# joshuacwnewton/swiftwatcher

Measured on AMD Instinct MI355X. Metric: frames/sec (segment+classify) on 1080p ROI batches, higher is better.
Workload: dtype f64 (image_filtering), f32 (CNN)

## Files before the change

### include/swk.h

```cpp
#ifndef SWK_H
#define SWK_H

#include <stdint.h>

#ifdef __cplusplus
extern "C" {
#endif

#define SWK_ABI_VERSION 2

enum {
    SWK_OK = 0,
    SWK_ERR_ARG = -1,
    SWK_ERR_HIP = -2,
    SWK_ERR_NOGPU = -3,
    SWK_ERR_CAPACITY = -4,
    SWK_ERR_NOMEM = -5,
    SWK_ERR_STALE = -6
};

enum { SWK_MEM_HOST = 0, SWK_MEM_DEVICE = 1 };

enum { SWK_ORDER_RASTER = 0, SWK_ORDER_BLOCK2X2 = 1 };

enum { SWK_GRAY_Q14 = 0, SWK_GRAY_Q15 = 1 };

typedef struct swk_ctx swk_ctx;

typedef struct swk_params {
    double  lmbda;
    double  tol;
    int32_t maxiter;
    int32_t bil_d;
    double  bil_sigma_color;
    double  bil_sigma_space;
    int32_t bil_fma;
    int32_t thresh;
    int32_t open_kh, open_kw;
    int32_t connectivity;
    int32_t label_order;
    int32_t gray_mode;
    int32_t reserved_;
} swk_params;

typedef struct swk_segment {
    int32_t label;
    int32_t r0, c0, r1, c1;
    int32_t reserved_;
    int64_t area;
    int64_t sum_r, sum_c;
} swk_segment;

typedef struct swk_input {
    const uint8_t *frames;
    int32_t mem;
    int32_t channels;
    int32_t nwin;
    int32_t n;
    int32_t Hc, Wc;
    int32_t x0, y0;
    int64_t frame_stride;
    int64_t row_stride;
} swk_input;

typedef struct swk_output {
    int32_t mem;
    int32_t seg_cap;
    uint8_t *gray, *rpca, *bilateral, *thresh, *opened, *labels;
    double  *A, *E;
    int32_t *iters;
    int32_t *nseg;
    swk_segment *segs;
    int32_t planes_on_device;
    int32_t reserved_;
} swk_output;

int32_t swk_abi_version(void);
void    swk_params_default(swk_params *p);
int32_t swk_ctx_create(int32_t device, int32_t max_windows, int32_t max_n,
                       int32_t max_Hc, int32_t max_Wc, swk_ctx **out);
void    swk_ctx_destroy(swk_ctx *ctx);
const char *swk_last_error(const swk_ctx *ctx);
int64_t swk_ctx_device_bytes(const swk_ctx *ctx);

int32_t swk_pinned_alloc(int32_t device, int64_t bytes, void **out);
int32_t swk_pinned_free(void *p);
int32_t swk_stage_frames(const uint8_t *const *frames, int32_t count, int64_t row_stride, int32_t y0, int32_t rows, int64_t x_bytes,
                         int64_t row_bytes, uint8_t *dst, int32_t threads);
int32_t swk_cut_boxes(const uint8_t *const *frames, int32_t nframes, int64_t row_stride, int32_t pixel_bytes, int32_t count,
                      const int32_t *frame_of, const int32_t *boxes, const int64_t *offsets, uint8_t *out);
int32_t swk_device_alloc(swk_ctx *ctx, int64_t bytes, void **out);
int32_t swk_device_free(swk_ctx *ctx, void *p);
int32_t swk_device_read(swk_ctx *ctx, const void *src_device, void *dst_host, int64_t bytes);

int32_t swk_batch_run(swk_ctx *ctx, const swk_input *in, const swk_params *p, swk_output *out);
int32_t swk_batch_run_groups(swk_ctx *ctx, const swk_input *groups, int32_t ngroups, const swk_params *p, swk_output *outs);

enum { SWK_YUV_I420 = 0,
       SWK_YUV_NV12 = 1 };

typedef struct swk_yuv420 {
    const uint8_t *y, *u, *v;
    int32_t mem;
    int32_t layout;
    int32_t H, W;
    int64_t y_row_stride, y_frame_stride;
    int64_t c_row_stride, c_frame_stride;
} swk_yuv420;

int32_t swk_yuv420_to_bgr(swk_ctx *ctx, const swk_yuv420 *src, int32_t count, int32_t x0, int32_t y0, int32_t Hr, int32_t Wr,
                          uint8_t *bgr, int32_t bgr_mem);

int32_t swk_bgr2gray(swk_ctx *ctx, const uint8_t *bgr, int32_t count, int32_t H, int32_t W,
                     int32_t gray_mode, uint8_t *gray);
int32_t swk_ialm(swk_ctx *ctx, const uint8_t *planes, int32_t n, int32_t P,
                 double lmbda, double tol, int32_t maxiter,
                 double *A, double *E, int32_t *iters);
int32_t swk_rpca_epilogue(swk_ctx *ctx, const double *E, int64_t count, uint8_t *S);
int32_t swk_bilateral_u8(swk_ctx *ctx, const uint8_t *src, int32_t count, int32_t H, int32_t W,
                         int32_t d, double sigma_color, double sigma_space, int32_t use_fma,
                         uint8_t *dst);
int32_t swk_thresh_tozero_u8(swk_ctx *ctx, const uint8_t *src, int64_t count, int32_t thresh,
                             uint8_t *dst);
int32_t swk_grey_open3x3_u8(swk_ctx *ctx, const uint8_t *src, int32_t count, int32_t H, int32_t W,
                            uint8_t *dst);
int32_t swk_grey_open_u8(swk_ctx *ctx, const uint8_t *src, int32_t count, int32_t H, int32_t W, int32_t kh, int32_t kw, uint8_t *dst);
int32_t swk_resize_linear_u8(swk_ctx *ctx, const uint8_t *src, int32_t count, int32_t H, int32_t W, int32_t channels, int32_t dH, int32_t dW,
                             uint8_t *dst);
int32_t swk_ccl_u8(swk_ctx *ctx, const uint8_t *src, int32_t count, int32_t H, int32_t W,
                   int32_t connectivity, int32_t label_order, int32_t *labels, int32_t *ncomp);
int32_t swk_regionprops_u8(swk_ctx *ctx, const uint8_t *labels, int32_t count, int32_t H, int32_t W,
                           int32_t seg_cap, swk_segment *segs, int32_t *nseg);

int32_t swk_classifier_input(swk_ctx *ctx, const uint8_t *crops, int64_t crops_bytes, const int64_t *offsets,
                             const int32_t *hw, int32_t nseg, const float mean[3], const float std_[3],
                             uint8_t *patches, float *net, int32_t net_mem);
int32_t swk_classifier_input_window(swk_ctx *ctx, const uint8_t *crops, int64_t crops_bytes, const int64_t *offsets,
                                    const int32_t *hw, int32_t nseg, const float mean[3], const float std_[3],
                                    int32_t pad, int32_t channels_last, uint8_t *patches, float *net, int32_t net_mem);

int32_t swk_segment_inputs(swk_ctx *ctx, const swk_input *in, int32_t frame_h, int32_t frame_w,
                           const swk_segment *segs, const int32_t *nseg, int32_t seg_cap, int32_t min_h, int32_t min_w,
                           const float mean[3], const float std_[3], int32_t pad, int32_t channels_last, int32_t first,
                           int32_t net_cap, float *net, int32_t *seg_frame, int32_t *total, int32_t *skipped);
int32_t swk_segment_inputs_last(swk_ctx *ctx, int32_t min_h, int32_t min_w, const float mean[3], const float std_[3],
                                int32_t pad, int32_t channels_last, int32_t first, int32_t net_cap, float *net,
                                int32_t *seg_frame, int32_t *total, int32_t *skipped);

int32_t swk_nhwc_bias_relu_place(void *stream, const float *src, int32_t n, int32_t sh, int32_t sw, int32_t c, int32_t crop_y,
                                 int32_t crop_x, int32_t h, int32_t w, const float *bias, float *dst, int32_t dH, int32_t dW,
                                 int32_t dC, int32_t off_y, int32_t off_x, int32_t c_off);
int32_t swk_nhwc_maxpool3s2(void *stream, const float *src, int32_t n, int32_t h, int32_t w, int32_t c, float *dst);
int32_t swk_nhwc_head2_relu_mean(void *stream, const float *x, int32_t n, int32_t px, int32_t c, const float *w, const float *bias,
                                 const float *ring, float n_pos, float *out);
int32_t swk_nhwc_head2_dropout_relu_mean(void *stream, const float *x, int32_t n, int32_t px, int32_t c, const int32_t *pos, const float *bg,
                                         int32_t n_pos, const float *w, const float *bias, const uint64_t *keys, uint64_t seed,
                                         int32_t samples, float *out);
int32_t swk_nhwc_conv7x7s2_bias_relu(void *stream, const float *src, int32_t n, int32_t side, int32_t lo, int32_t m, const float *weight,
                                     const float *bias, int32_t cout, float *dst);
int32_t swk_nhwc_conv1x1_bias_relu_place(void *stream, const float *src, int32_t n, int32_t sh, int32_t sw, int32_t cin, int32_t crop_y,
                                         int32_t crop_x, int32_t h, int32_t w, const float *weight, const float *bias, int32_t cout,
                                         float *dst, int32_t dH, int32_t dW, int32_t dC, int32_t off_y, int32_t off_x, int32_t c_off);

int32_t swk_nhwc_maxpool3s2_conv1x1_bias_relu_place(void *stream, const float *src, int32_t n, int32_t t, int32_t cin, const float *weight,
                                                    const float *bias, int32_t cout, float *dst, int32_t dH, int32_t dW, int32_t dC,
                                                    int32_t off_y, int32_t off_x, const float *ring, int32_t live_lo, int32_t live_n);


int32_t swk_nhwc_conv3x3_bias_relu_place(void *stream, const float *src, int32_t n, int32_t t, int32_t cin, const float *weight_t,
                                         const float *bias, int32_t cout, float *dst, int32_t dH, int32_t dW, int32_t dC, int32_t off_y,
                                         int32_t off_x, int32_t c_off);

int32_t swk_winograd_f2x2_3x3_weights(const float *weight, int32_t cout, int32_t cin, float *out);
int32_t swk_nhwc_conv3x3_winograd_bias_relu_place(void *stream, const float *src, int32_t n, int32_t t, int32_t cin, const float *weight_w,
                                                  const float *bias, int32_t cout, float *dst, int32_t dH, int32_t dW, int32_t dC,
                                                  int32_t off_y, int32_t off_x, int32_t c_off);

int32_t swk_winograd_f2x2_3x3_weights_bf16s(const float *weight, int32_t cout, int32_t cin, uint16_t *out);
int32_t swk_nhwc_conv3x3_winograd_bf16s_bias_relu_place(void *stream, const float *src, int32_t n, int32_t t, int32_t cin,
                                                        const uint16_t *weight_s, const float *bias, int32_t cout, float *dst, int32_t dH,
                                                        int32_t dW, int32_t dC, int32_t off_y, int32_t off_x, int32_t c_off);

int32_t swk_track_costs(const double *prev_c, const double *prev_hist0, const uint8_t *prev_has_hist,
                        const double *curr_c, int32_t n_prev, int32_t n_curr, double *cost);
int32_t swk_lsap(const double *cost, int32_t n_rows, int32_t n_cols, int32_t *col4row);

int32_t swk_median_blur_u8(const uint8_t *src, int32_t H, int32_t W, int32_t channels, int32_t ksize, uint8_t *dst);
int32_t swk_otsu_threshold_u8(const uint8_t *src, int64_t count, uint8_t *dst, int32_t *thresh);
int32_t swk_canny_u8(const uint8_t *src, int32_t H, int32_t W, int32_t low, int32_t high, uint8_t *dst);
int32_t swk_dilate_up_u8(const uint8_t *src, int32_t H, int32_t W, int32_t N, uint8_t *dst);
int32_t swk_roi_mask(const uint8_t *frame, int32_t H, int32_t W, int64_t row_stride, const int32_t corners[4],
                     int32_t crop_region[4], uint8_t *mask, int64_t mask_capacity);


#ifdef __cplusplus
}
#endif
#endif
```

### swiftwatcher_amd/_lib.py

```python
import ctypes
import os
import threading

import numpy as np

_HERE = os.path.dirname(os.path.abspath(__file__))
LIB_PATH = os.environ.get("SWK_LIB", os.path.join(_HERE, "libswk.so"))

ABI_VERSION = 2
MEM_HOST, MEM_DEVICE = 0, 1
ERR_STALE = -6
STAGE_DENSE, STAGE_WHOLE, STAGE_ROWS, STAGE_2D, STAGE_DEVICE = 0, 1, 2, 3, -1
STAGES = ("gray", "rpca", "bilateral", "thresh", "opened", "labels")
ORDER_RASTER, ORDER_BLOCK2X2 = 0, 1
GRAY_Q14, GRAY_Q15 = 0, 1
YUV_I420, YUV_NV12 = 0, 1
K_GRAY, K_IALM_STATS, K_IALM_PASS, K_IALM_SMALL, K_FILTER, K_CCL, K_PROPS, K_COPY = range(8)
KERNEL_FAMILIES = ["gray", "ialm_stats", "ialm_pass", "ialm_small", "filter", "ccl", "props", "copy"]

c_u8p = ctypes.POINTER(ctypes.c_uint8)
c_f64p = ctypes.POINTER(ctypes.c_double)
c_i32p = ctypes.POINTER(ctypes.c_int32)


class SwkError(RuntimeError):
    pass


class StaleBatch(SwkError):
    """What a batch left on the device has been overwritten by a later call on the same context."""


class Params(ctypes.Structure):
    _fields_ = [("lmbda", ctypes.c_double), ("tol", ctypes.c_double), ("maxiter", ctypes.c_int32),
                ("bil_d", ctypes.c_int32), ("bil_sigma_color", ctypes.c_double),
                ("bil_sigma_space", ctypes.c_double), ("bil_fma", ctypes.c_int32),
                ("thresh", ctypes.c_int32), ("open_kh", ctypes.c_int32), ("open_kw", ctypes.c_int32),
                ("connectivity", ctypes.c_int32), ("label_order", ctypes.c_int32),
                ("gray_mode", ctypes.c_int32), ("reserved_", ctypes.c_int32)]


class Segment(ctypes.Structure):
    _fields_ = [("label", ctypes.c_int32), ("r0", ctypes.c_int32), ("c0", ctypes.c_int32),
                ("r1", ctypes.c_int32), ("c1", ctypes.c_int32), ("reserved_", ctypes.c_int32),
                ("area", ctypes.c_int64), ("sum_r", ctypes.c_int64), ("sum_c", ctypes.c_int64)]


SEGMENT_DTYPE = np.dtype([("label", "<i4"), ("r0", "<i4"), ("c0", "<i4"), ("r1", "<i4"), ("c1", "<i4"),
                          ("reserved_", "<i4"), ("area", "<i8"), ("sum_r", "<i8"), ("sum_c", "<i8")])
assert SEGMENT_DTYPE.itemsize == ctypes.sizeof(Segment) == 48


class Input(ctypes.Structure):
    _fields_ = [("frames", ctypes.c_void_p), ("mem", ctypes.c_int32), ("channels", ctypes.c_int32),
                ("nwin", ctypes.c_int32), ("n", ctypes.c_int32), ("Hc", ctypes.c_int32), ("Wc", ctypes.c_int32),
                ("x0", ctypes.c_int32), ("y0", ctypes.c_int32),
                ("frame_stride", ctypes.c_int64), ("row_stride", ctypes.c_int64)]


class Output(ctypes.Structure):
    _fields_ = [("mem", ctypes.c_int32), ("seg_cap", ctypes.c_int32),
                ("gray", ctypes.c_void_p), ("rpca", ctypes.c_void_p), ("bilateral", ctypes.c_void_p),
                ("thresh", ctypes.c_void_p), ("opened", ctypes.c_void_p), ("labels", ctypes.c_void_p),
                ("A", ctypes.c_void_p), ("E", ctypes.c_void_p),
                ("iters", ctypes.c_void_p), ("nseg", ctypes.c_void_p), ("segs", ctypes.c_void_p),
                ("planes_on_device", ctypes.c_int32), ("reserved_", ctypes.c_int32)]


class Yuv420(ctypes.Structure):
    _fields_ = [("y", ctypes.c_void_p), ("u", ctypes.c_void_p), ("v", ctypes.c_void_p), ("mem", ctypes.c_int32),
                ("layout", ctypes.c_int32), ("H", ctypes.c_int32), ("W", ctypes.c_int32),
                ("y_row_stride", ctypes.c_int64), ("y_frame_stride", ctypes.c_int64),
                ("c_row_stride", ctypes.c_int64), ("c_frame_stride", ctypes.c_int64)]


_lib = None
_lib_lock = threading.Lock()

_SIGS = {
    "swk_abi_version": (ctypes.c_int32, []),
    "swk_params_default": (None, [ctypes.POINTER(Params)]),
    "swk_ctx_create": (ctypes.c_int32, [ctypes.c_int32] * 5 + [ctypes.POINTER(ctypes.c_void_p)]),
    "swk_ctx_destroy": (None, [ctypes.c_void_p]),
    "swk_last_error": (ctypes.c_char_p, [ctypes.c_void_p]),
    "swk_ctx_device_bytes": (ctypes.c_int64, [ctypes.c_void_p]),
    "swk_batch_run": (ctypes.c_int32, [ctypes.c_void_p, ctypes.POINTER(Input), ctypes.POINTER(Params), ctypes.POINTER(Output)]),
    "swk_batch_run_groups": (ctypes.c_int32, [ctypes.c_void_p, ctypes.POINTER(Input), ctypes.c_int32, ctypes.POINTER(Params), ctypes.POINTER(Output)]),
    "swk_yuv420_to_bgr": (ctypes.c_int32, [ctypes.c_void_p, ctypes.POINTER(Yuv420)] + [ctypes.c_int32] * 5 + [ctypes.c_void_p, ctypes.c_int32]),
    "swk_bgr2gray": (ctypes.c_int32, [ctypes.c_void_p, ctypes.c_void_p, ctypes.c_int32, ctypes.c_int32, ctypes.c_int32, ctypes.c_int32, ctypes.c_void_p]),
    "swk_ialm": (ctypes.c_int32, [ctypes.c_void_p, ctypes.c_void_p, ctypes.c_int32, ctypes.c_int32, ctypes.c_double, ctypes.c_double, ctypes.c_int32, ctypes.c_void_p, ctypes.c_void_p, ctypes.c_void_p]),
    "swk_rpca_epilogue": (ctypes.c_int32, [ctypes.c_void_p, ctypes.c_void_p, ctypes.c_int64, ctypes.c_void_p]),
    "swk_bilateral_u8": (ctypes.c_int32, [ctypes.c_void_p, ctypes.c_void_p, ctypes.c_int32, ctypes.c_int32, ctypes.c_int32, ctypes.c_int32, ctypes.c_double, ctypes.c_double, ctypes.c_int32, ctypes.c_void_p]),
    "swk_thresh_tozero_u8": (ctypes.c_int32, [ctypes.c_void_p, ctypes.c_void_p, ctypes.c_int64, ctypes.c_int32, ctypes.c_void_p]),
    "swk_grey_open3x3_u8": (ctypes.c_int32, [ctypes.c_void_p, ctypes.c_void_p, ctypes.c_int32, ctypes.c_int32, ctypes.c_int32, ctypes.c_void_p]),
    "swk_grey_open_u8": (ctypes.c_int32, [ctypes.c_void_p, ctypes.c_void_p] + [ctypes.c_int32] * 5 + [ctypes.c_void_p]),
    "swk_resize_linear_u8": (ctypes.c_int32, [ctypes.c_void_p, ctypes.c_void_p] + [ctypes.c_int32] * 6 + [ctypes.c_void_p]),
    "swk_ccl_u8": (ctypes.c_int32, [ctypes.c_void_p, ctypes.c_void_p, ctypes.c_int32, ctypes.c_int32, ctypes.c_int32, ctypes.c_int32, ctypes.c_int32, ctypes.c_void_p, ctypes.c_void_p]),
    "swk_regionprops_u8": (ctypes.c_int32, [ctypes.c_void_p, ctypes.c_void_p, ctypes.c_int32, ctypes.c_int32, ctypes.c_int32, ctypes.c_int32, ctypes.c_void_p, ctypes.c_void_p]),
    "swk_classifier_input": (ctypes.c_int32, [ctypes.c_void_p, ctypes.c_void_p, ctypes.c_int64, ctypes.c_void_p, ctypes.c_void_p, ctypes.c_int32, ctypes.c_void_p, ctypes.c_void_p, ctypes.c_void_p, ctypes.c_void_p, ctypes.c_int32]),
    "swk_set_sparse_speculation": (ctypes.c_int32, [ctypes.c_void_p, ctypes.c_double]),
    "swk_set_integer_start": (ctypes.c_int32, [ctypes.c_void_p, ctypes.c_int32]),
    "swk_last_integer_start_windows": (ctypes.c_int32, [ctypes.c_void_p, ctypes.c_void_p]),
    "swk_debug_ialm_start": (ctypes.c_int32, [ctypes.c_void_p, ctypes.c_void_p, ctypes.c_int32, ctypes.c_int32, ctypes.c_int32, ctypes.c_double] + [ctypes.c_void_p] * 7),
    "swk_debug_ialm_first_step": (ctypes.c_int32, [ctypes.c_void_p, ctypes.c_void_p, ctypes.c_int32, ctypes.c_int32, ctypes.c_int32, ctypes.c_double] + [ctypes.c_void_p] * 7),
    "swk_last_host_stage": (ctypes.c_int32, [ctypes.c_void_p, ctypes.c_void_p, ctypes.c_int32]),
    "swk_debug_resize_table": (ctypes.c_int32, [ctypes.c_void_p, ctypes.c_int32, ctypes.c_int32, ctypes.c_int32, ctypes.c_void_p, ctypes.c_void_p]),
    "swk_last_eig_sweeps": (ctypes.c_int32, [ctypes.c_void_p, ctypes.c_void_p]),
    "swk_set_norm_speculation": (ctypes.c_int32, [ctypes.c_void_p, ctypes.c_double]),
    "swk_set_norm_guard": (ctypes.c_int32, [ctypes.c_void_p, ctypes.c_double]),
    "swk_prof_guard_windows": (ctypes.c_int32, [ctypes.c_void_p, ctypes.c_void_p]),
    "swk_last_stopping_norms": (ctypes.c_int32, [ctypes.c_void_p, ctypes.c_void_p, ctypes.c_void_p, ctypes.c_int32]),
    "swk_set_start_refine": (ctypes.c_int32, [ctypes.c_void_p, ctypes.c_double]),
    "swk_prof_refined_windows": (ctypes.c_int32, [ctypes.c_void_p, ctypes.c_void_p, ctypes.c_void_p]),
    "swk_prof_pass_bytes_per_element": (ctypes.c_int32, [ctypes.c_void_p, ctypes.c_void_p]),
    "swk_prof_redo_batches": (ctypes.c_int32, [ctypes.c_void_p, ctypes.c_void_p]),
    "swk_prof_redo_windows": (ctypes.c_int32, [ctypes.c_void_p, ctypes.c_void_p]),
    "swk_nhwc_bias_relu_place": (ctypes.c_int32, [ctypes.c_void_p, ctypes.c_void_p] + [ctypes.c_int32] * 8 + [ctypes.c_void_p, ctypes.c_void_p] + [ctypes.c_int32] * 6),
    "swk_set_cnn_tuning": (ctypes.c_int32, [ctypes.c_int32, ctypes.c_int32]),
    "swk_nhwc_conv7x7s2_bias_relu": (ctypes.c_int32, [ctypes.c_void_p, ctypes.c_void_p, ctypes.c_int32, ctypes.c_int32, ctypes.c_int32, ctypes.c_int32, ctypes.c_void_p, ctypes.c_void_p, ctypes.c_int32, ctypes.c_void_p]),
    "swk_nhwc_conv1x1_bias_relu_place": (ctypes.c_int32, [ctypes.c_void_p, ctypes.c_void_p] + [ctypes.c_int32] * 8 + [ctypes.c_void_p, ctypes.c_void_p, ctypes.c_int32, ctypes.c_void_p] + [ctypes.c_int32] * 6),
    "swk_nhwc_conv3x3_bias_relu_place": (ctypes.c_int32, [ctypes.c_void_p, ctypes.c_void_p, ctypes.c_int32, ctypes.c_int32, ctypes.c_int32, ctypes.c_void_p, ctypes.c_void_p, ctypes.c_int32, ctypes.c_void_p] + [ctypes.c_int32] * 6),
    "swk_nhwc_conv3x3_winograd_bias_relu_place": (ctypes.c_int32, [ctypes.c_void_p, ctypes.c_void_p, ctypes.c_int32, ctypes.c_int32, ctypes.c_int32, ctypes.c_void_p, ctypes.c_void_p, ctypes.c_int32, ctypes.c_void_p] + [ctypes.c_int32] * 6),
    "swk_winograd_f2x2_3x3_weights": (ctypes.c_int32, [ctypes.c_void_p, ctypes.c_int32, ctypes.c_int32, ctypes.c_void_p]),
    "swk_nhwc_conv3x3_winograd_bf16s_bias_relu_place": (ctypes.c_int32, [ctypes.c_void_p, ctypes.c_void_p, ctypes.c_int32, ctypes.c_int32, ctypes.c_int32, ctypes.c_void_p, ctypes.c_void_p, ctypes.c_int32, ctypes.c_void_p] + [ctypes.c_int32] * 6),
    "swk_winograd_f2x2_3x3_weights_bf16s": (ctypes.c_int32, [ctypes.c_void_p, ctypes.c_int32, ctypes.c_int32, ctypes.c_void_p]),
    "swk_nhwc_maxpool3s2_conv1x1_bias_relu_place": (ctypes.c_int32, [ctypes.c_void_p, ctypes.c_void_p, ctypes.c_int32, ctypes.c_int32, ctypes.c_int32, ctypes.c_void_p, ctypes.c_void_p, ctypes.c_int32, ctypes.c_void_p] + [ctypes.c_int32] * 5 + [ctypes.c_void_p, ctypes.c_int32, ctypes.c_int32]),
    "swk_nhwc_maxpool3s2": (ctypes.c_int32, [ctypes.c_void_p, ctypes.c_void_p, ctypes.c_int32, ctypes.c_int32, ctypes.c_int32, ctypes.c_int32, ctypes.c_void_p]),
    "swk_nhwc_head2_relu_mean": (ctypes.c_int32, [ctypes.c_void_p, ctypes.c_void_p, ctypes.c_int32, ctypes.c_int32, ctypes.c_int32, ctypes.c_void_p,
                                                  ctypes.c_void_p, ctypes.c_void_p, ctypes.c_float, ctypes.c_void_p]),
    "swk_nhwc_head2_dropout_relu_mean": (ctypes.c_int32, [ctypes.c_void_p, ctypes.c_void_p, ctypes.c_int32, ctypes.c_int32, ctypes.c_int32, ctypes.c_void_p,
                                                          ctypes.c_void_p, ctypes.c_int32, ctypes.c_void_p, ctypes.c_void_p, ctypes.c_void_p, ctypes.c_uint64,
                                                          ctypes.c_int32, ctypes.c_void_p]),
    "swk_segment_inputs": (ctypes.c_int32, [ctypes.c_void_p, ctypes.c_void_p, ctypes.c_int32, ctypes.c_int32, ctypes.c_void_p, ctypes.c_void_p, ctypes.c_int32, ctypes.c_int32, ctypes.c_int32, ctypes.c_void_p, ctypes.c_void_p, ctypes.c_int32, ctypes.c_int32, ctypes.c_int32, ctypes.c_int32, ctypes.c_void_p, ctypes.c_void_p, ctypes.c_void_p, ctypes.c_void_p]),
    "swk_segment_inputs_last": (ctypes.c_int32, [ctypes.c_void_p, ctypes.c_int32, ctypes.c_int32, ctypes.c_void_p, ctypes.c_void_p, ctypes.c_int32, ctypes.c_int32, ctypes.c_int32, ctypes.c_int32, ctypes.c_void_p, ctypes.c_void_p, ctypes.c_void_p, ctypes.c_void_p]),
    "swk_device_alloc": (ctypes.c_int32, [ctypes.c_void_p, ctypes.c_int64, ctypes.POINTER(ctypes.c_void_p)]),
    "swk_device_free": (ctypes.c_int32, [ctypes.c_void_p, ctypes.c_void_p]),
    "swk_device_read": (ctypes.c_int32, [ctypes.c_void_p, ctypes.c_void_p, ctypes.c_void_p, ctypes.c_int64]),
    "swk_classifier_input_window": (ctypes.c_int32, [ctypes.c_void_p, ctypes.c_void_p, ctypes.c_int64, ctypes.c_void_p, ctypes.c_void_p, ctypes.c_int32, ctypes.c_void_p, ctypes.c_void_p, ctypes.c_int32, ctypes.c_int32, ctypes.c_void_p, ctypes.c_void_p, ctypes.c_int32]),
    "swk_track_costs": (ctypes.c_int32, [ctypes.c_void_p, ctypes.c_void_p, ctypes.c_void_p, ctypes.c_void_p, ctypes.c_int32, ctypes.c_int32, ctypes.c_void_p]),
    "swk_lsap": (ctypes.c_int32, [ctypes.c_void_p, ctypes.c_int32, ctypes.c_int32, ctypes.c_void_p]),
    "swk_median_blur_u8": (ctypes.c_int32, [ctypes.c_void_p, ctypes.c_int32, ctypes.c_int32, ctypes.c_int32, ctypes.c_int32, ctypes.c_void_p]),
    "swk_otsu_threshold_u8": (ctypes.c_int32, [ctypes.c_void_p, ctypes.c_int64, ctypes.c_void_p, ctypes.c_void_p]),
    "swk_canny_u8": (ctypes.c_int32, [ctypes.c_void_p, ctypes.c_int32, ctypes.c_int32, ctypes.c_int32, ctypes.c_int32, ctypes.c_void_p]),
    "swk_dilate_up_u8": (ctypes.c_int32, [ctypes.c_void_p, ctypes.c_int32, ctypes.c_int32, ctypes.c_int32, ctypes.c_void_p]),
    "swk_roi_mask": (ctypes.c_int32, [ctypes.c_void_p, ctypes.c_int32, ctypes.c_int32, ctypes.c_int64, ctypes.c_void_p, ctypes.c_void_p, ctypes.c_void_p, ctypes.c_int64]),
    "swk_pinned_alloc": (ctypes.c_int32, [ctypes.c_int32, ctypes.c_int64, ctypes.POINTER(ctypes.c_void_p)]),
    "swk_pinned_free": (ctypes.c_int32, [ctypes.c_void_p]),
    "swk_cut_boxes": (ctypes.c_int32, [ctypes.c_void_p, ctypes.c_int32, ctypes.c_int64, ctypes.c_int32, ctypes.c_int32, ctypes.c_void_p, ctypes.c_void_p, ctypes.c_void_p, ctypes.c_void_p]),
    "swk_stage_frames": (ctypes.c_int32, [ctypes.c_void_p, ctypes.c_int32, ctypes.c_int64, ctypes.c_int32, ctypes.c_int32, ctypes.c_int64, ctypes.c_int64, ctypes.c_void_p, ctypes.c_int32]),
    "swk_prof_enable": (ctypes.c_int32, [ctypes.c_void_p, ctypes.c_int32]),
    "swk_prof_reset": (ctypes.c_int32, [ctypes.c_void_p]),
    "swk_prof_get": (ctypes.c_int32, [ctypes.c_void_p, ctypes.c_int32, ctypes.POINTER(ctypes.c_double), ctypes.POINTER(ctypes.c_int64)]),
    "swk_prof_window_iters": (ctypes.c_int32, [ctypes.c_void_p, ctypes.POINTER(ctypes.c_int64)]),
    "swk_set_ialm_variant": (ctypes.c_int32, [ctypes.c_void_p, ctypes.c_int32]),
    "swk_set_pass_tuning": (ctypes.c_int32, [ctypes.c_void_p, ctypes.c_int32]),
    "swk_set_eig_method": (ctypes.c_int32, [ctypes.c_void_p, ctypes.c_int32]),
}
EXPORTS = sorted(_SIGS)


def _preload_torch_hip_runtime():
    import importlib.util
    try:
        spec = importlib.util.find_spec("torch")
    except (ImportError, ValueError):
        spec = None
    if spec is None or not spec.origin:
        return
    cand = os.path.join(os.path.dirname(spec.origin), "lib", "libamdhip64.so")
    if os.path.exists(cand):
        try:
            ctypes.CDLL(cand, mode=ctypes.RTLD_GLOBAL)
        except OSError:
            pass


def load():
    global _lib
    with _lib_lock:
        if _lib is None:
            if not os.path.exists(LIB_PATH):
                raise SwkError("libswk.so not built: run `python swiftwatcher_amd/csrc/build.py` "
                               "(there is no CPU fallback)")
            _preload_torch_hip_runtime()
            lib = ctypes.CDLL(LIB_PATH)
            for name, (res, args) in _SIGS.items():
                fn = getattr(lib, name)
                fn.restype = res
                fn.argtypes = args
            if lib.swk_abi_version() != ABI_VERSION:
                raise SwkError("libswk.so ABI version mismatch")
            _lib = lib
    return _lib


def default_params(**overrides):
    p = Params()
    load().swk_params_default(ctypes.byref(p))
    for k, v in overrides.items():
        if not hasattr(p, k):
            raise TypeError("unknown swk parameter %r" % k)
        setattr(p, k, v)
    return p


def _ptr(a):
    return ctypes.c_void_p(a.ctypes.data) if a is not None else None


class _SerialisedLib:

    def __init__(self, lib, lock):
        self._lib, self._lock = lib, lock

    def __getattr__(self, name):
        fn = getattr(self._lib, name)
        lock = self._lock

        def call(*args):
            with lock:
                return fn(*args)
        call.__name__ = name
        setattr(self, name, call)
        return call


class Context:

    def __init__(self, device=0, max_windows=0, max_n=0, max_Hc=0, max_Wc=0):
        self._lock = threading.RLock()
        self._lib = _SerialisedLib(load(), self._lock)
        self._h = ctypes.c_void_p()
        rc = self._lib.swk_ctx_create(device, max_windows, max_n, max_Hc, max_Wc, ctypes.byref(self._h))
        if rc != 0:
            msg = self._lib.swk_last_error(None)
            self._h = None
            raise SwkError("swk_ctx_create failed (%d): %s" % (rc, msg.decode() if msg else "?"))
        self.device = device
        self.generation = 0
        self._plane_pool = {}

    def close(self):
        if getattr(self, "_h", None):
            for ptrs in self._plane_pool.values():
                for p in ptrs:
                    self._lib.swk_device_free(self._h, ctypes.c_void_p(p))
            self._plane_pool = {}
            self._lib.swk_ctx_destroy(self._h)
            self._h = None

    def device_alloc(self, nbytes):
        ptr = ctypes.c_void_p()
        self._check(self._lib.swk_device_alloc(self._h, int(nbytes), ctypes.byref(ptr)))
        return ptr.value

    def device_free(self, ptr):
        if getattr(self, "_h", None) and ptr:
            self._check(self._lib.swk_device_free(self._h, ctypes.c_void_p(ptr)))

    def device_read(self, ptr, shape, dtype=np.uint8):
        out = np.empty(shape, dtype)
        self._check(self._lib.swk_device_read(self._h, ctypes.c_void_p(ptr), _ptr(out), out.nbytes))
        return out

    def staging(self, shape):
        key = (threading.get_ident(), tuple(shape))
        with self._lock:
            cache = self.__dict__.setdefault("_staging", {})
            arr = cache.get(key)
            if arr is None:
                if len(cache) >= 3:
                    cache.pop(next(iter(cache)))
                arr = cache[key] = pinned_empty(shape, np.uint8, device=self.device)
        return arr

    def take_planes(self, nbytes):
        with self._lock:
            free = self._plane_pool.get(nbytes)
            if free:
                return free.pop()
        return self.device_alloc(nbytes)

    def give_planes(self, ptr, nbytes, keep=4):
        if not getattr(self, "_h", None):
            return
        with self._lock:
            free = self._plane_pool.setdefault(nbytes, [])
            if len(free) < keep:
                free.append(ptr)
                return
        self.device_free(ptr)

    def __del__(self):
        try:
            self.close()
        except Exception:
            pass

    def _check(self, rc):
        if rc != 0:
            msg = self._lib.swk_last_error(self._h)
            raise SwkError("libswk error %d: %s" % (rc, msg.decode() if msg else "?"))

    @property
    def device_bytes(self):
        return int(self._lib.swk_ctx_device_bytes(self._h))

    def prof_enable(self, on=True):
        self._check(self._lib.swk_prof_enable(self._h, int(bool(on))))

    def prof_reset(self):
        self._check(self._lib.swk_prof_reset(self._h))

    def prof(self):
        out = {}
        for i, name in enumerate(KERNEL_FAMILIES):
            ms, n = ctypes.c_double(), ctypes.c_int64()
            self._check(self._lib.swk_prof_get(self._h, i, ctypes.byref(ms), ctypes.byref(n)))
            out[name] = (ms.value, n.value)
        wi = ctypes.c_int64()
        self._check(self._lib.swk_prof_window_iters(self._h, ctypes.byref(wi)))
        out["window_iters"] = wi.value
        return out

    def set_ialm_variant(self, variant):
        self._check(self._lib.swk_set_ialm_variant(self._h, int(variant)))

    def set_pass_tuning(self, flags):
        self._check(self._lib.swk_set_pass_tuning(self._h, int(flags)))

    def set_sparse_speculation(self, factor):
        self._check(self._lib.swk_set_sparse_speculation(self._h, float(factor)))

    def set_integer_start(self, on):
        self._check(self._lib.swk_set_integer_start(self._h, int(bool(on))))

    def set_norm_guard(self, rel):
        self._check(self._lib.swk_set_norm_guard(self._h, float(rel)))

    @property
    def guard_windows(self):
        v = ctypes.c_int64(0)
        self._check(self._lib.swk_prof_guard_windows(self._h, ctypes.byref(v)))
        return v.value

    def set_start_refine(self, tau):
        self._check(self._lib.swk_set_start_refine(self._h, float(tau)))

    @property
    def refined_windows(self):
        a, b = ctypes.c_int64(0), ctypes.c_int64(0)
        self._check(self._lib.swk_prof_refined_windows(self._h, ctypes.byref(a), ctypes.byref(b)))
        return a.value, b.value

    def last_stopping_norms(self, cap=4096):
        r, e = np.zeros(cap), np.zeros(cap)
        n = self._lib.swk_last_stopping_norms(self._h, _ptr(r), _ptr(e), cap)
        if n < 0:
            self._check(n)
        return r[:min(n, cap)], e[:min(n, cap)]

    def set_norm_speculation(self, factor):
        self._check(self._lib.swk_set_norm_speculation(self._h, float(factor)))

    @property
    def pass_bytes_per_element(self):
        v = ctypes.c_double(0)
        self._check(self._lib.swk_prof_pass_bytes_per_element(self._h, ctypes.byref(v)))
        return v.value

    @property
    def last_eig_sweeps(self):
        v = ctypes.c_int32(0)
        self._check(self._lib.swk_last_eig_sweeps(self._h, ctypes.byref(v)))
        return v.value

    @property
    def last_integer_start_windows(self):
        v = ctypes.c_int32(0)
        self._check(self._lib.swk_last_integer_start_windows(self._h, ctypes.byref(v)))
        return v.value

    def debug_ialm_start(self, windows, lmbda=0.01):
        x = np.ascontiguousarray(windows, np.uint8)
        nwin, n, P = x.shape
        G = np.zeros((nwin, n, n), np.float64)
        sumsq, maxv = np.zeros(nwin, np.uint64), np.zeros(nwin, np.uint32)
        int_gram, scal = np.zeros(nwin, np.int32), np.zeros((nwin, 4), np.float64)
        nblk, ran = np.zeros(1, np.int32), np.zeros(1, np.int32)
        self._check(self._lib.swk_debug_ialm_start(self._h, _ptr(x), nwin, n, P, float(lmbda), _ptr(G), _ptr(sumsq), _ptr(maxv),
                                                   _ptr(int_gram), _ptr(scal), _ptr(nblk), _ptr(ran)))
        return dict(G=G, sumsq=sumsq, maxv=maxv, int_gram=int_gram, dual_norm=scal[:, 0], mu_0=scal[:, 1], thr_0=scal[:, 2],
                    dnorm=scal[:, 3], nblk=int(nblk[0]), gram8_ran=int(ran[0]))

    def debug_ialm_first_step(self, windows, lmbda=0.01):
        x = np.ascontiguousarray(windows, np.uint8)
        nwin, n, P = x.shape
        B_fin, B_std = np.zeros((nwin, n, n), np.float64), np.zeros((nwin, n, n), np.float64)
        refine, sweeps, int_gram = np.zeros(nwin, np.int32), np.zeros(nwin, np.int32), np.zeros(nwin, np.int32)
        cond_sum, scal = np.zeros(nwin, np.float64), np.zeros((nwin, 4), np.float64)
        self._check(self._lib.swk_debug_ialm_first_step(self._h, _ptr(x), nwin, n, P, float(lmbda), _ptr(B_fin), _ptr(B_std),
                                                        _ptr(refine), _ptr(cond_sum), _ptr(sweeps), _ptr(int_gram), _ptr(scal)))
        return dict(B_fin=B_fin, B_std=B_std, refine=refine, cond_sum=cond_sum, sweeps=sweeps, int_gram=int_gram,
                    dual_norm=scal[:, 0], mu_0=scal[:, 1], thr_0=scal[:, 2], dnorm=scal[:, 3])

    def last_host_stage(self, cap=256):
        kinds = np.zeros(cap, np.int32)
        n = self._lib.swk_last_host_stage(self._h, _ptr(kinds), cap)
        if n < 0:
            self._check(n)
        return [int(k) for k in kinds[:min(n, cap)]]

    @property
    def redo_batches(self):
        v = ctypes.c_int64(0)
        self._check(self._lib.swk_prof_redo_batches(self._h, ctypes.byref(v)))
        return v.value

    @property
    def redo_windows(self):
        v = ctypes.c_int64(0)
        self._check(self._lib.swk_prof_redo_windows(self._h, ctypes.byref(v)))
        return v.value

    def set_eig_method(self, method):
        self._check(self._lib.swk_set_eig_method(self._h, int(method)))

    def batch_run_raw(self, inp, params, out):
        with self._lock:
            self.generation += 1
            generation = self.generation
            self._check(self._lib.swk_batch_run(self._h, ctypes.byref(inp), ctypes.byref(params), ctypes.byref(out)))
        return generation

    def _group_io(self, frames, nwin, n, crop, reverse_frames, seg_cap, stages, want_A, want_E, device_stages=False):
        F = nwin * n
        on_device = hasattr(frames, "data_ptr") and getattr(frames, "is_cuda", False)
        shape = tuple(frames.shape)
        if str(frames.dtype) != ("torch.uint8" if on_device else "uint8") or shape[0] != F or len(shape) not in (3, 4):
            raise ValueError("frames must be uint8 (nwin*n, H, W[, 3])")
        if on_device:
            strides, base = tuple(int(x) for x in frames.stride()), frames.data_ptr()
        else:
            strides, base = frames.strides, frames.ctypes.data
        ch = 1 if len(shape) == 3 else shape[3]
        if (len(shape) == 4 and (strides[3] != 1 or strides[2] != ch)) or (len(shape) == 3 and strides[2] != 1):
            raise ValueError("frames must be contiguous along columns/channels")
        H, W = shape[1], shape[2]
        x0, y0, Wc, Hc = crop if crop is not None else (0, 0, W, H)
        if x0 < 0 or y0 < 0 or x0 + Wc > W or y0 + Hc > H:
            raise ValueError("crop rectangle outside the frame")
        inp = Input(frames=base + ((F - 1) * strides[0] if reverse_frames else 0), mem=MEM_DEVICE if on_device else MEM_HOST,
                    channels=ch, nwin=nwin, n=n, Hc=Hc, Wc=Wc, x0=x0, y0=y0,
                    frame_stride=-strides[0] if reverse_frames else strides[0], row_stride=strides[1])
        res = {}
        out = Output(mem=MEM_HOST, seg_cap=seg_cap)
        if device_stages and stages:
            planes = res["planes"] = DevicePlanes(self, tuple(stages), F, Hc, Wc)
            out.planes_on_device = 1
            for name in stages:
                setattr(out, name, planes.pointer(name))
        else:
            for name in stages:
                res[name] = np.empty((F, Hc, Wc), np.uint8)
                setattr(out, name, res[name].ctypes.data)
        P = Hc * Wc
        if want_A:
            res["A"] = np.empty((nwin, P, n), np.float64)
            out.A = res["A"].ctypes.data
        if want_E:
            res["E"] = np.empty((nwin, P, n), np.float64)
            out.E = res["E"].ctypes.data
        res["iters"] = np.zeros(nwin, np.int32)
        res["nseg"] = np.zeros(F, np.int32)
        res["segs"] = np.zeros((F, seg_cap), SEGMENT_DTYPE)
        out.iters = res["iters"].ctypes.data
        out.nseg = res["nseg"].ctypes.data
        out.segs = res["segs"].ctypes.data
        return inp, out, res

    def batch_run(self, frames, nwin, n, crop=None, params=None, stages=STAGES, want_A=False, want_E=False, seg_cap=255,
                  device_stages=False, reverse_frames=False):
        inp, out, res = self._group_io(frames, nwin, n, crop, reverse_frames, seg_cap, stages, want_A, want_E, device_stages)
        res["generation"] = self.batch_run_raw(inp, params or default_params(), out)
        return res

    def batch_run_groups(self, groups, params=None, stages=STAGES, want_A=False, want_E=False, seg_cap=255):
        params = params or default_params()
        G = len(groups)
        if G < 1:
            raise ValueError("no groups")
        ins = (Input * G)()
        outs = (Output * G)()
        results = []
        for g, grp in enumerate(groups):
            ins[g], outs[g], res = self._group_io(grp["frames"], int(grp["nwin"]), int(grp["n"]), grp.get("crop"),
                                                  bool(grp.get("reverse_frames", False)), int(grp.get("seg_cap", seg_cap)), stages,
                                                  want_A, want_E)
            results.append(res)
        with self._lock:
            self.generation += 1
            generation = self.generation
            self._check(self._lib.swk_batch_run_groups(self._h, ins, G, ctypes.byref(params), outs))
        for res in results:
            res["generation"] = generation
        return results

    def yuv420_to_bgr(self, y, u, v=None, rect=None, device_out=False):
        on_device = hasattr(y, "data_ptr") and getattr(y, "is_cuda", False)
        planes = [y, u] + ([v] if v is not None else [])
        want = "torch.uint8" if on_device else "uint8"
        if not on_device:
            planes = [p if isinstance(p, np.ndarray) and p.dtype == np.uint8 and p.ndim and p.strides[-1] == 1 else np.ascontiguousarray(p, np.uint8)
                      for p in planes]
        if any((hasattr(p, "data_ptr") and getattr(p, "is_cuda", False)) != on_device or str(p.dtype) != want for p in planes):
            raise ValueError("the planes must be uint8, all numpy arrays or all tensors on the context's GPU")
        single = len(planes[0].shape) == 2
        if single:
            planes = [p[None] for p in planes]

        def geometry(p):
            if on_device:
                return tuple(p.shape), tuple(int(x) for x in p.stride()), p.data_ptr()
            return p.shape, p.strides, p.ctypes.data
        (yshape, ystr, yptr), (cshape, cstr, uptr) = geometry(planes[0]), geometry(planes[1])
        if len(yshape) != 3 or ystr[2] != 1:
            raise ValueError("y must be (count, H, W), contiguous along a row")
        count, H, W = yshape
        ch, cw = (H + 1) // 2, (W + 1) // 2
        if v is not None:
            vshape, vstr, vptr = geometry(planes[2])
            if tuple(cshape) != (count, ch, cw) or tuple(vshape) != (count, ch, cw) or cstr[2] != 1 or tuple(vstr) != tuple(cstr):
                raise ValueError("u and v must be (count, ceil(H/2), ceil(W/2)) with equal strides, contiguous along a row")
            layout = YUV_I420
        else:
            vptr = None
            ok = (len(cshape) == 4 and tuple(cshape) == (count, ch, cw, 2) and cstr[3] == 1 and cstr[2] == 2) or \
                 (len(cshape) == 3 and tuple(cshape) == (count, ch, 2 * cw) and cstr[2] == 1)
            if not ok:
                raise ValueError("the NV12 chroma plane must be (count, ceil(H/2), ceil(W/2), 2) or (count, ceil(H/2), 2 ceil(W/2))")
            layout = YUV_NV12
        x0, y0, Wr, Hr = rect if rect is not None else (0, 0, W, H)
        src = Yuv420(y=yptr, u=uptr, v=vptr, mem=MEM_DEVICE if on_device else MEM_HOST, layout=layout, H=H, W=W,
                     y_row_stride=ystr[1], y_frame_stride=ystr[0], c_row_stride=cstr[1], c_frame_stride=cstr[0])
        shape = (count, int(Hr), int(Wr), 3) if Hr > 0 and Wr > 0 and count > 0 else (1, 1, 1, 3)
        if device_out:
            import torch
            out = torch.empty(shape, dtype=torch.uint8, device="cuda:%d" % self.device)
            optr, omem = ctypes.c_void_p(out.data_ptr()), MEM_DEVICE
        else:
            out = np.empty(shape, np.uint8)
            optr, omem = _ptr(out), MEM_HOST
        self._check(self._lib.swk_yuv420_to_bgr(self._h, ctypes.byref(src), count, int(x0), int(y0), int(Hr), int(Wr), optr, omem))
        return out[0] if single else out

    def bgr2gray(self, bgr, gray_mode=GRAY_Q14):
        bgr = np.ascontiguousarray(bgr, np.uint8)
        single = bgr.ndim == 3
        b4 = bgr[None] if single else bgr
        cnt, H, W, _ = b4.shape
        out = np.empty((cnt, H, W), np.uint8)
        self._check(self._lib.swk_bgr2gray(self._h, _ptr(b4), cnt, H, W, gray_mode, _ptr(out)))
        return out[0] if single else out

    def ialm(self, planes, lmbda=0.01, tol=0.001, maxiter=100, want_E=True):
        planes = np.ascontiguousarray(planes, np.uint8)
        n, P = planes.shape
        A = np.empty((P, n), np.float64)
        E = np.empty((P, n), np.float64) if want_E else None
        it = np.zeros(1, np.int32)
        self._check(self._lib.swk_ialm(self._h, _ptr(planes), n, P, lmbda, tol, maxiter, _ptr(A), _ptr(E), _ptr(it)))
        return A, E, int(it[0])

    def rpca_epilogue(self, E):
        E = np.ascontiguousarray(E, np.float64)
        out = np.empty(E.shape, np.uint8)
        self._check(self._lib.swk_rpca_epilogue(self._h, _ptr(E), E.size, _ptr(out)))
        return out

    def _planes(self, a):
        a = np.ascontiguousarray(a, np.uint8)
        return (a[None], True) if a.ndim == 2 else (a, False)

    def bilateral_u8(self, src, d=7, sigma_color=15.0, sigma_space=1.0, use_fma=False):
        s, single = self._planes(src)
        out = np.empty_like(s)
        self._check(self._lib.swk_bilateral_u8(self._h, _ptr(s), s.shape[0], s.shape[1], s.shape[2], d,
                                               sigma_color, sigma_space, int(bool(use_fma)), _ptr(out)))
        return out[0] if single else out

    def thresh_tozero_u8(self, src, thresh=15):
        s = np.ascontiguousarray(src, np.uint8)
        out = np.empty_like(s)
        self._check(self._lib.swk_thresh_tozero_u8(self._h, _ptr(s), s.size, thresh, _ptr(out)))
        return out

    def grey_open3x3_u8(self, src):
        s, single = self._planes(src)
        out = np.empty_like(s)
        self._check(self._lib.swk_grey_open3x3_u8(self._h, _ptr(s), s.shape[0], s.shape[1], s.shape[2], _ptr(out)))
        return out[0] if single else out

    def grey_open_u8(self, src, size):
        s, single = self._planes(src)
        out = np.empty_like(s)
        self._check(self._lib.swk_grey_open_u8(self._h, _ptr(s), s.shape[0], s.shape[1], s.shape[2], int(size[0]), int(size[1]), _ptr(out)))
        return out[0] if single else out

    def resize_linear_u8(self, frame, dsize):
        f = np.ascontiguousarray(frame, np.uint8)
        H, W = f.shape[:2]
        ch = 1 if f.ndim == 2 else f.shape[2]
        dW, dH = int(dsize[0]), int(dsize[1])
        out = np.empty((dH, dW) + ((ch,) if f.ndim == 3 else ()), np.uint8)
        self._check(self._lib.swk_resize_linear_u8(self._h, _ptr(f), 1, H, W, ch, dH, dW, _ptr(out)))
        return out

    def ccl_u8(self, src, connectivity=8, label_order=ORDER_BLOCK2X2):
        s, single = self._planes(src)
        lab = np.empty(s.shape, np.int32)
        nc = np.zeros(s.shape[0], np.int32)
        self._check(self._lib.swk_ccl_u8(self._h, _ptr(s), s.shape[0], s.shape[1], s.shape[2], connectivity,
                                         label_order, _ptr(lab), _ptr(nc)))
        return (int(nc[0]), lab[0]) if single else (nc, lab)

    def classifier_input(self, crops, mean, std, want_patches=False, net_ptr=None, pad=100, channels_last=False):
        n = len(crops)
        flat = [np.ascontiguousarray(c, np.uint8).reshape(-1) for c in crops]
        sizes = np.array([f.size for f in flat], np.int64)
        offsets = np.concatenate([[0], np.cumsum(sizes)[:-1]]).astype(np.int64)
        packed = np.concatenate(flat) if n else np.zeros(0, np.uint8)
        hw = np.array([[c.shape[0], c.shape[1]] for c in crops], np.int32)
        m = np.asarray(mean, np.float32)
        s = np.asarray(std, np.float32)
        patches = np.empty((n, 24, 24, 3), np.uint8) if want_patches else None
        net = None
        if net_ptr is None:
            net = np.empty((n, 3, 24 + 2 * pad, 24 + 2 * pad), np.float32)
            nptr, nmem = _ptr(net), MEM_HOST
        else:
            nptr, nmem = ctypes.c_void_p(net_ptr), MEM_DEVICE
        self._check(self._lib.swk_classifier_input_window(self._h, _ptr(packed), packed.size, _ptr(offsets), _ptr(hw), n,
                                                          _ptr(m), _ptr(s), int(pad), 1 if channels_last else 0, _ptr(patches), nptr,
                                                          nmem))
        return patches, net

    def segment_inputs(self, inp, frame_hw, segs_ptr, nseg_ptr, seg_cap, mean, std, net_ptr, net_cap, first=0, pad=8,
                       min_seg_size=(24, 24), seg_frame_ptr=None, channels_last=False):
        m = np.asarray(mean, np.float32)
        s = np.asarray(std, np.float32)
        total = ctypes.c_int32(0)
        skipped = ctypes.c_int32(0)
        self._check(self._lib.swk_segment_inputs(self._h, ctypes.byref(inp), int(frame_hw[0]), int(frame_hw[1]),
                                                 ctypes.c_void_p(segs_ptr), ctypes.c_void_p(nseg_ptr), int(seg_cap),
                                                 int(min_seg_size[0]), int(min_seg_size[1]), _ptr(m), _ptr(s), int(pad),
                                                 1 if channels_last else 0, int(first), int(net_cap), ctypes.c_void_p(net_ptr),
                                                 ctypes.c_void_p(seg_frame_ptr) if seg_frame_ptr else None,
                                                 ctypes.byref(total), ctypes.byref(skipped)))
        return total.value, skipped.value

    def segment_inputs_last(self, generation, mean, std, net_ptr, net_cap, first=0, pad=8, min_seg_size=(24, 24),
                            seg_frame_ptr=None, channels_last=False, known_total=-1):
        m = np.asarray(mean, np.float32)
        s = np.asarray(std, np.float32)
        total = ctypes.c_int32(int(known_total))
        skipped = ctypes.c_int32(0)
        with self._lock:
            if generation != self.generation:
                raise StaleBatch("the context has run another batch since")
            rc = self._lib.swk_segment_inputs_last(self._h, int(min_seg_size[0]), int(min_seg_size[1]), _ptr(m), _ptr(s), int(pad),
                                                   1 if channels_last else 0, int(first), int(net_cap), ctypes.c_void_p(net_ptr),
                                                   ctypes.c_void_p(seg_frame_ptr) if seg_frame_ptr else None,
                                                   ctypes.byref(total), ctypes.byref(skipped))
            if rc == ERR_STALE:
                raise StaleBatch("the context no longer holds that batch")
            self._check(rc)
        return total.value, skipped.value

    def debug_resize_table(self, first, count, route=1):
        bounds = np.empty((count, 24, 2), np.int32)
        coeffs = np.empty((count, 24, 343), np.int32)
        self._check(self._lib.swk_debug_resize_table(self._h, int(first), int(count), int(route), _ptr(bounds), _ptr(coeffs)))
        return bounds, coeffs

    def regionprops_u8(self, labels, seg_cap=255):
        s, single = self._planes(labels)
        segs = np.zeros((s.shape[0], seg_cap), SEGMENT_DTYPE)
        nseg = np.zeros(s.shape[0], np.int32)
        self._check(self._lib.swk_regionprops_u8(self._h, _ptr(s), s.shape[0], s.shape[1], s.shape[2], seg_cap,
                                                 _ptr(segs), _ptr(nseg)))
        return (segs[0, :nseg[0]], int(nseg[0])) if single else (segs, nseg)


def stage_frames(frames, y0, y1, x0, x1, dst, threads=4):
    f0 = frames[0]
    px = f0.strides[1] if f0.ndim >= 2 else 1
    ok = all(f.dtype == np.uint8 and f.shape == f0.shape and f.strides == f0.strides for f in frames) and \
        f0.ndim in (2, 3) and (f0.ndim == 2 or (f0.strides[2] == 1 and f0.strides[1] == f0.shape[2])) and \
        (f0.ndim == 3 or f0.strides[1] == 1) and f0.strides[0] >= f0.shape[1] * px and dst.flags.c_contiguous
    if not ok:
        for i, f in enumerate(frames):
            dst[i] = f[y0:y1, x0:x1]
        return
    ptrs = (ctypes.c_void_p * len(frames))(*[f.ctypes.data for f in frames])
    rc = load().swk_stage_frames(ptrs, len(frames), f0.strides[0], y0, y1 - y0, x0 * px, (x1 - x0) * px, dst.ctypes.data, threads)
    if rc:
        raise SwkError("swk_stage_frames failed (%d)" % rc)


def cut_boxes(arrays, frame_of, boxes):
    a0 = arrays[0]
    px = a0.strides[1]
    h = np.maximum(boxes[:, 1] - boxes[:, 0], 0).astype(np.int64)
    w = np.maximum(boxes[:, 3] - boxes[:, 2], 0).astype(np.int64)
    sizes = h * w * px
    offsets = np.zeros(len(boxes), np.int64)
    if len(boxes) > 1:
        np.cumsum(sizes[:-1], out=offsets[1:])
    out = np.empty(int(sizes.sum()) if len(boxes) else 0, np.uint8)
    if len(boxes):
        ptrs = (ctypes.c_void_p * len(arrays))(*[a.ctypes.data for a in arrays])
        fo = np.ascontiguousarray(frame_of, np.int32)
        bx = np.ascontiguousarray(boxes, np.int32)
        rc = load().swk_cut_boxes(ptrs, len(arrays), a0.strides[0], px, len(boxes), fo.ctypes.data, bx.ctypes.data, offsets.ctypes.data,
                                  out.ctypes.data)
        if rc:
            raise SwkError("swk_cut_boxes failed (%d)" % rc)
    return out, offsets


class DevicePlanes:

    def __init__(self, ctx, stages, F, Hc, Wc):
        self.ctx, self.stages, self.F, self.Hc, self.Wc = ctx, stages, F, Hc, Wc
        self.plane = F * Hc * Wc
        self.nbytes = (self.plane + 3) // 4 * 4 * len(stages)
        self.ptr = ctx.take_planes(self.nbytes)

    def pointer(self, stage):
        return self.ptr + self.stages.index(stage) * ((self.plane + 3) // 4 * 4)

    def read(self, stage, frame):
        return self.ctx.device_read(self.pointer(stage) + frame * self.Hc * self.Wc, (self.Hc, self.Wc))

    def read_stack(self, stage):
        return self.ctx.device_read(self.pointer(stage), (self.F, self.Hc, self.Wc))

    def __del__(self):
        try:
            if self.ptr:
                self.ctx.give_planes(self.ptr, self.nbytes)
                self.ptr = 0
        except Exception:
            pass


def track_costs(prev_c, prev_hist0, prev_has_hist, curr_c):
    n_prev, n_curr = len(prev_c), len(curr_c)
    pc = np.ascontiguousarray(prev_c, np.float64).reshape(n_prev, 2)
    ph = np.ascontiguousarray(prev_hist0, np.float64).reshape(n_prev, 2)
    hh = np.ascontiguousarray(prev_has_hist, np.uint8).reshape(n_prev)
    cc = np.ascontiguousarray(curr_c, np.float64).reshape(n_curr, 2)
    packed = np.concatenate([pc.ravel(), ph.ravel(), cc.ravel()])
    return track_costs_packed(packed, hh.tobytes(), n_prev, n_curr)


def track_costs_packed(packed, has_hist, n_prev, n_curr):
    n = n_prev + n_curr
    cost = np.empty((n, n), np.float64)
    base = packed.ctypes.data
    rc = _track_costs_fn()(base, base + 16 * n_prev, has_hist, base + 32 * n_prev, n_prev, n_curr, cost.ctypes.data)
    if rc:
        raise SwkError("swk_track_costs failed (%d)" % rc)
    return cost


_fast = {}


def _track_costs_fn():
    fn = _fast.get("costs")
    if fn is None:
        fn = _fast["costs"] = load().swk_track_costs
    return fn


def lsap(cost):
    if cost.dtype != np.float64 or not cost.flags.c_contiguous:
        cost = np.ascontiguousarray(cost, np.float64)
    nr, nc = cost.shape
    out = np.empty(nr, np.int32)
    fn = _fast.get("lsap")
    if fn is None:
        fn = _fast["lsap"] = load().swk_lsap
    rc = fn(cost.ctypes.data, nr, nc, out.ctypes.data)
    if rc:
        raise SwkError("swk_lsap failed (%d)" % rc)
    return out


def pinned_empty(shape, dtype=np.uint8, device=0):
    import weakref
    count = int(np.prod(shape))
    nbytes = max(count * np.dtype(dtype).itemsize, 1)
    lib = load()
    ptr = ctypes.c_void_p()
    if lib.swk_pinned_alloc(int(device), nbytes, ctypes.byref(ptr)) != 0 or not ptr.value:
        return np.empty(shape, dtype)
    buf = (ctypes.c_uint8 * nbytes).from_address(ptr.value)
    weakref.finalize(buf, lib.swk_pinned_free, ctypes.c_void_p(ptr.value))
    return np.frombuffer(buf, dtype=dtype, count=count).reshape(shape)


def _host_call(name, *args):
    rc = getattr(load(), name)(*args)
    if rc:
        raise SwkError("%s failed (%d)" % (name, rc))


def median_blur_u8(image, ksize):
    a = np.ascontiguousarray(image, np.uint8)
    ch = 1 if a.ndim == 2 else a.shape[2]
    out = np.empty_like(a)
    _host_call("swk_median_blur_u8", _ptr(a), a.shape[0], a.shape[1], ch, int(ksize), _ptr(out))
    return out


def otsu_threshold_u8(image):
    a = np.ascontiguousarray(image, np.uint8)
    out = np.empty_like(a)
    t = ctypes.c_int32(0)
    _host_call("swk_otsu_threshold_u8", _ptr(a), a.size, _ptr(out), ctypes.byref(t))
    return t.value, out


def canny_u8(image, low, high):
    a = np.ascontiguousarray(image, np.uint8)
    out = np.empty_like(a)
    _host_call("swk_canny_u8", _ptr(a), a.shape[0], a.shape[1], int(low), int(high), _ptr(out))
    return out


def dilate_up_u8(image, N):
    a = np.ascontiguousarray(image, np.uint8)
    out = np.empty_like(a)
    _host_call("swk_dilate_up_u8", _ptr(a), a.shape[0], a.shape[1], int(N), _ptr(out))
    return out


def roi_mask(frame, corners):
    if hasattr(frame, "as_full_frame"):
        frame = frame.as_full_frame()
    if not isinstance(frame, np.ndarray):
        frame = np.asarray(frame)
    if frame.dtype != np.uint8 or frame.ndim != 3 or frame.shape[2] != 3 or frame.strides[2] != 1 or frame.strides[1] != 3:
        frame = np.ascontiguousarray(frame, np.uint8)
    c = np.array([corners[0][0], corners[0][1], corners[1][0], corners[1][1]], np.int32)
    crop = np.zeros(4, np.int32)
    left, right = min(c[0], c[2]), max(c[0], c[2])
    width = int(right - left)
    hc, wc = int(0.5 * width) + int(0.125 * width), width + 2 * int(0.125 * width)
    mask = np.empty((max(hc, 1), max(wc, 1)), np.uint8)
    _host_call("swk_roi_mask", _ptr(frame), frame.shape[0], frame.shape[1], frame.strides[0], _ptr(c), _ptr(crop), _ptr(mask), mask.size)
    return [(int(crop[0]), int(crop[1])), (int(crop[2]), int(crop[3]))], mask


_default_ctx = {}
_ctx_lock = threading.Lock()


def default_context(device=0):
    with _ctx_lock:
        ctx = _default_ctx.get(device)
        if ctx is None:
            ctx = _default_ctx[device] = Context(device)
    return ctx
```

### swiftwatcher_amd/csrc/cnn_common.h

```cpp
#pragma once
#include "swk_internal.h"

#include <cstring>

namespace swk {

typedef float f16v __attribute__((ext_vector_type(16)));
typedef __bf16 bf16x8 __attribute__((ext_vector_type(8)));

struct Place {
    float *dst;
    int dH, dW, dC, off_y, off_x, c_off;
};
struct Crop {
    int sh, sw, crop_y, crop_x;
};

inline bool place_ok(const Place &p, int h, int w, int c, bool quads, const Crop *crop = nullptr)
{
    if (!p.dst || c < 1 || p.off_y < 0 || p.off_x < 0 || p.off_y + h > p.dH || p.off_x + w > p.dW || p.c_off < 0 || p.c_off + c > p.dC) return false;
    if (quads && ((c & 3) || (p.dC & 3) || (p.c_off & 3) || ((uintptr_t)p.dst & 15))) return false;
    return !crop || (crop->crop_y >= 0 && crop->crop_x >= 0 && crop->crop_y + h <= crop->sh && crop->crop_x + w <= crop->sw);
}

int launch_expand1x1_split_bf16(hipStream_t s, const float *src, int64_t rows, const Crop &cr, int cin, int h, int w, const float *wgt,
                                const float *bias, int cout, const Place &pl);
extern int g_expand_split_bf16;
extern int g_wino_bf16s_layout;

__device__ __forceinline__ void store_bias_relu(float *q, const f16v &acc, int g, const float4 b)
{
    float4 v;
    v.x = fmaxf(acc[4 * g] + b.x, 0.0f);
    v.y = fmaxf(acc[4 * g + 1] + b.y, 0.0f);
    v.z = fmaxf(acc[4 * g + 2] + b.z, 0.0f);
    v.w = fmaxf(acc[4 * g + 3] + b.w, 0.0f);
    *(float4 *)q = v;
}

__device__ __forceinline__ void split3(float x, __bf16 &a, __bf16 &b, __bf16 &c)
{
    a = (__bf16)x;
    const float r = x - (float)a;
    b = (__bf16)r;
    c = (__bf16)(r - (float)b);
}
inline void split3_host(float x, uint16_t part[3])
{
    for (int i = 0; i < 3; ++i) {
        uint32_t u;
        float back;
        memcpy(&u, &x, 4);
        u = (u + 0x7fffu + ((u >> 16) & 1u)) & 0xffff0000u;
        memcpy(&back, &u, 4);
        part[i] = (uint16_t)(u >> 16);
        x -= back;
    }
}

inline void winograd_U(const float g[9], double U[4][4])
{
    static const double G[4][3] = {{1.0, 0.0, 0.0}, {0.5, 0.5, 0.5}, {0.5, -0.5, 0.5}, {0.0, 0.0, 1.0}};
    double tmp[4][3];
    for (int a = 0; a < 4; ++a)
        for (int c = 0; c < 3; ++c) tmp[a][c] = G[a][0] * g[c] + G[a][1] * g[3 + c] + G[a][2] * g[6 + c];
    for (int a = 0; a < 4; ++a)
        for (int c = 0; c < 4; ++c) U[a][c] = tmp[a][0] * G[c][0] + tmp[a][1] * G[c][1] + tmp[a][2] * G[c][2];
}

template <int N>
__device__ __forceinline__ void lds_dma_copy(unsigned lds, const void *g, unsigned voff)
{
    static_assert(N >= 1 && N <= 3, "1 KB pieces per statement");
    unsigned keep;
#define SWK_LDS_DMA(pieces)                                                                                                 \
    asm volatile("s_mov_b32 %0, m0\n\ts_mov_b32 m0, %2\n\ts_nop 0\n\t" pieces "s_mov_b32 m0, %0" : "=&s"(keep) : "v"(voff), "s"(lds), "s"(g) : "memory")
#define SWK_LDS_DMA_PIECE(offset) "global_load_lds_dwordx4 %1, %3" offset "\n\t"
    if constexpr (N == 1) SWK_LDS_DMA(SWK_LDS_DMA_PIECE(""));
    else if constexpr (N == 2) SWK_LDS_DMA(SWK_LDS_DMA_PIECE("") SWK_LDS_DMA_PIECE(" offset:1024"));
    else SWK_LDS_DMA(SWK_LDS_DMA_PIECE("") SWK_LDS_DMA_PIECE(" offset:1024") SWK_LDS_DMA_PIECE(" offset:2048"));
#undef SWK_LDS_DMA_PIECE
#undef SWK_LDS_DMA
}
template <int KEEP>
__device__ __forceinline__ void lds_dma_wait()
{
    asm volatile("s_waitcnt vmcnt(%0)" ::"n"(KEEP) : "memory");
}

}
```

### swiftwatcher_amd/csrc/cnn_conv1x1.hip

```cpp
#include "cnn_common.h"

namespace swk {

template <int NBLK, int KC, int D, int CS, int NWV>
__global__ __launch_bounds__(64 * NWV) void k_conv1x1_relu_place(const float *__restrict__ src, int64_t rows, int sh, int sw, int cin, int crop_y,
                                                            int crop_x, int h, int w, const float *__restrict__ wgt, const float *__restrict__ bias,
                                                            int cout, float *__restrict__ dst, int dH, int dW, int dC, int off_y, int off_x, int c_off,
                                                            FastDiv fhw, FastDiv fw)
{
    constexpr int NP = 32 * NBLK, PITCH = NP + 1, KH = KC / 2, NV = KH / 4, NB = NBLK / CS, NT = 64 * NWV, SLOTS = NWV / CS;
    static_assert(NBLK % CS == 0 && NWV % CS == 0, "column splits");
    extern __shared__ float lds[];
    const int tid = threadIdx.x, lane = tid & 63, wave = tid >> 6, r = lane & 31, hh = lane >> 5;
    float *lbias = lds + ((cin * PITCH + 3) & ~3);
    const int hw = h * w;
    const int cs = wave % CS;
    const int64_t ntiles = (rows + 31) >> 5, stride = (int64_t)gridDim.x * SLOTS;
    int64_t tile = (int64_t)blockIdx.x * SLOTS + wave / CS;

    auto locate = [&](int64_t t, int64_t &ro) -> const float * {
        const unsigned m = (unsigned)t * 32u + (unsigned)r;
        const bool valid = m < (unsigned)rows;
        const unsigned mm = valid ? m : (unsigned)rows - 1u;
        const unsigned b = fhw.div(mm), rem = mm - b * (unsigned)hw;
        const unsigned y = fw.div(rem), x = rem - y * (unsigned)w;
        ro = valid ? (((int64_t)b * dH + off_y + y) * dW + off_x + x) * (int64_t)dC + c_off + 32 * NB * cs : -1;
        return src + (((int64_t)b * sh + crop_y + y) * sw + crop_x + x) * (int64_t)cin + KH * hh;
    };
    float4 a[D][NV];
    int64_t ro = -1, ro_next = -1;
    const float *p = src, *pn = src;
    if (tile < ntiles) {
        p = locate(tile, ro);
#pragma unroll
        for (int d = 0; d < D; ++d)
#pragma unroll
            for (int v = 0; v < NV; ++v) a[d][v] = *(const float4 *)(p + KC * d + 4 * v);
    }
    for (int co = tid >> 4; co < NP; co += NT / 16)
        for (int c4 = (tid & 15) * 4; c4 < cin; c4 += 64) {
            const float4 wv = co < cout ? *(const float4 *)(wgt + (int64_t)co * cin + c4) : make_float4(0.0f, 0.0f, 0.0f, 0.0f);
            float *q = lds + c4 * PITCH + co;
            q[0] = wv.x; q[PITCH] = wv.y; q[2 * PITCH] = wv.z; q[3 * PITCH] = wv.w;
        }
    for (int i = tid; i < NP; i += NT) lbias[i] = i < cout ? bias[i] : 0.0f;
    __syncthreads();

    for (; tile < ntiles; tile += stride) {
        const bool more = tile + stride < ntiles;
        if (more) pn = locate(tile + stride, ro_next);
        f16v acc[NB];
#pragma unroll
        for (int nb = 0; nb < NB; ++nb)
#pragma unroll
            for (int e = 0; e < 16; ++e) acc[nb][e] = 0.0f;
        for (int kb = 0; kb < cin; kb += KC * D) {
#pragma unroll
            for (int d = 0; d < D; ++d) {
                const int k0 = kb + KC * d;
                float av[KH];
#pragma unroll
                for (int v = 0; v < NV; ++v) { av[4 * v] = a[d][v].x; av[4 * v + 1] = a[d][v].y; av[4 * v + 2] = a[d][v].z; av[4 * v + 3] = a[d][v].w; }
                const int kn = k0 + KC * D;
                if (kn < cin) {
#pragma unroll
                    for (int v = 0; v < NV; ++v) a[d][v] = *(const float4 *)(p + kn + 4 * v);
                } else if (more) {
#pragma unroll
                    for (int v = 0; v < NV; ++v) a[d][v] = *(const float4 *)(pn + kn - cin + 4 * v);
                }
                const float *wrow = lds + (k0 + KH * hh) * PITCH + 32 * NB * cs + r;
                float bw[2][NB];
#pragma unroll
                for (int nb = 0; nb < NB; ++nb) bw[0][nb] = wrow[32 * nb];
#pragma unroll
                for (int i = 0; i < KH; ++i) {
                    if (i < KH - 1) {
#pragma unroll
                        for (int nb = 0; nb < NB; ++nb) bw[(i + 1) & 1][nb] = wrow[(i + 1) * PITCH + 32 * nb];
                    }
#pragma unroll
                    for (int nb = 0; nb < NB; ++nb) acc[nb] = __builtin_amdgcn_mfma_f32_32x32x2f32(bw[i & 1][nb], av[i], acc[nb], 0, 0, 0);
                    if (i < KH - 1) __builtin_amdgcn_sched_group_barrier(0x100 , NB, 0);
                    __builtin_amdgcn_sched_group_barrier(0x008 , NB, 0);
                }
            }
        }
        if (ro >= 0) {
            float *o = dst + ro + 4 * hh;
#pragma unroll
            for (int nb = 0; nb < NB; ++nb)
#pragma unroll
                for (int g = 0; g < 4; ++g) {
                    const int c = nb * 32 + 8 * g;
                    if (32 * NB * cs + c + 4 * hh < cout) store_bias_relu(o + c, acc[nb], g, *(const float4 *)(lbias + 32 * NB * cs + c + 4 * hh));
                }
        }
        p = pn;
        ro = ro_next;
    }
}

template <int NBLK, int KC, int D, int CS, int NWV>
static int launch_conv1x1_d(hipStream_t s, const float *src, int64_t rows, const Crop &cr, int cin, int h, int w, const float *wgt,
                            const float *bias, int cout, const Place &pl)
{
    const size_t lds = (size_t)(((cin * (32 * NBLK + 1) + 3) & ~3) + 32 * NBLK) * sizeof(float);
    static unsigned long long attr_mask = 0;
    if (!ensure_dyn_lds((const void *)k_conv1x1_relu_place<NBLK, KC, D, CS, NWV>, 160 * 1024 - 256, attr_mask)) return SWK_ERR_HIP;
    if (lds > 160 * 1024 - 256 || rows > (int64_t)0x7fffff00) return SWK_ERR_CAPACITY;
    constexpr int SLOTS = NWV / CS;
    const int64_t ntiles = (rows + 31) / 32;
    int64_t blocks = (ntiles + SLOTS - 1) / SLOTS;
    const int64_t by_lds = (int64_t)((160 * 1024 - 256) / lds), by_waves = 16 / NWV;
    const int64_t per_cu = by_lds < 1 ? 1 : (by_lds < by_waves ? by_lds : by_waves);
    const int64_t cap = 256 * per_cu;
    if (blocks > cap) blocks = cap;
    hipLaunchKernelGGL((k_conv1x1_relu_place<NBLK, KC, D, CS, NWV>), dim3((unsigned)blocks), dim3(64 * NWV), lds, s, src, rows, cr.sh, cr.sw, cin,
                       cr.crop_y, cr.crop_x, h, w, wgt, bias, cout, pl.dst, pl.dH, pl.dW, pl.dC, pl.off_y, pl.off_x, pl.c_off, FastDiv((unsigned)(h * w)), FastDiv((unsigned)w));
    return hipGetLastError() == hipSuccess ? SWK_OK : SWK_ERR_HIP;
}

int g_expand_split_bf16 = getenv("SWK_EXPAND_SPLIT_BF16") ? atoi(getenv("SWK_EXPAND_SPLIT_BF16")) : 0;
int g_conv1x1_ring = 0;

#define SWK_C1_ARGS s, src, rows, cr, cin, h, w, wgt, bias, cout, pl
template <int NBLK>
static int launch_conv1x1(hipStream_t s, const float *src, int64_t rows, const Crop &cr, int cin, int h, int w, const float *wgt, const float *bias,
                          int cout, const Place &pl)
{
    constexpr int CS = NBLK >= 6 ? 2 : 1;
    if (g_conv1x1_ring == 0) {
        const int64_t ntiles = (rows + 31) / 32;
        const int nwv = ntiles >= 16 * 160 / CS ? 16 : ntiles >= 8 * 160 / CS ? 8 : 4;
#define SWK_C1_BY_WAVES(KC)                                                              \
        do {                                                                             \
            if (nwv == 16) return launch_conv1x1_d<NBLK, KC, 1, CS, 16>(SWK_C1_ARGS);    \
            if (nwv == 8) return launch_conv1x1_d<NBLK, KC, 1, CS, 8>(SWK_C1_ARGS);      \
            return launch_conv1x1_d<NBLK, KC, 1, CS, 4>(SWK_C1_ARGS);                    \
        } while (0)
        if (cin % 32 == 0) SWK_C1_BY_WAVES(32);
        if (cin == 48) SWK_C1_BY_WAVES(48);
        SWK_C1_BY_WAVES(16);
#undef SWK_C1_BY_WAVES
    }
    if (cin % 32 == 0) {
        const int n = cin / 32, dmax = NBLK >= 6 ? 2 : 4;
        const int d = dmax >= 4 && n % 4 == 0 ? 4 : dmax >= 3 && n % 3 == 0 ? 3 : dmax >= 2 && n % 2 == 0 ? 2 : 1;
        switch (d) {
        case 4: if constexpr (NBLK < 6) return launch_conv1x1_d<NBLK, 32, 4, 1, 8>(SWK_C1_ARGS);
        case 3: if constexpr (NBLK < 6) return launch_conv1x1_d<NBLK, 32, 3, 1, 8>(SWK_C1_ARGS);
        case 2: return launch_conv1x1_d<NBLK, 32, 2, 1, 8>(SWK_C1_ARGS);
        default: return launch_conv1x1_d<NBLK, 32, 1, 1, 8>(SWK_C1_ARGS);
        }
    }
    if (cin == 48) return launch_conv1x1_d<NBLK, 48, 1, 1, 8>(SWK_C1_ARGS);
    return launch_conv1x1_d<NBLK, 16, 1, 1, 8>(SWK_C1_ARGS);
}
#undef SWK_C1_ARGS

}

#pragma GCC visibility push(default)
extern "C" {

int32_t swk_nhwc_conv1x1_bias_relu_place(void *stream, const float *src, int32_t n, int32_t sh, int32_t sw, int32_t cin, int32_t crop_y,
                                         int32_t crop_x, int32_t h, int32_t w, const float *weight, const float *bias, int32_t cout,
                                         float *dst, int32_t dH, int32_t dW, int32_t dC, int32_t off_y, int32_t off_x, int32_t c_off)
{
    const swk::Place pl{dst, dH, dW, dC, off_y, off_x, c_off};
    const swk::Crop cr{sh, sw, crop_y, crop_x};
    if (!src || !weight || !bias || n < 1 || h < 1 || w < 1 || cin < 16 || (cin & 15) || cin > 1024 || cout > 256 ||
        !swk::place_ok(pl, h, w, cout, true, &cr) || ((((uintptr_t)src) | ((uintptr_t)weight)) & 15))
        return SWK_ERR_ARG;
    using namespace swk;
    const int64_t rows = (int64_t)n * h * w;
    hipStream_t s = (hipStream_t)stream;
    if (g_expand_split_bf16 && cout == 4 * cin) {
        const int rc = launch_expand1x1_split_bf16(s, src, rows, cr, cin, h, w, weight, bias, cout, pl);
        if (rc != SWK_ERR_ARG) return rc;
    }
    switch ((cout + 31) / 32) {
    case 1: return launch_conv1x1<1>(s, src, rows, cr, cin, h, w, weight, bias, cout, pl);
    case 2: return launch_conv1x1<2>(s, src, rows, cr, cin, h, w, weight, bias, cout, pl);
    case 3: return launch_conv1x1<3>(s, src, rows, cr, cin, h, w, weight, bias, cout, pl);
    case 4: return launch_conv1x1<4>(s, src, rows, cr, cin, h, w, weight, bias, cout, pl);
    case 6: return launch_conv1x1<6>(s, src, rows, cr, cin, h, w, weight, bias, cout, pl);
    case 8: return launch_conv1x1<8>(s, src, rows, cr, cin, h, w, weight, bias, cout, pl);
    default: return SWK_ERR_ARG;
    }
}

int32_t swk_set_cnn_tuning(int32_t knob, int32_t value)
{
    if (knob == 0 && (value == 0 || value == 1)) { swk::g_conv1x1_ring = value; return SWK_OK; }
    if (knob == 1 && (value == 0 || value == 1)) { swk::g_expand_split_bf16 = value; return SWK_OK; }
    if (knob == 2 && value >= 0 && value <= 2) { swk::g_wino_bf16s_layout = value; return SWK_OK; }
    return SWK_ERR_ARG;
}

}
#pragma GCC visibility pop
```

### swiftwatcher_amd/csrc/cnn_wino3x3_bf16s.hip

```cpp
#include "cnn_common.h"

#include <type_traits>

namespace swk {

static int wino_bf16s_spp(int cin, int cout) { return cin == 64 && cout == 256 ? 2 : cin / 16; }

template <int KG> struct WinoVPad { static constexpr int value = KG == 6 ? 3 : 16 / KG; };

template <int NBLK, int SPP>
__global__ __launch_bounds__(64 * NBLK, 2) void k_wino3x3_bf16s_relu_place(const float *__restrict__ src, int nseg, int t, int T,
                                                                          const uint16_t *__restrict__ wu, const float *__restrict__ bias,
                                                                          int cout, float *__restrict__ dst, int dH, int dW, int dC, int off_y,
                                                                          int off_x, int c_off, FastDiv fTT, FastDiv fT)
{
    constexpr int NW = NBLK, NT = 64 * NW, KG = NBLK, CIN = 8 * KG, S = CIN / 16, PHS = S / SPP, SLOTS = 64, NP = 32 * NBLK;
    constexpr int VT = SLOTS + WinoVPad<KG>::value;
    constexpr int WPB = SPP * 3 * 1024;
    static_assert(S % SPP == 0 && NT == SLOTS * KG, "one staging item per thread");
    extern __shared__ uint4 lds_w[];
    char *const Wl = (char *)lds_w;
    uint4 *const V0 = (uint4 *)(Wl + 2 * NW * WPB), *const V1 = V0 + 3 * KG * VT;
    float *const lbias = (float *)(V1 + 3 * KG * VT);
    const int tid = threadIdx.x, lane = tid & 63, wave = tid >> 6, r = lane & 31, hh = lane >> 5;
    const int o = t - 2, TT = T * T;
    const int64_t ntiles = (int64_t)nseg * TT, src_floats = (int64_t)nseg * t * t * CIN;
    const int64_t ntasks = (ntiles + SLOTS - 1) / SLOTS;
    for (int i = tid; i < NP; i += NT) lbias[i] = i < cout ? bias[i] : 0.0f;

    const int sg = tid % KG, sslot = tid / KG;
    unsigned sbase;
    int slim;
    const char *const srcb = (const char *)src;
    auto stage_setup = [&](int64_t task) {
        int64_t m = task * SLOTS + sslot;
        if (m >= ntiles) m = ntiles - 1;
        const unsigned bu = fTT.div((unsigned)m), rem = (unsigned)m - bu * (unsigned)TT, ty = fT.div(rem), tx = rem - ty * (unsigned)T;
        const int64_t b = bu;
        const int64_t base = (((b * t + 2 * ty) * t + 2 * tx) * (int64_t)CIN + 8 * sg) * 4;
        const int64_t lim = src_floats * 4 - 32 - base;
        sbase = (unsigned)base;
        slim = (int)(lim < (1 << 30) ? lim : (1 << 30));
    };
    float4 st[4][2];
    auto stage_issue = [&](int p) {
        const int xi = p >> 2, nu = p & 3;
        const int ra0 = (0x1210 >> (4 * xi)) & 15, ra1 = (0x3122 >> (4 * xi)) & 15;
        const int rb0 = (0x1210 >> (4 * nu)) & 15, rb1 = (0x3122 >> (4 * nu)) & 15;
        const int os[4] = {(ra0 * t + rb0) * (CIN * 4), (ra0 * t + rb1) * (CIN * 4), (ra1 * t + rb0) * (CIN * 4), (ra1 * t + rb1) * (CIN * 4)};
#pragma unroll
        for (int i = 0; i < 4; ++i) {
            const char *q = srcb + (sbase + (unsigned)(os[i] < slim ? os[i] : slim));
            st[i][0] = *(const float4 *)q;
            st[i][1] = *(const float4 *)(q + 16);
        }
    };
    auto stage_store = [&](int p, uint4 *Vn) {
        const float sx = (p >> 2) == 1 ? 1.0f : -1.0f, sn = (p & 3) == 1 ? 1.0f : -1.0f;
        bf16x8 v1, v2, v3;
#pragma unroll
        for (int h = 0; h < 2; ++h) {
            const float a[4] = {st[0][h].x, st[0][h].y, st[0][h].z, st[0][h].w}, b[4] = {st[1][h].x, st[1][h].y, st[1][h].z, st[1][h].w},
                        c[4] = {st[2][h].x, st[2][h].y, st[2][h].z, st[2][h].w}, d[4] = {st[3][h].x, st[3][h].y, st[3][h].z, st[3][h].w};
#pragma unroll
            for (int e = 0; e < 4; ++e) {
                const float v = __builtin_fmaf(__builtin_fmaf(d[e], sn, c[e]), sx, __builtin_fmaf(b[e], sn, a[e]));
                __bf16 x1, x2, x3;
                split3(v, x1, x2, x3);
                v1[4 * h + e] = x1; v2[4 * h + e] = x2; v3[4 * h + e] = x3;
            }
        }
        uint4 *q = Vn + sg * VT + sslot;
        q[0] = __builtin_bit_cast(uint4, v1);
        q[KG * VT] = __builtin_bit_cast(uint4, v2);
        q[2 * KG * VT] = __builtin_bit_cast(uint4, v3);
    };

    const unsigned wvoff = (unsigned)(lane * 16);
    auto w_issue = [&](int g, int buf) {
        const char *gp = (const char *)wu + ((int64_t)g * NW + __builtin_amdgcn_readfirstlane(wave)) * WPB;
        const unsigned l = __builtin_amdgcn_readfirstlane((unsigned)(uintptr_t)(Wl + (buf * NW + wave) * WPB));
#pragma unroll
        for (int sub = 0; sub < SPP; ++sub) lds_dma_copy<3>(l + sub * 3072u, gp + sub * 3072, wvoff);
    };

    int64_t task = blockIdx.x;
    if (task < ntasks) {
        stage_setup(task);
        stage_issue(0);
        stage_store(0, V0);
        w_issue(0, 0);
    }
    lds_dma_wait<0>();
    __syncthreads();
    for (; task < ntasks; task += gridDim.x) {
        int64_t ro[2];
        bool valid[2], vy1[2], vx1[2];
#pragma unroll
        for (int tg = 0; tg < 2; ++tg) {
            const int64_t m = task * SLOTS + tg * 32 + r;
            valid[tg] = m < ntiles;
            const int64_t mm = valid[tg] ? m : ntiles - 1;
            const unsigned bu = fTT.div((unsigned)mm), rem = (unsigned)mm - bu * (unsigned)TT;
            const int ty = (int)fT.div(rem), tx = (int)(rem - (unsigned)ty * (unsigned)T);
            const int64_t b = bu;
            ro[tg] = ((b * dH + off_y + 2 * ty) * dW + off_x + 2 * tx) * (int64_t)dC + c_off + 32 * wave + 4 * hh;
            vy1[tg] = 2 * ty + 1 < o;
            vx1[tg] = 2 * tx + 1 < o;
        }
        const bool more = task + gridDim.x < ntasks;
        f16v Y[2][2][2];
#pragma unroll
        for (int i = 0; i < 2; ++i)
#pragma unroll
            for (int j = 0; j < 2; ++j)
#pragma unroll
                for (int tg = 0; tg < 2; ++tg)
#pragma unroll
                    for (int e = 0; e < 16; ++e) Y[i][j][tg][e] = 0.0f;
        auto phase = [&](const char *Wb, const uint4 *Vc, int s0, f16v *M) {
            const uint4 *wq = (const uint4 *)Wb + lane;
#pragma unroll
            for (int sub = 0; sub < SPP; ++sub) {
                const int s = s0 + sub;
                const bf16x8 u1 = __builtin_bit_cast(bf16x8, wq[(3 * sub) * 64]), u2 = __builtin_bit_cast(bf16x8, wq[(3 * sub + 1) * 64]),
                             u3 = __builtin_bit_cast(bf16x8, wq[(3 * sub + 2) * 64]);
#pragma unroll
                for (int tg = 0; tg < 2; ++tg) {
                    const uint4 *vq = Vc + (2 * s + hh) * VT + 32 * tg + r;
                    const bf16x8 x1 = __builtin_bit_cast(bf16x8, vq[0]), x2 = __builtin_bit_cast(bf16x8, vq[KG * VT]),
                                 x3 = __builtin_bit_cast(bf16x8, vq[2 * KG * VT]);
                    M[tg] = __builtin_amdgcn_mfma_f32_32x32x16_bf16(u1, x3, M[tg], 0, 0, 0);
                    M[tg] = __builtin_amdgcn_mfma_f32_32x32x16_bf16(u2, x2, M[tg], 0, 0, 0);
                    M[tg] = __builtin_amdgcn_mfma_f32_32x32x16_bf16(u3, x1, M[tg], 0, 0, 0);
                    M[tg] = __builtin_amdgcn_mfma_f32_32x32x16_bf16(u1, x2, M[tg], 0, 0, 0);
                    M[tg] = __builtin_amdgcn_mfma_f32_32x32x16_bf16(u2, x1, M[tg], 0, 0, 0);
                    M[tg] = __builtin_amdgcn_mfma_f32_32x32x16_bf16(u1, x1, M[tg], 0, 0, 0);
                }
            }
        };
        for (int p = 0; p < 16; ++p) {
            const uint4 *Vc = (p & 1) ? V1 : V0;
            uint4 *Vn = (p & 1) ? V0 : V1;
            const int pn = (p + 1) & 15;
            if (p == 15 && more) stage_setup(task + gridDim.x);
            const int xi = p >> 2, nu = p & 3;
            const float ax[2] = {xi < 3 ? 1.0f : 0.0f, xi == 0 ? 0.0f : xi == 1 ? 1.0f : -1.0f};
            const float an[2] = {nu < 3 ? 1.0f : 0.0f, nu == 0 ? 0.0f : nu == 1 ? 1.0f : -1.0f};
            f16v M[2];
#pragma unroll
            for (int tg = 0; tg < 2; ++tg)
#pragma unroll
                for (int e = 0; e < 16; ++e) M[tg][e] = 0.0f;
#pragma unroll
            for (int h = 0; h < PHS; ++h) {
                const int g = p * PHS + h, gn = g + 1 == 16 * PHS ? 0 : g + 1;
                w_issue(gn, (g + 1) & 1);
                if (h == 0) stage_issue(pn);
                phase(Wl + ((g & 1) * NW + wave) * WPB, Vc, h * SPP, M);
                if (h == PHS - 1) {
                    stage_store(pn, Vn);
#pragma unroll
                    for (int i = 0; i < 2; ++i)
#pragma unroll
                        for (int j = 0; j < 2; ++j) {
                            const float c = ax[i] * an[j];
                            if (c != 0.0f) {
#pragma unroll
                                for (int tg = 0; tg < 2; ++tg)
#pragma unroll
                                    for (int e = 0; e < 16; ++e) Y[i][j][tg][e] = __builtin_fmaf(M[tg][e], c, Y[i][j][tg][e]);
                            }
                        }
                }
                if (h == 0 && PHS > 1) lds_dma_wait<8>();
                else lds_dma_wait<0>();
                if (h == PHS - 1) __syncthreads();
            }
        }
#pragma unroll
        for (int tg = 0; tg < 2; ++tg) {
            if (!valid[tg]) continue;
#pragma unroll
            for (int i = 0; i < 2; ++i)
#pragma unroll
                for (int j = 0; j < 2; ++j) {
                    if ((i == 1 && !vy1[tg]) || (j == 1 && !vx1[tg])) continue;
                    float *q = dst + ro[tg] + ((int64_t)i * dW + j) * dC;
#pragma unroll
                    for (int gq = 0; gq < 4; ++gq) {
                        const int c = 32 * wave + 8 * gq + 4 * hh;
                        if (c < cout) store_bias_relu(q + 8 * gq, Y[i][j][tg], gq, *(const float4 *)(lbias + c));
                    }
                }
        }
    }
}

template <int NBLK, int SPP>
static int launch_wino3x3_bf16s(hipStream_t s, const float *src, int n, int t, const uint16_t *wu, const float *bias, int cout, const Place &pl)
{
    constexpr int NW = NBLK, KG = NBLK, CIN = 8 * NBLK, VT = 64 + WinoVPad<KG>::value;
    const size_t lds = (size_t)2 * NW * SPP * 3 * 1024 + (size_t)2 * 3 * KG * VT * 16 + 32 * NBLK * sizeof(float);
    static_assert((size_t)2 * NW * SPP * 3 * 1024 + (size_t)2 * 3 * KG * VT * 16 + 32 * NBLK * 4 <= 160 * 1024 - 256, "LDS of one workgroup");
    static unsigned long long attr_mask = 0;
    if (!ensure_dyn_lds((const void *)k_wino3x3_bf16s_relu_place<NBLK, SPP>, 160 * 1024 - 256, attr_mask)) return SWK_ERR_HIP;
    if ((int64_t)n * t * t * CIN * 4 >= ((int64_t)1 << 32)) return SWK_ERR_CAPACITY;
    const int T = (t - 2 + 1) / 2;
    const int64_t ntiles = (int64_t)n * T * T;
    int64_t blocks = (ntiles + 63) / 64;
    const int64_t by_lds = (int64_t)((160 * 1024 - 256) / lds), by_waves = 8 / NW;
    const int64_t per_cu = by_waves < 1 ? 1 : (by_lds < by_waves ? by_lds : by_waves);
    if (blocks > 256 * per_cu) blocks = 256 * per_cu;
    hipLaunchKernelGGL((k_wino3x3_bf16s_relu_place<NBLK, SPP>), dim3((unsigned)blocks), dim3(64 * NW), lds, s, src, n, t, T, wu, bias, cout, pl.dst,
                       pl.dH, pl.dW, pl.dC, pl.off_y, pl.off_x, pl.c_off, FastDiv((unsigned)(T * T)), FastDiv((unsigned)T));
    return hipGetLastError() == hipSuccess ? SWK_OK : SWK_ERR_HIP;
}

template <int KG> struct WinoVPadW { static constexpr int value = KG == 4 ? 2 : KG == 6 ? 3 : 1; };

typedef __bf16 bf16x4 __attribute__((ext_vector_type(4)));

template <int NBLK, int SPP, int TGW, int WCB, int WPS>
__global__ __launch_bounds__(64 * NBLK * WCB, WPS) void k_wino3x3_bf16s_shared_relu_place(const float *__restrict__ src, int nseg, int t, int T,
                                                                                         const uint16_t *__restrict__ wu,
                                                                                         const float *__restrict__ bias, int cout,
                                                                                         float *__restrict__ dst, int dH, int dW, int dC, int off_y,
                                                                                         int off_x, int c_off, FastDiv fTT, FastDiv fT)
{
    constexpr int NW = NBLK * WCB, NT = 64 * NW, KG = NBLK, CIN = 8 * KG, S = CIN / 16, PHS = S / SPP, SLOTS = 32 * TGW * WCB, NP = 32 * NBLK;
    constexpr bool LATE = WPS == 4;
    constexpr int NH = TGW;
    constexpr int VT = SLOTS + WinoVPadW<KG>::value;
    constexpr int WPB = SPP * 3 * 1024;
    constexpr int PC = 3 * SPP, PC0 = (PC + WCB - 1) / WCB;
    static_assert(S % SPP == 0 && NT * NH == 2 * SLOTS * KG && (TGW == 1 || TGW == 2) && (WCB == 1 || WCB == 2), "staging items and waves");
    extern __shared__ uint4 lds_w[];
    char *const Wl = (char *)lds_w;
    uint4 *const V0 = (uint4 *)(Wl + 2 * NBLK * WPB), *const V1 = V0 + 3 * KG * VT;
    float *const lbias = (float *)(V1 + 3 * KG * VT);
    const int tid = threadIdx.x, lane = tid & 63, r = lane & 31, hh = lane >> 5;
    const int wv = __builtin_amdgcn_readfirstlane(tid >> 6), cb = wv % NBLK, wj = wv / NBLK, tg0 = wj * TGW;
    const int o = t - 2, TT = T * T;
    const int64_t ntiles = (int64_t)nseg * TT, src_floats = (int64_t)nseg * t * t * CIN;
    const int64_t ntasks = (ntiles + SLOTS - 1) / SLOTS;
    for (int i = tid; i < NP; i += NT) lbias[i] = i < cout ? bias[i] : 0.0f;

    const int item = NH == 2 ? tid : tid >> 1, shalf = NH == 2 ? 0 : tid & 1;
    const int sg = item % KG, sslot = item / KG;
    unsigned sbase;
    int slim;
    const char *const srcb = (const char *)src;
    auto stage_setup = [&](int64_t task) {
        int64_t m = task * SLOTS + sslot;
        if (m >= ntiles) m = ntiles - 1;
        const unsigned bu = fTT.div((unsigned)m), rem = (unsigned)m - bu * (unsigned)TT, ty = fT.div(rem), tx = rem - ty * (unsigned)T;
        const int64_t b = bu;
        const int64_t base = (((b * t + 2 * ty) * t + 2 * tx) * (int64_t)CIN + 8 * sg + 4 * shalf) * 4;
        const int64_t lim = src_floats * 4 - 16 * NH - base;
        sbase = (unsigned)base;
        slim = (int)(lim < (1 << 30) ? lim : (1 << 30));
    };
    float4 st[4][NH];
    auto stage_issue = [&](int p) {
        const int xi = p >> 2, nu = p & 3;
        const int ra0 = (0x1210 >> (4 * xi)) & 15, ra1 = (0x3122 >> (4 * xi)) & 15;
        const int rb0 = (0x1210 >> (4 * nu)) & 15, rb1 = (0x3122 >> (4 * nu)) & 15;
        const int os[4] = {(ra0 * t + rb0) * (CIN * 4), (ra0 * t + rb1) * (CIN * 4), (ra1 * t + rb0) * (CIN * 4), (ra1 * t + rb1) * (CIN * 4)};
#pragma unroll
        for (int i = 0; i < 4; ++i) {
            const char *q = srcb + (sbase + (unsigned)(os[i] < slim ? os[i] : slim));
#pragma unroll
            for (int h = 0; h < NH; ++h) st[i][h] = *(const float4 *)(q + 16 * h);
        }
    };
    auto stage_store = [&](int p, uint4 *Vn) {
        const float sx = (p >> 2) == 1 ? 1.0f : -1.0f, sn = (p & 3) == 1 ? 1.0f : -1.0f;
        bf16x4 v1[NH], v2[NH], v3[NH];
#pragma unroll
        for (int h = 0; h < NH; ++h) {
            const float a[4] = {st[0][h].x, st[0][h].y, st[0][h].z, st[0][h].w}, b[4] = {st[1][h].x, st[1][h].y, st[1][h].z, st[1][h].w},
                        c[4] = {st[2][h].x, st[2][h].y, st[2][h].z, st[2][h].w}, d[4] = {st[3][h].x, st[3][h].y, st[3][h].z, st[3][h].w};
#pragma unroll
            for (int e = 0; e < 4; ++e) {
                const float v = __builtin_fmaf(__builtin_fmaf(d[e], sn, c[e]), sx, __builtin_fmaf(b[e], sn, a[e]));
                __bf16 x1, x2, x3;
                split3(v, x1, x2, x3);
                v1[h][e] = x1; v2[h][e] = x2; v3[h][e] = x3;
            }
        }
        uint4 *q = Vn + sg * VT + sslot;
        if constexpr (NH == 2) {
            const uint2 a1 = __builtin_bit_cast(uint2, v1[0]), b1 = __builtin_bit_cast(uint2, v1[NH - 1]), a2 = __builtin_bit_cast(uint2, v2[0]),
                        b2 = __builtin_bit_cast(uint2, v2[NH - 1]), a3 = __builtin_bit_cast(uint2, v3[0]), b3 = __builtin_bit_cast(uint2, v3[NH - 1]);
            q[0] = make_uint4(a1.x, a1.y, b1.x, b1.y);
            q[KG * VT] = make_uint4(a2.x, a2.y, b2.x, b2.y);
            q[2 * KG * VT] = make_uint4(a3.x, a3.y, b3.x, b3.y);
        } else {
            ((uint2 *)q)[shalf] = __builtin_bit_cast(uint2, v1[0]);
            ((uint2 *)(q + KG * VT))[shalf] = __builtin_bit_cast(uint2, v2[0]);
            ((uint2 *)(q + 2 * KG * VT))[shalf] = __builtin_bit_cast(uint2, v3[0]);
        }
    };

    const unsigned wvoff = (unsigned)(lane * 16);
    auto w_pieces = [&](auto first, auto count, unsigned l, const char *gp) {
        constexpr int F = decltype(first)::value, N = decltype(count)::value;
#pragma unroll
        for (int i = 0; i + 3 <= N; i += 3) lds_dma_copy<3>(l + (F + i) * 1024u, gp + (F + i) * 1024, wvoff);
        if constexpr (N % 3 != 0) lds_dma_copy<N % 3>(l + (F + N - N % 3) * 1024u, gp + (F + N - N % 3) * 1024, wvoff);
    };
    auto w_issue = [&](int g, int buf) {
        const char *gp = (const char *)wu + ((int64_t)g * NBLK + cb) * WPB;
        const unsigned l = __builtin_amdgcn_readfirstlane((unsigned)(uintptr_t)(Wl + (buf * NBLK + cb) * WPB));
        if (WCB == 1 || wj == 0) w_pieces(std::integral_constant<int, 0>(), std::integral_constant<int, PC0>(), l, gp);
        else w_pieces(std::integral_constant<int, PC0>(), std::integral_constant<int, PC - PC0>(), l, gp);
    };

    int64_t task = blockIdx.x;
    if (task < ntasks) {
        stage_setup(task);
        stage_issue(0);
        stage_store(0, V0);
        w_issue(0, 0);
    }
    lds_dma_wait<0>();
    __syncthreads();
    for (; task < ntasks; task += gridDim.x) {
        const bool more = task + gridDim.x < ntasks;
        f16v Y[2][2][TGW];
#pragma unroll
        for (int i = 0; i < 2; ++i)
#pragma unroll
            for (int j = 0; j < 2; ++j)
#pragma unroll
                for (int tg = 0; tg < TGW; ++tg)
#pragma unroll
                    for (int e = 0; e < 16; ++e) Y[i][j][tg][e] = 0.0f;
        auto phase = [&](const char *Wb, const uint4 *Vc, int s0, f16v *M) {
            const uint4 *wq = (const uint4 *)Wb + lane;
#pragma unroll
            for (int sub = 0; sub < SPP; ++sub) {
                const int s = s0 + sub;
                const bf16x8 u1 = __builtin_bit_cast(bf16x8, wq[(3 * sub) * 64]), u2 = __builtin_bit_cast(bf16x8, wq[(3 * sub + 1) * 64]),
                             u3 = __builtin_bit_cast(bf16x8, wq[(3 * sub + 2) * 64]);
#pragma unroll
                for (int tg = 0; tg < TGW; ++tg) {
                    const uint4 *vq = Vc + (2 * s + hh) * VT + 32 * (tg0 + tg) + r;
                    const bf16x8 x1 = __builtin_bit_cast(bf16x8, vq[0]), x2 = __builtin_bit_cast(bf16x8, vq[KG * VT]),
                                 x3 = __builtin_bit_cast(bf16x8, vq[2 * KG * VT]);
                    M[tg] = __builtin_amdgcn_mfma_f32_32x32x16_bf16(u1, x3, M[tg], 0, 0, 0);
                    M[tg] = __builtin_amdgcn_mfma_f32_32x32x16_bf16(u2, x2, M[tg], 0, 0, 0);
                    M[tg] = __builtin_amdgcn_mfma_f32_32x32x16_bf16(u3, x1, M[tg], 0, 0, 0);
                    M[tg] = __builtin_amdgcn_mfma_f32_32x32x16_bf16(u1, x2, M[tg], 0, 0, 0);
                    M[tg] = __builtin_amdgcn_mfma_f32_32x32x16_bf16(u2, x1, M[tg], 0, 0, 0);
                    M[tg] = __builtin_amdgcn_mfma_f32_32x32x16_bf16(u1, x1, M[tg], 0, 0, 0);
                }
                if constexpr (WPS == 4) __builtin_amdgcn_sched_barrier(0);
            }
        };
        for (int p = 0; p < 16; ++p) {
            const uint4 *Vc = (p & 1) ? V1 : V0;
            uint4 *Vn = (p & 1) ? V0 : V1;
            const int pn = (p + 1) & 15;
            if (p == 15 && more) stage_setup(task + gridDim.x);
            const int xi = p >> 2, nu = p & 3;
            const float ax[2] = {xi < 3 ? 1.0f : 0.0f, xi == 0 ? 0.0f : xi == 1 ? 1.0f : -1.0f};
            const float an[2] = {nu < 3 ? 1.0f : 0.0f, nu == 0 ? 0.0f : nu == 1 ? 1.0f : -1.0f};
            f16v M[TGW];
#pragma unroll
            for (int tg = 0; tg < TGW; ++tg)
#pragma unroll
                for (int e = 0; e < 16; ++e) M[tg][e] = 0.0f;
#pragma unroll
            for (int h = 0; h < PHS; ++h) {
                const int g = p * PHS + h, gn = g + 1 == 16 * PHS ? 0 : g + 1;
                w_issue(gn, (g + 1) & 1);
                if (h == 0 && !LATE) stage_issue(pn);
                phase(Wl + ((g & 1) * NBLK + cb) * WPB, Vc, h * SPP, M);
                if (h == PHS - 1) {
                    if (LATE) stage_issue(pn);
                    stage_store(pn, Vn);
#pragma unroll
                    for (int i = 0; i < 2; ++i)
#pragma unroll
                        for (int j = 0; j < 2; ++j) {
                            const float c = ax[i] * an[j];
                            if (c != 0.0f) {
#pragma unroll
                                for (int tg = 0; tg < TGW; ++tg)
#pragma unroll
                                    for (int e = 0; e < 16; ++e) Y[i][j][tg][e] = __builtin_fmaf(M[tg][e], c, Y[i][j][tg][e]);
                            }
                        }
                }
                if (h == 0 && PHS > 1) lds_dma_wait<LATE ? 0 : 4 * NH>();
                else lds_dma_wait<0>();
                if (h == PHS - 1 || WCB > 1) __syncthreads();
            }
        }
        int le = lane;
        asm volatile("" : "+v"(le));
        const int re = le & 31, he = le >> 5;
        int64_t ro[TGW];
        bool valid[TGW], vy1[TGW], vx1[TGW];
#pragma unroll
        for (int tg = 0; tg < TGW; ++tg) {
            const int64_t m = task * SLOTS + (tg0 + tg) * 32 + re;
            valid[tg] = m < ntiles;
            const int64_t mm = valid[tg] ? m : ntiles - 1;
            const unsigned bu = fTT.div((unsigned)mm), rem = (unsigned)mm - bu * (unsigned)TT;
            const int ty = (int)fT.div(rem), tx = (int)(rem - (unsigned)ty * (unsigned)T);
            const int64_t b = bu;
            ro[tg] = ((b * dH + off_y + 2 * ty) * dW + off_x + 2 * tx) * (int64_t)dC + c_off + 32 * cb + 4 * he;
            vy1[tg] = 2 * ty + 1 < o;
            vx1[tg] = 2 * tx + 1 < o;
        }
#pragma unroll
        for (int tg = 0; tg < TGW; ++tg) {
            if (!valid[tg]) continue;
#pragma unroll
            for (int i = 0; i < 2; ++i)
#pragma unroll
                for (int j = 0; j < 2; ++j) {
                    if ((i == 1 && !vy1[tg]) || (j == 1 && !vx1[tg])) continue;
                    float *q = dst + ro[tg] + ((int64_t)i * dW + j) * dC;
#pragma unroll
                    for (int gq = 0; gq < 4; ++gq) {
                        const int c = 32 * cb + 8 * gq + 4 * he;
                        if (c < cout) store_bias_relu(q + 8 * gq, Y[i][j][tg], gq, *(const float4 *)(lbias + c));
                    }
                }
        }
    }
}

template <int NBLK, int SPP, int TGW, int WCB, int WPS>
static int launch_wino3x3_bf16s_shared(hipStream_t s, const float *src, int n, int t, const uint16_t *wu, const float *bias, int cout,
                                       const Place &pl)
{
    constexpr int KG = NBLK, CIN = 8 * NBLK, SLOTS = 32 * TGW * WCB, VT = SLOTS + WinoVPadW<KG>::value;
    constexpr size_t lds = (size_t)2 * NBLK * SPP * 3 * 1024 + (size_t)2 * 3 * KG * VT * 16 + 32 * NBLK * sizeof(float);
    constexpr int per_cu = 4 * WPS / (NBLK * WCB);
    static_assert(per_cu >= 1 && per_cu * lds <= 160 * 1024 - 256, "LDS of a CU's workgroups");
    static unsigned long long attr_mask = 0;
    if (!ensure_dyn_lds((const void *)k_wino3x3_bf16s_shared_relu_place<NBLK, SPP, TGW, WCB, WPS>, 160 * 1024 - 256, attr_mask)) return SWK_ERR_HIP;
    if ((int64_t)n * t * t * CIN * 4 >= ((int64_t)1 << 32)) return SWK_ERR_CAPACITY;
    const int T = (t - 2 + 1) / 2;
    const int64_t ntiles = (int64_t)n * T * T;
    int64_t blocks = (ntiles + SLOTS - 1) / SLOTS;
    if (blocks > 256 * per_cu) blocks = 256 * per_cu;
    hipLaunchKernelGGL((k_wino3x3_bf16s_shared_relu_place<NBLK, SPP, TGW, WCB, WPS>), dim3((unsigned)blocks), dim3(64 * NBLK * WCB), lds, s, src, n, t,
                       T, wu, bias, cout, pl.dst, pl.dH, pl.dW, pl.dC, pl.off_y, pl.off_x, pl.c_off, FastDiv((unsigned)(T * T)),
                       FastDiv((unsigned)T));
    return hipGetLastError() == hipSuccess ? SWK_OK : SWK_ERR_HIP;
}

int g_wino_bf16s_layout = 0;

}

#pragma GCC visibility push(default)
extern "C" {

int32_t swk_winograd_f2x2_3x3_weights_bf16s(const float *weight, int32_t cout, int32_t cin, uint16_t *out)
{
    if (!weight || !out || cout < 1 || cin < 16 || (cin & 15)) return SWK_ERR_ARG;
    const int spp = swk::wino_bf16s_spp(cin, cout), S = cin / 16, PHS = S / spp, CG = (cout + 31) / 32;
    if (S % spp) return SWK_ERR_ARG;
    for (int64_t i = 0, e = (int64_t)16 * cin * CG * 32 * 3; i < e; ++i) out[i] = 0;
    for (int co = 0; co < cout; ++co)
        for (int ci = 0; ci < cin; ++ci) {
            double U[4][4];
            swk::winograd_U(weight + ((int64_t)co * cin + ci) * 9, U);
            const int s = ci >> 4, ph = s / spp, sub = s % spp, lane = ((ci >> 3) & 1) * 32 + (co & 31), j = ci & 7, cb = co >> 5;
            for (int p = 0; p < 16; ++p) {
                uint16_t part[3];
                swk::split3_host((float)U[p >> 2][p & 3], part);
                const int64_t blk = (((int64_t)p * PHS + ph) * CG + cb) * spp + sub;
                for (int k = 0; k < 3; ++k) out[((blk * 3 + k) * 64 + lane) * 8 + j] = part[k];
            }
        }
    return SWK_OK;
}

int32_t swk_nhwc_conv3x3_winograd_bf16s_bias_relu_place(void *stream, const float *src, int32_t n, int32_t t, int32_t cin,
                                                        const uint16_t *weight_s, const float *bias, int32_t cout, float *dst, int32_t dH,
                                                        int32_t dW, int32_t dC, int32_t off_y, int32_t off_x, int32_t c_off)
{
    const swk::Place pl{dst, dH, dW, dC, off_y, off_x, c_off};
    if (!src || !weight_s || !bias || n < 1 || t < 3 || !swk::place_ok(pl, t - 2, t - 2, cout, true) || (((uintptr_t)src | (uintptr_t)weight_s) & 15))
        return SWK_ERR_ARG;
    using namespace swk;
    hipStream_t s = (hipStream_t)stream;
    const int knob = g_wino_bf16s_layout;
    if (cin == 16 && cout == 64) return launch_wino3x3_bf16s<2, 1>(s, src, n, t, weight_s, bias, cout, pl);
    if (cin == 32 && cout == 128) {
        const int lay = knob ? knob : 1;
        if (lay == 2) return launch_wino3x3_bf16s_shared<4, 2, 2, 2, 2>(s, src, n, t, weight_s, bias, cout, pl);
        return launch_wino3x3_bf16s<4, 2>(s, src, n, t, weight_s, bias, cout, pl);
    }
    if (cin == 48 && cout == 192) {
        const int lay = knob ? knob : 2;
        if (lay == 2) return launch_wino3x3_bf16s_shared<6, 3, 1, 2, 3>(s, src, n, t, weight_s, bias, cout, pl);
        return launch_wino3x3_bf16s<6, 3>(s, src, n, t, weight_s, bias, cout, pl);
    }
    if (cin == 64 && cout == 256) {
        const int lay = knob ? knob : 2;
        if (lay == 2) return launch_wino3x3_bf16s_shared<8, 2, 1, 2, 4>(s, src, n, t, weight_s, bias, cout, pl);
        return launch_wino3x3_bf16s<8, 2>(s, src, n, t, weight_s, bias, cout, pl);
    }
    return SWK_ERR_ARG;
}

}
#pragma GCC visibility pop
```

### swiftwatcher_amd/segment_classification.py

```python
import ctypes
import os
import threading

import numpy as np
import torch
from torch import nn

IMAGENET_MEAN = (0.485, 0.456, 0.406)
IMAGENET_STD = (0.229, 0.224, 0.225)
RESIZE = 24
PAD = (224 - 24) // 2


class Fire(nn.Module):

    def __init__(self, inplanes, squeeze_planes, expand1x1_planes, expand3x3_planes):
        super().__init__()
        self.squeeze = nn.Conv2d(inplanes, squeeze_planes, kernel_size=1)
        self.squeeze_activation = nn.ReLU(inplace=True)
        self.expand1x1 = nn.Conv2d(squeeze_planes, expand1x1_planes, kernel_size=1)
        self.expand1x1_activation = nn.ReLU(inplace=True)
        self.expand3x3 = nn.Conv2d(squeeze_planes, expand3x3_planes, kernel_size=3, padding=1)
        self.expand3x3_activation = nn.ReLU(inplace=True)

    def forward(self, x):
        x = self.squeeze_activation(self.squeeze(x))
        return torch.cat([self.expand1x1_activation(self.expand1x1(x)),
                          self.expand3x3_activation(self.expand3x3(x))], 1)


class SqueezeNet10(nn.Module):

    def __init__(self, num_classes=2):
        super().__init__()
        self.num_classes = num_classes
        self.features = nn.Sequential(
            nn.Conv2d(3, 96, kernel_size=7, stride=2), nn.ReLU(inplace=True),
            nn.MaxPool2d(kernel_size=3, stride=2, ceil_mode=True),
            Fire(96, 16, 64, 64), Fire(128, 16, 64, 64), Fire(128, 32, 128, 128),
            nn.MaxPool2d(kernel_size=3, stride=2, ceil_mode=True),
            Fire(256, 32, 128, 128), Fire(256, 48, 192, 192), Fire(384, 48, 192, 192), Fire(384, 64, 256, 256),
            nn.MaxPool2d(kernel_size=3, stride=2, ceil_mode=True),
            Fire(512, 64, 256, 256))
        self.classifier = nn.Sequential(nn.Dropout(p=0.5), nn.Conv2d(512, num_classes, kernel_size=1),
                                        nn.ReLU(inplace=True), nn.AdaptiveAvgPool2d((1, 1)))

    def forward(self, x):
        return torch.flatten(self.classifier(self.features(x)), 1)


def _dropout_head(x, pos, bg, n_pos, hw, hb, keys, seed, samples):
    from . import _lib
    lib = _lib.load()
    k = x.shape[0]
    if not (x.is_contiguous(memory_format=torch.channels_last) and hw.shape[0] == 2 and keys.shape[0] == k and keys.is_contiguous()):
        raise RuntimeError("the dropout head needs a channels-last tensor, a two-class head and one key per segment")
    out = torch.empty((k, samples, 2), dtype=torch.float32, device=x.device)
    stream = ctypes.c_void_p(torch.cuda.current_stream(x.device).cuda_stream)
    rc = lib.swk_nhwc_head2_dropout_relu_mean(stream, x.data_ptr(), k, x.shape[2] * x.shape[3], x.shape[1], pos.data_ptr(),
                                              None if bg is None else bg.data_ptr(), n_pos, hw.data_ptr(), hb.data_ptr(), keys.data_ptr(),
                                              ctypes.c_uint64(seed & 0xFFFFFFFFFFFFFFFF), samples, out.data_ptr())
    if rc:
        raise RuntimeError("swk_nhwc_head2_dropout_relu_mean failed (%d)" % rc)
    return out


def _affected(lo, hi, k, st, pad, out_size):
    a = -((-(lo + pad - k + 1)) // st)
    b = (hi + pad) // st
    return max(a, 0), min(b, out_size - 1)


class CroppedSqueezeNet10:

    IN_LO, IN_HI = 92, 131

    def __init__(self, model, border):
        self.model = model
        dev = next(model.parameters()).device
        feats = list(model.features)
        with torch.no_grad():
            x = border.to(dev, torch.float32).view(1, 3, 1, 1).expand(1, 3, 224, 224).contiguous()
            maps = []
            for layer in feats:
                maps.append(x)
                x = layer(x)
            head = torch.relu(model.classifier[1](x))
        lo, hi = PAD, PAD + RESIZE - 1
        size = 224
        self.plan = []
        assert isinstance(feats[0], nn.Conv2d) and feats[0].padding == (0, 0)
        out_size = maps[1].shape[-1]
        lo, hi = _affected(lo, hi, 7, 2, 0, out_size)
        need = (2 * lo, 2 * hi + 6)
        assert need[0] >= self.IN_LO and need[1] <= self.IN_HI
        assert (2 * lo - self.IN_LO) % 2 == 0
        self.conv_skip = (2 * lo - self.IN_LO) // 2
        conv_lo = lo - self.conv_skip
        conv_hi = conv_lo + (self.IN_HI - self.IN_LO + 1 - 7) // 2
        size = out_size
        out_size = maps[3].shape[-1]
        plo, phi = _affected(lo, hi, 3, 2, 0, out_size)
        assert 2 * plo >= conv_lo and 2 * phi + 2 <= conv_hi
        self.pool1_slice = (2 * plo - conv_lo, 2 * phi + 2 - conv_lo + 1)
        lo, hi, size = plo, phi, out_size
        for i in range(3, len(feats)):
            layer = feats[i]
            in_map = maps[i]
            if isinstance(layer, Fire):
                a, b = max(lo - 1, 0), min(hi + 1, size - 1)
                n0, n1 = a - 1, b + 1
                c0, c1 = max(n0, 0), min(n1, size - 1)
                tile = in_map[:, :, c0:c1 + 1, c0:c1 + 1].contiguous()
                self.plan.append(("fire", layer, tile, lo - c0, hi - lo + 1, (c0 - n0, n1 - c1), (a - c0, b - a + 1)))
                lo, hi = a, b
            else:
                out_size = maps[i + 1].shape[-1] if i + 1 < len(feats) else x.shape[-1]
                a, b = _affected(lo, hi, 3, 2, 0, out_size)
                n0, n1 = 2 * a, 2 * b + 2
                assert n0 >= 0 and n1 <= size - 1
                tile = in_map[:, :, n0:n1 + 1, n0:n1 + 1].contiguous()
                self.plan.append(("pool", layer, tile, lo - n0, hi - lo + 1, None, None))
                lo, hi, size = a, b, out_size
        self.final = (lo, hi, size)
        self.final_bg = x[:, :, lo:hi + 1, lo:hi + 1].contiguous()
        ring = head.clone()
        ring[:, :, lo:hi + 1, lo:hi + 1] = 0
        self.ring_sum = ring.sum(dim=(2, 3))
        self.n_pos = float(size * size)
        self.head_bg = x.permute(0, 2, 3, 1).reshape(size * size, x.shape[1]).contiguous()
        self.head_pos = torch.tensor([r * size + c for r in range(lo, hi + 1) for c in range(lo, hi + 1)], dtype=torch.int32, device=dev)
        self.sq_bg = []
        with torch.no_grad():
            for kind, layer, tile, off, n, pad, crop in self.plan:
                if kind != "fire":
                    self.sq_bg.append(None)
                    continue
                sq = layer.squeeze_activation(layer.squeeze(tile))
                if pad[0] or pad[1]:
                    sq = torch.nn.functional.pad(sq, (pad[0], pad[1], pad[0], pad[1]))
                self.sq_bg.append(sq.contiguous())
        self._cap = 0
        self._buf = None
        self.memory_format = torch.channels_last if dev.type == "cuda" else torch.contiguous_format
        if self.memory_format == torch.channels_last:
            model.to(memory_format=torch.channels_last)
        self.own_kernels = os.environ.get("SWK_OWN_CNN_KERNELS", "1") == "1"
        self._head = None
        self.winograd = True
        self.wino_split_bf16 = os.environ.get("SWK_WINO_SPLIT_BF16", "1") == "1"
        self.fuse_pool = os.environ.get("SWK_FUSE_POOL", "1") == "1"
        self._w1 = None
        self._wt3 = {}
        self._ww3 = {}
        self._ws3 = {}

    def macs_per_segment(self):
        m = self.model
        c1 = m.features[0]
        side = (self.IN_HI - self.IN_LO + 1 - 7) // 2 + 1
        executed = useful = side * side * c1.out_channels * c1.in_channels * 49
        last_n = None
        on_gpu = self.ring_sum.is_cuda and self.memory_format == torch.channels_last and self.own_kernels
        for kind, layer, tile, off, n, pad, crop in self.plan:
            if kind != "fire":
                continue
            t = tile.shape[2] + pad[0] + pad[1]
            sq, e1, e3 = layer.squeeze, layer.expand1x1, layer.expand3x3
            executed += n * n * sq.out_channels * sq.in_channels
            e1_side = n if on_gpu else t
            executed += e1_side * e1_side * e1.out_channels * e1.in_channels
            wino = on_gpu and self.winograd and e3.out_channels == 4 * e3.in_channels and e3.in_channels in (16, 32, 48, 64)
            if wino:
                tiles = ((t - 2 + 1) // 2) ** 2
                executed += tiles * 16 * e3.out_channels * e3.in_channels
            else:
                executed += (t - 2) ** 2 * e3.out_channels * e3.in_channels * 9
            useful += n * n * sq.out_channels * sq.in_channels
            useful += crop[1] ** 2 * (e1.out_channels * e1.in_channels + e3.out_channels * e3.in_channels * 9)
            last_n = crop[1]
        head = m.classifier[1]
        executed += last_n * last_n * head.out_channels * head.in_channels
        useful += last_n * last_n * head.out_channels * head.in_channels
        return int(executed), int(useful)

    def _buffers(self, batch):
        if batch <= self._cap:
            return self._buf
        bufs = []
        for (kind, layer, tile, off, n, pad, crop), sq in zip(self.plan, self.sq_bg):
            if kind == "fire":
                bufs.append(sq.expand(batch, -1, -1, -1).contiguous(memory_format=self.memory_format))
            else:
                bufs.append(tile.expand(batch, -1, -1, -1).contiguous(memory_format=self.memory_format))
        live = []
        for j, (kind, layer, tile, off, n, pad, crop) in enumerate(self.plan):
            nxt = self.plan[j + 1][0] if j + 1 < len(self.plan) else "head"
            if kind == "fire" and nxt != "pool":
                if nxt == "fire":
                    _, _, ntile, noff, nn, _, _ = self.plan[j + 1]
                    bg = ntile[:, :, noff:noff + nn, noff:noff + nn]
                else:
                    bg = self.final_bg
                assert bg.shape[2] == crop[1] and bg.shape[1] == layer.expand1x1.out_channels + layer.expand3x3.out_channels
                live.append(bg.expand(batch, -1, -1, -1).contiguous(memory_format=self.memory_format))
            else:
                live.append(None)
        self._buf, self._cap = (bufs, live), batch
        self.version = getattr(self, "version", 0) + 1
        return self._buf

    def _gpu_path(self, tiles):
        return tiles.is_cuda and self.memory_format == torch.channels_last and all(
            kind != "fire" or not (pad[0] or pad[1]) for kind, _, _, _, _, pad, _ in self.plan)

    def reserve(self, batch):
        self._buffers(batch)
        if self.ring_sum.is_cuda:
            self._aux_buffers(batch)
            self._prepare_operands()

    def _prepare_operands(self):
        if not (self.own_kernels and self.ring_sum.is_cuda and self.memory_format == torch.channels_last):
            return
        self._conv1_operand()
        for j, (kind, layer, tile, off, n, pad, crop) in enumerate(self.plan):
            if kind == "fire":
                self._w3_operand(j, layer.expand3x3)
        self._head_operand()

    def _conv1_operand(self):
        if self._w1 is None:
            self._w1 = self.model.features[0].weight.detach().contiguous(memory_format=torch.contiguous_format).clone()
        return self._w1

    def _head_operand(self):
        if self._head is None:
            head = self.model.classifier[1]
            self._head = (head.weight.detach().reshape(head.out_channels, -1).contiguous(), head.bias.detach().contiguous(),
                          self.ring_sum.reshape(-1).contiguous())
        return self._head

    def _w3_kind(self, conv):
        cin, cout = conv.in_channels, conv.out_channels
        if self.winograd and cout == 4 * cin and cin in (16, 32, 48, 64):
            return "bf16s" if self.wino_split_bf16 and cin != 16 else "f32"
        return "direct"

    def _w3_operand(self, j, conv, kind=None):
        from . import _lib
        kind = kind or self._w3_kind(conv)
        cache = {"bf16s": self._ws3, "f32": self._ww3, "direct": self._wt3}[kind]
        w = cache.get(j)
        if w is not None:
            return w
        cin, cout = conv.in_channels, conv.out_channels
        dev = conv.weight.device
        if kind == "direct":
            w = conv.weight.detach().permute(2, 3, 1, 0).contiguous(memory_format=torch.contiguous_format)
        else:
            lib = _lib.load()
            wc = conv.weight.detach().to("cpu", torch.float32).contiguous()
            ncol = 32 * (-(-cout // 32))
            if kind == "bf16s":
                out = torch.empty(3 * 16 * cin * ncol, dtype=torch.int16)
                if lib.swk_winograd_f2x2_3x3_weights_bf16s(wc.data_ptr(), cout, cin, out.data_ptr()):
                    raise RuntimeError("swk_winograd_f2x2_3x3_weights_bf16s failed")
            else:
                out = torch.empty(16 * cin * ncol, dtype=torch.float32)
                if lib.swk_winograd_f2x2_3x3_weights(wc.data_ptr(), cout, cin, out.data_ptr()):
                    raise RuntimeError("swk_winograd_f2x2_3x3_weights failed")
            w = out.to(dev)
        cache[j] = w
        return w

    @torch.no_grad()
    def __call__(self, tiles, row0=0, dropout=None):
        if self._gpu_path(tiles):
            with torch.cuda.device(tiles.device):
                return self._forward_hip_glue(tiles, row0, dropout)
        if dropout is not None:
            raise RuntimeError("dropout sampling runs on the library's HIP head kernel: it needs the GPU path")
        if row0:
            raise ValueError("row0 is a feature of the GPU path")
        m = self.model
        conv2d = torch.nn.functional.conv2d
        k = tiles.shape[0]
        bufs, live = self._buffers(k)
        x = torch.relu(m.features[0](tiles.contiguous(memory_format=self.memory_format)))
        a, b = self.pool1_slice
        x = m.features[2](x[:, :, a:b, a:b])
        for j, (kind, layer, tile, off, n, pad, crop) in enumerate(self.plan):
            if kind == "pool":
                x = layer(bufs[j][:k])
                continue
            sq = bufs[j][:k]
            o = off + pad[0]
            torch.clamp_min(layer.squeeze(x), 0, out=sq[:, :, o:o + n, o:o + n])
            e3 = conv2d(sq, layer.expand3x3.weight, layer.expand3x3.bias)
            e1 = conv2d(sq, layer.expand1x1.weight, layer.expand1x1.bias)
            c, cn = crop
            c1 = layer.expand1x1.out_channels
            if live[j] is not None:
                dest = live[j][:k]
            else:
                _, _, _, poff, pn, _, _ = self.plan[j + 1]
                assert pn == cn
                dest = bufs[j + 1][:k, :, poff:poff + pn, poff:poff + pn]
            cp = c + pad[0]
            torch.clamp_min(e1[:, :, cp:cp + cn, cp:cp + cn], 0, out=dest[:, :c1])
            torch.clamp_min(e3, 0, out=dest[:, c1:])
            x = dest
        s = torch.relu(m.classifier[1](x)).sum(dim=(2, 3))
        return (s + self.ring_sum) / self.n_pos

    def _forward_hip_glue(self, tiles, row0=0, dropout=None):
        from . import _lib
        lib = _lib.load()
        stream = ctypes.c_void_p(torch.cuda.current_stream(tiles.device).cuda_stream)
        m = self.model
        conv2d = torch.nn.functional.conv2d
        k = tiles.shape[0]
        bufs, live = self._buffers(row0 + k)
        rows = slice(row0, row0 + k)
        cl = torch.channels_last

        def nhwc(t):
            return t if t.is_contiguous(memory_format=cl) else t.contiguous(memory_format=cl)

        def place(e, bias, dest, crop, size, off, c_off):
            e = nhwc(e)
            rc = lib.swk_nhwc_bias_relu_place(stream, e.data_ptr(), k, e.shape[2], e.shape[3], e.shape[1], crop, crop, size, size,
                                              bias.data_ptr(), dest.data_ptr(), dest.shape[2], dest.shape[3], dest.shape[1],
                                              off, off, c_off)
            if rc:
                raise RuntimeError("swk_nhwc_bias_relu_place failed (%d)" % rc)

        def conv1x1(src, crop, size, conv, dest, off, c_off):
            src = nhwc(src)
            wgt = conv.weight.reshape(conv.out_channels, conv.in_channels)
            rc = lib.swk_nhwc_conv1x1_bias_relu_place(stream, src.data_ptr(), k, src.shape[2], src.shape[3], src.shape[1], crop, crop,
                                                      size, size, wgt.data_ptr(), conv.bias.data_ptr(), conv.out_channels,
                                                      dest.data_ptr(), dest.shape[2], dest.shape[3], dest.shape[1], off, off, c_off)
            if rc:
                raise RuntimeError("swk_nhwc_conv1x1_bias_relu_place failed (%d)" % rc)

        def conv3x3(src, j, conv, dest, off, c_off):
            src = nhwc(src)
            cin, cout = conv.in_channels, conv.out_channels
            kind = self._w3_kind(conv)
            if kind != "direct" and k * src.shape[2] * src.shape[2] * cin * 4 < (1 << 32):
                ww = self._w3_operand(j, conv, kind)
                fn = "swk_nhwc_conv3x3_winograd_bf16s_bias_relu_place" if kind == "bf16s" else "swk_nhwc_conv3x3_winograd_bias_relu_place"
                rc = getattr(lib, fn)(stream, src.data_ptr(), k, src.shape[2], cin, ww.data_ptr(), conv.bias.data_ptr(), cout,
                                      dest.data_ptr(), dest.shape[2], dest.shape[3], dest.shape[1], off, off, c_off)
                if rc:
                    raise RuntimeError("%s failed (%d)" % (fn, rc))
                return
            wt = self._w3_operand(j, conv, "direct")
            assert src.shape[2] == src.shape[3]
            rc = lib.swk_nhwc_conv3x3_bias_relu_place(stream, src.data_ptr(), k, src.shape[2], src.shape[1], wt.data_ptr(),
                                                      conv.bias.data_ptr(), conv.out_channels, dest.data_ptr(), dest.shape[2],
                                                      dest.shape[3], dest.shape[1], off, off, c_off)
            if rc:
                raise RuntimeError("swk_nhwc_conv3x3_bias_relu_place failed (%d)" % rc)

        def pool(src, dst):
            rc = lib.swk_nhwc_maxpool3s2(stream, src.data_ptr(), k, src.shape[2], src.shape[3], src.shape[1], dst.data_ptr())
            if rc:
                raise RuntimeError("swk_nhwc_maxpool3s2 failed (%d)" % rc)

        def pool_squeeze(src, conv, dest, off, ring=None, live=(0, 0)):
            wgt = conv.weight.reshape(conv.out_channels, conv.in_channels)
            rc = lib.swk_nhwc_maxpool3s2_conv1x1_bias_relu_place(stream, src.data_ptr(), k, src.shape[2], src.shape[1], wgt.data_ptr(),
                                                                 conv.bias.data_ptr(), conv.out_channels, dest.data_ptr(), dest.shape[2],
                                                                 dest.shape[3], dest.shape[1], off, off,
                                                                 None if ring is None else ring.data_ptr(), live[0], live[1])
            if rc:
                raise RuntimeError("swk_nhwc_maxpool3s2_conv1x1_bias_relu_place failed (%d)" % rc)

        aux = self._aux_buffers(row0 + k)
        conv1 = m.features[0]
        a, b = self.pool1_slice
        c1buf = aux["conv1"][rows]
        side = tiles.shape[2]
        if self.own_kernels and conv1.out_channels == 96 and side % 2 == 0 and 2 * (b - 1) + 8 <= side:
            w1 = self._conv1_operand()
            xin = nhwc(tiles)
            rc = lib.swk_nhwc_conv7x7s2_bias_relu(stream, xin.data_ptr(), k, side, a, b - a, w1.data_ptr(), conv1.bias.data_ptr(),
                                                  conv1.out_channels, c1buf.data_ptr())
            if rc:
                raise RuntimeError("swk_nhwc_conv7x7s2_bias_relu failed (%d)" % rc)
        else:
            e = conv2d(nhwc(tiles), conv1.weight, None, stride=conv1.stride)
            place(e, conv1.bias, c1buf, a, b - a, 0, 0)
        fuse = self.fuse_pool and self.own_kernels
        to_pool = c1buf
        pool_ring, pool_live = None, (0, 0)
        x = aux["pool_in"][rows]
        if not fuse:
            pool(c1buf, x)
        pi = 0
        for j, (kind, layer, tile, off, n, pad, crop) in enumerate(self.plan):
            if kind == "pool":
                x = aux["pool_out"][pi][rows]
                if fuse:
                    to_pool, pool_ring, pool_live = bufs[j][rows], bufs[j][0:1], (off, n)
                else:
                    pool(bufs[j][rows], x)
                pi += 1
                continue
            sq = bufs[j][rows]
            c, cn = crop
            c1 = layer.expand1x1.out_channels
            if live[j] is not None:
                dest, doff = live[j][rows], 0
            else:
                dest, doff = bufs[j + 1][rows], self.plan[j + 1][3]
            if self.own_kernels:
                if fuse and to_pool is not None:
                    assert (to_pool.shape[2] - 3) // 2 + 1 == n
                    pool_squeeze(to_pool, layer.squeeze, sq, off, pool_ring, pool_live)
                    to_pool = None
                else:
                    conv1x1(x, 0, n, layer.squeeze, sq, off, 0)
                conv1x1(sq, off, n, layer.expand1x1, dest, doff + off - c, 0)
            else:
                place(conv2d(x, layer.squeeze.weight, None), layer.squeeze.bias, sq, 0, n, off, 0)
                e1 = conv2d(sq, layer.expand1x1.weight, None)
                place(e1, layer.expand1x1.bias, dest, c, cn, doff, 0)
            if self.own_kernels:
                conv3x3(sq, j, layer.expand3x3, dest, doff, c1)
            else:
                place(conv2d(sq, layer.expand3x3.weight, None), layer.expand3x3.bias, dest, 0, cn, doff, c1)
            x = dest
        head = m.classifier[1]
        if dropout is not None:
            if not (self.own_kernels and head.out_channels == 2 and x.shape[1] in (256, 512, 768, 1024)):
                raise RuntimeError("dropout sampling runs on the library's HIP head kernel (own kernels, a two-class head)")
            hw, hb, _ = self._head_operand()
            keys, seed, samples = dropout
            return _dropout_head(x, self.head_pos, self.head_bg, int(self.n_pos), hw, hb, keys, seed, samples)
        if self.own_kernels and head.out_channels == 2 and x.shape[1] in (256, 512, 768, 1024) and x.is_contiguous(memory_format=cl):
            hw, hb, ring = self._head_operand()
            out = torch.empty((k, 2), dtype=torch.float32, device=x.device)
            rc = lib.swk_nhwc_head2_relu_mean(stream, x.data_ptr(), k, x.shape[2] * x.shape[3], x.shape[1], hw.data_ptr(), hb.data_ptr(),
                                              ring.data_ptr(), self.n_pos, out.data_ptr())
            if rc:
                raise RuntimeError("swk_nhwc_head2_relu_mean failed (%d)" % rc)
            return out
        px = x.permute(0, 2, 3, 1).reshape(-1, x.shape[1])
        s = torch.relu(torch.nn.functional.linear(px, head.weight.view(head.out_channels, -1), head.bias))
        s = s.view(k, -1, head.out_channels).sum(dim=1)
        return (s + self.ring_sum) / self.n_pos

    def _aux_buffers(self, batch):
        if getattr(self, "_aux_cap", 0) >= batch:
            return self._aux
        dev = self.ring_sum.device
        cl = torch.channels_last

        def buf(c, h):
            return torch.empty((batch, c, h, h), dtype=torch.float32, device=dev).contiguous(memory_format=cl)

        a, b = self.pool1_slice
        conv1_c = self.model.features[0].out_channels
        aux = {"conv1": buf(conv1_c, b - a), "pool_in": buf(conv1_c, (b - a - 3) // 2 + 1), "pool_out": []}
        for kind, layer, tile, off, n, pad, crop in self.plan:
            if kind == "pool":
                aux["pool_out"].append(buf(tile.shape[1], (tile.shape[2] - 3) // 2 + 1))
        self._aux, self._aux_cap = aux, batch
        self.version = getattr(self, "version", 0) + 1
        return aux


def setup_model(num_classes):
    model = SqueezeNet10(num_classes)
    for p in model.parameters():
        p.requires_grad = False
    return model


def resize_segment(segment_image):
    if segment_image.shape[0] == RESIZE and segment_image.shape[1] == RESIZE:
        return np.ascontiguousarray(segment_image)
    from PIL import Image
    bil = getattr(Image, "Resampling", Image).BILINEAR
    return np.asarray(Image.fromarray(np.ascontiguousarray(segment_image)).resize((RESIZE, RESIZE), bil))


class SegmentClassifier:

    @classmethod
    def from_state_dict(cls, state, **kw):
        import io
        buf = io.BytesIO()
        torch.save(state, buf)
        buf.seek(0)
        return cls(buf, **kw)

    def __init__(self, model_path, device=None, batch_size=1024, cropped=True, dropout_seed=None):
        if device is None:
            if not torch.cuda.is_available():
                raise RuntimeError("SegmentClassifier runs on the MI355X (PyTorch-ROCm); pass device='cpu' "
                                   "explicitly to run the torch CPU kernels instead")
            device = "cuda:0"
        self.device = torch.device(device)
        self._cudnn_benchmark = self.device.type == "cuda" and os.environ.get("SWK_CUDNN_BENCHMARK", "1") == "1"
        self.batch_size = batch_size
        self.model = setup_model(2)
        state = torch.load(model_path, map_location="cpu", weights_only=True)
        self.model.load_state_dict(state, strict=True)
        self.model = self.model.to(self.device).eval()
        mean = torch.tensor(IMAGENET_MEAN, dtype=torch.float32, device=self.device).view(1, 3, 1, 1)
        std = torch.tensor(IMAGENET_STD, dtype=torch.float32, device=self.device).view(1, 3, 1, 1)
        self._mean, self._std = mean, std
        self._border = ((0.0 - mean) / std).expand(1, 3, 224, 224).contiguous()
        self.cropped = CroppedSqueezeNet10(self.model, ((0.0 - mean) / std).view(3)) if cropped else None
        self.timing = False
        self._events = []
        self._slots = None
        self._lock = threading.RLock()
        self._split_rows = int(os.environ.get("SWK_CNN_SPLIT_ROWS", "1024")) if self.device.type == "cuda" else 0
        self._side_stream = None
        self._graphs = {}
        self._use_graphs = self.device.type == "cuda" and os.environ.get("SWK_HIP_GRAPHS", "1") == "1"
        self._graph_error = None
        self.dropout_seed = None if dropout_seed is None else int(dropout_seed)
        self._full_head = None

    def preprocess(self, segment_images, window=False):
        lo, hi = (CroppedSqueezeNet10.IN_LO, CroppedSqueezeNet10.IN_HI + 1) if window else (0, 224)
        if self.device.type == "cuda" and all(max(im.shape[0], im.shape[1]) <= 512 for im in segment_images):
            from . import _lib
            x = torch.empty((len(segment_images), 3, hi - lo, hi - lo), dtype=torch.float32, device=self.device)
            torch.cuda.current_stream(self.device).synchronize()
            _lib.default_context(self.device.index or 0).classifier_input(segment_images, IMAGENET_MEAN, IMAGENET_STD,
                                                                          net_ptr=x.data_ptr(), pad=PAD - lo)
            return x
        patches = np.stack([resize_segment(im) for im in segment_images])
        t = torch.from_numpy(patches).to(self.device).permute(0, 3, 1, 2).to(torch.float32).div_(255.0)
        t = (t - self._mean) / self._std
        x = self._border[:, :, lo:hi, lo:hi].repeat(t.shape[0], 1, 1, 1)
        x[:, :, PAD - lo:PAD - lo + RESIZE, PAD - lo:PAD - lo + RESIZE] = t
        return x

    @torch.no_grad()
    def _bucket(self, k):
        if self.device.type != "cuda":
            return k
        if k >= self.batch_size:
            return max(self.batch_size, k)
        if k <= 512:
            return min(self.batch_size, -(-k // 64) * 64)
        return min(self.batch_size, -(-k // 512) * 512)

    def _forward(self, x):
        if self._cudnn_benchmark and (self.cropped is None or not self.cropped.own_kernels):
            with torch.backends.cudnn.flags(enabled=True, benchmark=True):
                return self.cropped(x) if self.cropped is not None else self.model(x)
        if (self._split_rows and x.shape[0] >= self._split_rows and self.cropped is not None and self.cropped.own_kernels
                and self.cropped._gpu_path(x)):
            return self._forward_two_streams(x)
        return self.cropped(x) if self.cropped is not None else self.model(x)

    def _full_head_operand(self, n_pos):
        if self._full_head is None or self._full_head[2].shape[0] != n_pos:
            head = self.model.classifier[1]
            self._full_head = (head.weight.detach().reshape(head.out_channels, -1).contiguous(), head.bias.detach().contiguous(),
                               torch.arange(n_pos, dtype=torch.int32, device=self.device))
        return self._full_head

    @torch.no_grad()
    def _forward_dropout(self, x, keys, samples, seed):
        if self.device.type != "cuda":
            raise RuntimeError("dropout sampling runs on the library's HIP head kernel: it needs the GPU")
        samples = int(samples)
        if not 1 <= samples <= 256:
            raise ValueError("samples must be 1..256")
        if self.cropped is not None:
            if not (self.cropped.own_kernels and self.cropped._gpu_path(x)):
                raise RuntimeError("dropout sampling runs on the library's own kernels (SWK_OWN_CNN_KERNELS=1, channels-last)")
            self.cropped.reserve(x.shape[0])
            return self.cropped(x, dropout=(keys, int(seed), samples))
        with torch.cuda.device(self.device):
            with torch.backends.cudnn.flags(enabled=True, benchmark=self._cudnn_benchmark):
                f = self.model.features(x)
            f = f.contiguous(memory_format=torch.channels_last)
            n_pos = f.shape[2] * f.shape[3]
            hw, hb, pos = self._full_head_operand(n_pos)
            return _dropout_head(f, pos, None, n_pos, hw, hb, keys, int(seed), samples)

    def _keys_tensor(self, keys, k):
        if not (isinstance(keys, np.ndarray) and keys.dtype in (np.uint64, np.int64)):
            keys = np.array([int(v) & 0xFFFFFFFFFFFFFFFF for v in np.asarray(keys, dtype=object).reshape(-1)], dtype=np.uint64)
        keys = np.ascontiguousarray(keys.reshape(-1)).view(np.int64)
        if keys.shape[0] != k:
            raise ValueError("%d keys for %d segments" % (keys.shape[0], k))
        return torch.from_numpy(keys.copy()).to(self.device)

    def dropout_scores(self, segment_images, keys, samples=32, seed=0):
        with self._lock:
            kt = self._keys_tensor(keys, len(segment_images))
            out = []
            for i in range(0, len(segment_images), self.batch_size):
                chunk = segment_images[i:i + self.batch_size]
                x = self.preprocess(chunk, window=self.cropped is not None)
                out.append(self._forward_dropout(x, kt[i:i + len(chunk)], samples, seed))
            return torch.cat(out) if out else torch.zeros((0, int(samples), 2), device=self.device)

    def keep_probability(self, segments, samples=32, seed=0):
        from .data_structures import segment_keys
        if not segments:
            return np.zeros(0, np.float64)
        keys = segment_keys([s.parent_frame_number for s in segments], [s.label for s in segments])
        sc = self.dropout_scores([s.segment_image for s in segments], keys, samples, seed)
        return (sc[:, :, 1] > sc[:, :, 0]).sum(dim=1).cpu().numpy().astype(np.float64) / float(int(samples))

    def _predict_images(self, segments):
        images = [s.segment_image for s in segments]
        if self.dropout_seed is None:
            return torch.max(self.scores(images), 1)[1].cpu().numpy()
        from .data_structures import segment_keys
        keys = segment_keys([s.parent_frame_number for s in segments], [s.label for s in segments])
        return torch.max(self.dropout_scores(images, keys, 1, self.dropout_seed)[:, 0], 1)[1].cpu().numpy()

    def _forward_two_streams(self, x):
        k = x.shape[0]
        half = -(-k // 2 // 512) * 512
        cur = torch.cuda.current_stream(self.device)
        if self._side_stream is None:
            self._side_stream = torch.cuda.Stream(device=self.device)
        side = self._side_stream
        self.cropped.reserve(k)
        side.wait_stream(cur)
        with torch.cuda.stream(side):
            hi = self.cropped(x[half:], row0=half)
        lo = self.cropped(x[:half])
        cur.wait_stream(side)
        hi.record_stream(cur)
        return torch.cat([lo, hi])

    def _forward_graphed(self, x):
        key = (x.data_ptr(), int(x.shape[0]), getattr(self.cropped, "version", 0))
        entry = self._graphs.get(key)
        if entry is None:
            try:
                self._forward(x)
                torch.cuda.current_stream(self.device).synchronize()
                graph = torch.cuda.CUDAGraph()
                with torch.cuda.graph(graph, capture_error_mode="thread_local"):
                    out = self._forward(x)
                if len(self._graphs) >= 24:
                    self._graphs.clear()
                entry = self._graphs[key] = (graph, out)
            except Exception as exc:
                self._use_graphs = False
                self._graph_error = repr(exc)
                torch.cuda.synchronize(self.device)
                return self._forward(x)
        entry[0].replay()
        return entry[1]

    def _run(self, x, k, persistent=False):
        if persistent and self._use_graphs and x.shape[0] <= 512 and self.cropped is not None and not self.timing:
            return self._forward_graphed(x)[:k]
        if self.timing and self.device.type == "cuda":
            a, b = torch.cuda.Event(enable_timing=True), torch.cuda.Event(enable_timing=True)
            a.record()
            out = self._forward(x)[:k]
            b.record()
            self._events.append((a, b, int(x.shape[0])))
            return out
        return self._forward(x)[:k]

    def net_time(self, reset=True):
        if self._events:
            torch.cuda.synchronize(self.device)
        ms = sum(a.elapsed_time(b) for a, b, _ in self._events)
        rows, calls = sum(r for _, _, r in self._events), len(self._events)
        if reset:
            self._events = []
        return ms, rows, calls

    def _scores_unlocked(self, segment_images):
        out = []
        for i in range(0, len(segment_images), self.batch_size):
            chunk = segment_images[i:i + self.batch_size]
            k, b = len(chunk), self._bucket(len(chunk))
            x = self.preprocess(chunk, window=self.cropped is not None)
            if b != k:
                x = torch.cat([x, x[:1].expand(b - k, -1, -1, -1)])
            out.append(self._run(x, k))
        return torch.cat(out) if out else torch.zeros((0, 2), device=self.device)

    def _device_slots(self, side, nhwc):
        key = (side, nhwc, self.batch_size)
        if self._slots is None or self._slots[0] != key:
            fmt = torch.channels_last if nhwc else torch.contiguous_format
            xb = [torch.empty((self.batch_size, 3, side, side), dtype=torch.float32, device=self.device, memory_format=fmt) for _ in range(2)]
            fb = [torch.empty((self.batch_size,), dtype=torch.int32, device=self.device) for _ in range(2)]
            torch.cuda.current_stream(self.device).synchronize()
            self._slots = (key, xb, fb, [None, None])
        return self._slots[1:]

    def scores(self, segment_images):
        with self._lock:
            return self._scores_unlocked(segment_images)

    def _scores_device(self, cut, keys=None):
        with self._lock:
            return self._scores_device_unlocked(cut, keys)

    @torch.no_grad()
    def _scores_device_unlocked(self, cut, keys=None):
        if self.device.type != "cuda":
            raise RuntimeError("device-resident scoring needs the GPU")
        pad = PAD - CroppedSqueezeNet10.IN_LO if self.cropped is not None else PAD
        side = RESIZE + 2 * pad
        bs = self.batch_size
        nhwc = self.cropped is not None and self.cropped.memory_format == torch.channels_last
        xb, fb, done = self._device_slots(side, nhwc)

        def produce(slot, first):
            if done[slot] is not None:
                done[slot].synchronize()
            total, skipped = cut(xb[slot].data_ptr(), fb[slot].data_ptr(), bs, first, pad, nhwc)
            if skipped:
                raise RuntimeError("%d segment boxes were empty or had a side above 4096 pixels" % skipped)
            return total

        scores, frames_of = [], []
        total = produce(0, 0)
        kt = self._keys_tensor(keys, total) if keys is not None else None
        first, i = 0, 0
        while first < total:
            slot = i & 1
            k = min(bs, total - first)
            if kt is not None:
                scores.append(self._forward_dropout(xb[slot][:k], kt[first:first + k], 1, self.dropout_seed)[:, 0])
            else:
                scores.append(self._run(xb[slot][:self._bucket(k)], k, persistent=True).clone())
            frames_of.append(fb[slot][:k].clone())
            done[slot] = torch.cuda.Event()
            done[slot].record(torch.cuda.current_stream(self.device))
            first += k
            i += 1
            if first < total:
                produce(i & 1, first)
        if not scores:
            return torch.zeros((0, 2), device=self.device), torch.zeros((0,), dtype=torch.int32, device=self.device)
        return torch.cat(scores), torch.cat(frames_of)

    def scores_from_device(self, ctx, inp, frame_hw, segs, nseg, seg_cap, min_seg_size=(24, 24)):
        def cut(net_ptr, frame_ptr, cap, first, pad, nhwc):
            return ctx.segment_inputs(inp, frame_hw, segs.data_ptr(), nseg.data_ptr(), seg_cap, IMAGENET_MEAN, IMAGENET_STD, net_ptr, cap,
                                      first=first, pad=pad, min_seg_size=min_seg_size, seg_frame_ptr=frame_ptr, channels_last=nhwc)
        return self._scores_device(cut)

    def predict_last_batch(self, ctx, generation, total, min_seg_size=(24, 24), keys=None):
        if self.dropout_seed is not None and keys is None:
            raise ValueError("a classifier with a dropout_seed needs the segments' keys")
        if self.dropout_seed is None:
            keys = None
        def cut(net_ptr, frame_ptr, cap, first, pad, nhwc):
            return ctx.segment_inputs_last(generation, IMAGENET_MEAN, IMAGENET_STD, net_ptr, cap, first=first, pad=pad,
                                           min_seg_size=min_seg_size, seg_frame_ptr=frame_ptr, channels_last=nhwc, known_total=total)
        scores, _ = self._scores_device(cut) if keys is None else self._scores_device(cut, keys)
        if scores.shape[0] != total:
            raise RuntimeError("the device holds %d segments, the window has %d" % (scores.shape[0], total))
        return torch.max(scores, 1)[1]

    def classify_frames(self, frames):
        segs = [s for fr in frames for s in fr.segments]
        if not segs:
            return
        pred = self._window_predictions(segs)
        if pred is None:
            pred = self._predict_images(segs)
        i = 0
        for fr in frames:
            kept = []
            for s in fr.segments:
                if pred[i] == 1:
                    kept.append(s)
                i += 1
            for j, s in enumerate(kept):
                s.label = j + 1
            fr.segments = kept

    def _window_predictions(self, segments):
        if self.device.type != "cuda":
            return None
        batch = getattr(segments[0], "_batch", None)
        if batch is None or any(getattr(s, "_batch", None) is not batch for s in segments):
            return None
        if (self.device.index or 0) != batch.ctx.device:
            return None
        table = batch.predictions(self)
        if table is None:
            return None
        return [table[s._index] for s in segments]

    def __call__(self, segments):
        if not segments:
            return []
        pred = self._window_predictions(segments)
        if pred is None:
            pred = self._predict_images(segments)
        kept = [s for s, y in zip(segments, pred) if y == 1]
        for i, s in enumerate(kept):
            s.label = i + 1
        return kept
```

Measured before the change: 42560.

## Fuse fire-module expand1x1 into the bf16-split Winograd expand3x3 kernel

Adds a fused fire-expand kernel that runs the 1x1 expand as extra pixel-direct phases inside the Winograd 3x3 task loop. It reuses the staged squeeze tiles and LDS weight pipeline, and writes both outputs with a live-region mask. This removes a separate expand1x1 launch and its re-read of the squeeze activations. In exchange, each task does extra phases over the full tile grid rather than only the live region, and LDS use grows. It is enabled by default for three channel configurations.

```diff
diff --git a/include/swk.h b/include/swk.h
--- a/include/swk.h
+++ b/include/swk.h
@@ -181,6 +181,13 @@
                                                         const uint16_t *weight_s, const float *bias, int32_t cout, float *dst, int32_t dH,
                                                         int32_t dW, int32_t dC, int32_t off_y, int32_t off_x, int32_t c_off);
 
+int32_t swk_expand1x1_weights_bf16s(const float *weight, int32_t cout, int32_t cin, uint16_t *out);
+int32_t swk_fire_expand_fused(int32_t cin, int32_t cout);
+int32_t swk_nhwc_fire_expand_bf16s_bias_relu_place(void *stream, const float *src, int32_t n, int32_t t, int32_t cin, const uint16_t *w3_s,
+                                                   const float *bias3, int32_t cout3, const uint16_t *w1_s, const float *bias1, int32_t cout1,
+                                                   float *dst, int32_t dH, int32_t dW, int32_t dC, int32_t off_y, int32_t off_x, int32_t c_off3,
+                                                   int32_t c_off1, int32_t live_lo, int32_t live_n);
+
 int32_t swk_track_costs(const double *prev_c, const double *prev_hist0, const uint8_t *prev_has_hist,
                         const double *curr_c, int32_t n_prev, int32_t n_curr, double *cost);
 int32_t swk_lsap(const double *cost, int32_t n_rows, int32_t n_cols, int32_t *col4row);
diff --git a/swiftwatcher_amd/_lib.py b/swiftwatcher_amd/_lib.py
--- a/swiftwatcher_amd/_lib.py
+++ b/swiftwatcher_amd/_lib.py
@@ -124,6 +124,9 @@
     "swk_winograd_f2x2_3x3_weights": (ctypes.c_int32, [ctypes.c_void_p, ctypes.c_int32, ctypes.c_int32, ctypes.c_void_p]),
     "swk_nhwc_conv3x3_winograd_bf16s_bias_relu_place": (ctypes.c_int32, [ctypes.c_void_p, ctypes.c_void_p, ctypes.c_int32, ctypes.c_int32, ctypes.c_int32, ctypes.c_void_p, ctypes.c_void_p, ctypes.c_int32, ctypes.c_void_p] + [ctypes.c_int32] * 6),
     "swk_winograd_f2x2_3x3_weights_bf16s": (ctypes.c_int32, [ctypes.c_void_p, ctypes.c_int32, ctypes.c_int32, ctypes.c_void_p]),
+    "swk_expand1x1_weights_bf16s": (ctypes.c_int32, [ctypes.c_void_p, ctypes.c_int32, ctypes.c_int32, ctypes.c_void_p]),
+    "swk_fire_expand_fused": (ctypes.c_int32, [ctypes.c_int32, ctypes.c_int32]),
+    "swk_nhwc_fire_expand_bf16s_bias_relu_place": (ctypes.c_int32, [ctypes.c_void_p, ctypes.c_void_p, ctypes.c_int32, ctypes.c_int32, ctypes.c_int32, ctypes.c_void_p, ctypes.c_void_p, ctypes.c_int32, ctypes.c_void_p, ctypes.c_void_p, ctypes.c_int32, ctypes.c_void_p] + [ctypes.c_int32] * 9),
     "swk_nhwc_maxpool3s2_conv1x1_bias_relu_place": (ctypes.c_int32, [ctypes.c_void_p, ctypes.c_void_p, ctypes.c_int32, ctypes.c_int32, ctypes.c_int32, ctypes.c_void_p, ctypes.c_void_p, ctypes.c_int32, ctypes.c_void_p] + [ctypes.c_int32] * 5 + [ctypes.c_void_p, ctypes.c_int32, ctypes.c_int32]),
     "swk_nhwc_maxpool3s2": (ctypes.c_int32, [ctypes.c_void_p, ctypes.c_void_p, ctypes.c_int32, ctypes.c_int32, ctypes.c_int32, ctypes.c_int32, ctypes.c_void_p]),
     "swk_nhwc_head2_relu_mean": (ctypes.c_int32, [ctypes.c_void_p, ctypes.c_void_p, ctypes.c_int32, ctypes.c_int32, ctypes.c_int32, ctypes.c_void_p,
diff --git a/swiftwatcher_amd/csrc/cnn_common.h b/swiftwatcher_amd/csrc/cnn_common.h
--- a/swiftwatcher_amd/csrc/cnn_common.h
+++ b/swiftwatcher_amd/csrc/cnn_common.h
@@ -27,6 +27,7 @@
                                 const float *bias, int cout, const Place &pl);
 extern int g_expand_split_bf16;
 extern int g_wino_bf16s_layout;
+extern int g_fire_expand_fused;
 
 __device__ __forceinline__ void store_bias_relu(float *q, const f16v &acc, int g, const float4 b)
 {
diff --git a/swiftwatcher_amd/csrc/cnn_conv1x1.hip b/swiftwatcher_amd/csrc/cnn_conv1x1.hip
--- a/swiftwatcher_amd/csrc/cnn_conv1x1.hip
+++ b/swiftwatcher_amd/csrc/cnn_conv1x1.hip
@@ -196,6 +196,7 @@
     if (knob == 0 && (value == 0 || value == 1)) { swk::g_conv1x1_ring = value; return SWK_OK; }
     if (knob == 1 && (value == 0 || value == 1)) { swk::g_expand_split_bf16 = value; return SWK_OK; }
     if (knob == 2 && value >= 0 && value <= 2) { swk::g_wino_bf16s_layout = value; return SWK_OK; }
+    if (knob == 4 && value >= 0 && value <= 2) { swk::g_fire_expand_fused = value; return SWK_OK; }
     return SWK_ERR_ARG;
 }
 
diff --git a/swiftwatcher_amd/csrc/cnn_wino3x3_bf16s.hip b/swiftwatcher_amd/csrc/cnn_wino3x3_bf16s.hip
--- a/swiftwatcher_amd/csrc/cnn_wino3x3_bf16s.hip
+++ b/swiftwatcher_amd/csrc/cnn_wino3x3_bf16s.hip
@@ -6,13 +6,30 @@
 
 static int wino_bf16s_spp(int cin, int cout) { return cin == 64 && cout == 256 ? 2 : cin / 16; }
 
+struct FireE1 {
+    const uint16_t *wu;
+    const float *bias;
+    int c_off, live_lo, live_n;
+};
+__device__ __forceinline__ unsigned fire_e1_mask(int y0, int x0, int o, int live_lo, int live_n)
+{
+    unsigned m = 0;
+#pragma unroll
+    for (int i = 0; i < 2; ++i)
+#pragma unroll
+        for (int j = 0; j < 2; ++j) {
+            const int y = y0 + i, x = x0 + j;
+            if (y < o && x < o && y >= live_lo && y < live_lo + live_n && x >= live_lo && x < live_lo + live_n) m |= 1u << (2 * i + j);
+        }
+    return m;
+}
+
 template <int KG> struct WinoVPad { static constexpr int value = KG == 6 ? 3 : 16 / KG; };
 
-template <int NBLK, int SPP>
-__global__ __launch_bounds__(64 * NBLK, 2) void k_wino3x3_bf16s_relu_place(const float *__restrict__ src, int nseg, int t, int T,
-                                                                          const uint16_t *__restrict__ wu, const float *__restrict__ bias,
-                                                                          int cout, float *__restrict__ dst, int dH, int dW, int dC, int off_y,
-                                                                          int off_x, int c_off, FastDiv fTT, FastDiv fT)
+template <int NBLK, int SPP, bool E1>
+__device__ __forceinline__ void wino3x3_bf16s_tasks(const float *__restrict__ src, int nseg, int t, int T, const uint16_t *__restrict__ wu,
+                                                    const float *__restrict__ bias, int cout, float *__restrict__ dst, int dH, int dW, int dC,
+                                                    int off_y, int off_x, int c_off, FastDiv fTT, FastDiv fT, const FireE1 e1)
 {
     constexpr int NW = NBLK, NT = 64 * NW, KG = NBLK, CIN = 8 * KG, S = CIN / 16, PHS = S / SPP, SLOTS = 64, NP = 32 * NBLK;
     constexpr int VT = SLOTS + WinoVPad<KG>::value;
@@ -27,6 +44,8 @@
     const int64_t ntiles = (int64_t)nseg * TT, src_floats = (int64_t)nseg * t * t * CIN;
     const int64_t ntasks = (ntiles + SLOTS - 1) / SLOTS;
     for (int i = tid; i < NP; i += NT) lbias[i] = i < cout ? bias[i] : 0.0f;
+    if constexpr (E1)
+        for (int i = tid; i < NP; i += NT) lbias[NP + i] = i < cout ? e1.bias[i] : 0.0f;
 
     const int sg = tid % KG, sslot = tid / KG;
     unsigned sbase;
@@ -55,7 +74,8 @@
             st[i][1] = *(const float4 *)(q + 16);
         }
     };
-    auto stage_store = [&](int p, uint4 *Vn) {
+    auto stage_store = [&](int p, uint4 *Vn, auto direct) {
+        constexpr bool DIRECT = decltype(direct)::value;
         const float sx = (p >> 2) == 1 ? 1.0f : -1.0f, sn = (p & 3) == 1 ? 1.0f : -1.0f;
         bf16x8 v1, v2, v3;
 #pragma unroll
@@ -64,7 +84,7 @@
                         c[4] = {st[2][h].x, st[2][h].y, st[2][h].z, st[2][h].w}, d[4] = {st[3][h].x, st[3][h].y, st[3][h].z, st[3][h].w};
 #pragma unroll
             for (int e = 0; e < 4; ++e) {
-                const float v = __builtin_fmaf(__builtin_fmaf(d[e], sn, c[e]), sx, __builtin_fmaf(b[e], sn, a[e]));
+                const float v = DIRECT ? a[e] : __builtin_fmaf(__builtin_fmaf(d[e], sn, c[e]), sx, __builtin_fmaf(b[e], sn, a[e]));
                 __bf16 x1, x2, x3;
                 split3(v, x1, x2, x3);
                 v1[4 * h + e] = x1; v2[4 * h + e] = x2; v3[4 * h + e] = x3;
@@ -75,10 +95,18 @@
         q[KG * VT] = __builtin_bit_cast(uint4, v2);
         q[2 * KG * VT] = __builtin_bit_cast(uint4, v3);
     };
+    auto stage_issue_px = [&](int d) {
+        const int os = ((1 + (d >> 1)) * t + 1 + (d & 1)) * (CIN * 4);
+        const char *q = srcb + (sbase + (unsigned)(os < slim ? os : slim));
+        st[0][0] = *(const float4 *)q;
+        st[0][1] = *(const float4 *)(q + 16);
+    };
+    constexpr std::false_type WINO{};
+    constexpr std::true_type PIXEL{};
 
     const unsigned wvoff = (unsigned)(lane * 16);
-    auto w_issue = [&](int g, int buf) {
-        const char *gp = (const char *)wu + ((int64_t)g * NW + __builtin_amdgcn_readfirstlane(wave)) * WPB;
+    auto w_issue = [&](const uint16_t *wbase, int g, int buf) {
+        const char *gp = (const char *)wbase + ((int64_t)g * NW + __builtin_amdgcn_readfirstlane(wave)) * WPB;
         const unsigned l = __builtin_amdgcn_readfirstlane((unsigned)(uintptr_t)(Wl + (buf * NW + wave) * WPB));
 #pragma unroll
         for (int sub = 0; sub < SPP; ++sub) lds_dma_copy<3>(l + sub * 3072u, gp + sub * 3072, wvoff);
@@ -88,8 +116,8 @@
     if (task < ntasks) {
         stage_setup(task);
         stage_issue(0);
-        stage_store(0, V0);
-        w_issue(0, 0);
+        stage_store(0, V0, WINO);
+        w_issue(wu, 0, 0);
     }
     lds_dma_wait<0>();
     __syncthreads();
@@ -143,7 +171,8 @@
             const uint4 *Vc = (p & 1) ? V1 : V0;
             uint4 *Vn = (p & 1) ? V0 : V1;
             const int pn = (p + 1) & 15;
-            if (p == 15 && more) stage_setup(task + gridDim.x);
+            const bool px = E1 && p == 15;
+            if (!E1 && p == 15 && more) stage_setup(task + gridDim.x);
             const int xi = p >> 2, nu = p & 3;
             const float ax[2] = {xi < 3 ? 1.0f : 0.0f, xi == 0 ? 0.0f : xi == 1 ? 1.0f : -1.0f};
             const float an[2] = {nu < 3 ? 1.0f : 0.0f, nu == 0 ? 0.0f : nu == 1 ? 1.0f : -1.0f};
@@ -155,11 +184,16 @@
 #pragma unroll
             for (int h = 0; h < PHS; ++h) {
                 const int g = p * PHS + h, gn = g + 1 == 16 * PHS ? 0 : g + 1;
-                w_issue(gn, (g + 1) & 1);
-                if (h == 0) stage_issue(pn);
+                if (E1 && g + 1 == 16 * PHS) w_issue(e1.wu, 0, 0);
+                else w_issue(wu, gn, (g + 1) & 1);
+                if (h == 0) {
+                    if (px) stage_issue_px(0);
+                    else stage_issue(pn);
+                }
                 phase(Wl + ((g & 1) * NW + wave) * WPB, Vc, h * SPP, M);
                 if (h == PHS - 1) {
-                    stage_store(pn, Vn);
+                    if (px) stage_store(0, Vn, PIXEL);
+                    else stage_store(pn, Vn, WINO);
 #pragma unroll
                     for (int i = 0; i < 2; ++i)
 #pragma unroll
@@ -173,8 +207,10 @@
                             }
                         }
                 }
-                if (h == 0 && PHS > 1) lds_dma_wait<8>();
-                else lds_dma_wait<0>();
+                if (h == 0 && PHS > 1) {
+                    if (px) lds_dma_wait<2>();
+                    else lds_dma_wait<8>();
+                } else lds_dma_wait<0>();
                 if (h == PHS - 1) __syncthreads();
             }
         }
@@ -194,17 +230,90 @@
                     }
                 }
         }
+        if constexpr (E1) {
+            int le = lane;
+            asm volatile("" : "+v"(le));
+            unsigned em[2];
+#pragma unroll
+            for (int tg = 0; tg < 2; ++tg) {
+                const int64_t m = task * SLOTS + tg * 32 + (le & 31);
+                const unsigned mm = (unsigned)(m < ntiles ? m : ntiles - 1), rem = mm - fTT.div(mm) * (unsigned)TT;
+                const int ty = (int)fT.div(rem), tx = (int)(rem - (unsigned)ty * (unsigned)T);
+                em[tg] = m < ntiles ? fire_e1_mask(2 * ty, 2 * tx, o, e1.live_lo, e1.live_n) : 0u;
+            }
+            for (int d = 0; d < 4; ++d) {
+                const uint4 *Vc = (d & 1) ? V1 : V0;
+                uint4 *Vn = (d & 1) ? V0 : V1;
+                if (d == 3 && more) stage_setup(task + gridDim.x);
+                f16v M[2];
+#pragma unroll
+                for (int tg = 0; tg < 2; ++tg)
+#pragma unroll
+                    for (int e = 0; e < 16; ++e) M[tg][e] = 0.0f;
+#pragma unroll
+                for (int h = 0; h < PHS; ++h) {
+                    const int g = d * PHS + h;
+                    if (d == 3 && h == PHS - 1) w_issue(wu, 0, 0);
+                    else w_issue(e1.wu, h + 1 == PHS ? 0 : h + 1, (g + 1) & 1);
+                    if (h == 0) {
+                        if (d < 3) stage_issue_px(d + 1);
+                        else stage_issue(0);
+                    }
+                    phase(Wl + ((g & 1) * NW + wave) * WPB, Vc, h * SPP, M);
+                    if (h == PHS - 1) {
+                        if (d < 3) stage_store(0, Vn, PIXEL);
+                        else stage_store(0, Vn, WINO);
+                    }
+                    if (h == 0 && PHS > 1) {
+                        if (d < 3) lds_dma_wait<2>();
+                        else lds_dma_wait<8>();
+                    } else lds_dma_wait<0>();
+                    if (h == PHS - 1) __syncthreads();
+                }
+#pragma unroll
+                for (int tg = 0; tg < 2; ++tg) {
+                    if (!((em[tg] >> d) & 1u)) continue;
+                    float *q = dst + ro[tg] + (e1.c_off - c_off) + ((int64_t)(d >> 1) * dW + (d & 1)) * dC;
+#pragma unroll
+                    for (int gq = 0; gq < 4; ++gq) {
+                        const int c = 32 * wave + 8 * gq + 4 * hh;
+                        if (c < cout) store_bias_relu(q + 8 * gq, M[tg], gq, *(const float4 *)(lbias + NP + c));
+                    }
+                }
+            }
+        }
     }
 }
 
 template <int NBLK, int SPP>
-static int launch_wino3x3_bf16s(hipStream_t s, const float *src, int n, int t, const uint16_t *wu, const float *bias, int cout, const Place &pl)
+__global__ __launch_bounds__(64 * NBLK, 2) void k_wino3x3_bf16s_relu_place(const float *__restrict__ src, int nseg, int t, int T,
+                                                                          const uint16_t *__restrict__ wu, const float *__restrict__ bias,
+                                                                          int cout, float *__restrict__ dst, int dH, int dW, int dC, int off_y,
+                                                                          int off_x, int c_off, FastDiv fTT, FastDiv fT)
+{
+    wino3x3_bf16s_tasks<NBLK, SPP, false>(src, nseg, t, T, wu, bias, cout, dst, dH, dW, dC, off_y, off_x, c_off, fTT, fT, FireE1{});
+}
+template <int NBLK, int SPP>
+__global__ __launch_bounds__(64 * NBLK, 2) void k_fire_expand_bf16s_relu_place(const float *__restrict__ src, int nseg, int t, int T,
+                                                                              const uint16_t *__restrict__ wu, const float *__restrict__ bias,
+                                                                              int cout, float *__restrict__ dst, int dH, int dW, int dC, int off_y,
+                                                                              int off_x, int c_off, FastDiv fTT, FastDiv fT, FireE1 e1)
+{
+    wino3x3_bf16s_tasks<NBLK, SPP, true>(src, nseg, t, T, wu, bias, cout, dst, dH, dW, dC, off_y, off_x, c_off, fTT, fT, e1);
+}
+
+template <int NBLK, int SPP, bool E1 = false>
+static int launch_wino3x3_bf16s(hipStream_t s, const float *src, int n, int t, const uint16_t *wu, const float *bias, int cout, const Place &pl,
+                                const FireE1 &e1 = FireE1{})
 {
     constexpr int NW = NBLK, KG = NBLK, CIN = 8 * NBLK, VT = 64 + WinoVPad<KG>::value;
-    const size_t lds = (size_t)2 * NW * SPP * 3 * 1024 + (size_t)2 * 3 * KG * VT * 16 + 32 * NBLK * sizeof(float);
-    static_assert((size_t)2 * NW * SPP * 3 * 1024 + (size_t)2 * 3 * KG * VT * 16 + 32 * NBLK * 4 <= 160 * 1024 - 256, "LDS of one workgroup");
+    constexpr size_t lds = (size_t)2 * NW * SPP * 3 * 1024 + (size_t)2 * 3 * KG * VT * 16 + (E1 ? 2 : 1) * 32 * NBLK * sizeof(float);
+    static_assert(lds <= 160 * 1024 - 256, "LDS of one workgroup");
     static unsigned long long attr_mask = 0;
-    if (!ensure_dyn_lds((const void *)k_wino3x3_bf16s_relu_place<NBLK, SPP>, 160 * 1024 - 256, attr_mask)) return SWK_ERR_HIP;
+    const void *kernel;
+    if constexpr (E1) kernel = (const void *)k_fire_expand_bf16s_relu_place<NBLK, SPP>;
+    else kernel = (const void *)k_wino3x3_bf16s_relu_place<NBLK, SPP>;
+    if (!ensure_dyn_lds(kernel, 160 * 1024 - 256, attr_mask)) return SWK_ERR_HIP;
     if ((int64_t)n * t * t * CIN * 4 >= ((int64_t)1 << 32)) return SWK_ERR_CAPACITY;
     const int T = (t - 2 + 1) / 2;
     const int64_t ntiles = (int64_t)n * T * T;
@@ -212,8 +321,13 @@
     const int64_t by_lds = (int64_t)((160 * 1024 - 256) / lds), by_waves = 8 / NW;
     const int64_t per_cu = by_waves < 1 ? 1 : (by_lds < by_waves ? by_lds : by_waves);
     if (blocks > 256 * per_cu) blocks = 256 * per_cu;
-    hipLaunchKernelGGL((k_wino3x3_bf16s_relu_place<NBLK, SPP>), dim3((unsigned)blocks), dim3(64 * NW), lds, s, src, n, t, T, wu, bias, cout, pl.dst,
-                       pl.dH, pl.dW, pl.dC, pl.off_y, pl.off_x, pl.c_off, FastDiv((unsigned)(T * T)), FastDiv((unsigned)T));
+    const FastDiv fTT((unsigned)(T * T)), fT((unsigned)T);
+    if constexpr (E1)
+        hipLaunchKernelGGL((k_fire_expand_bf16s_relu_place<NBLK, SPP>), dim3((unsigned)blocks), dim3(64 * NW), lds, s, src, n, t, T, wu, bias, cout,
+                           pl.dst, pl.dH, pl.dW, pl.dC, pl.off_y, pl.off_x, pl.c_off, fTT, fT, e1);
+    else
+        hipLaunchKernelGGL((k_wino3x3_bf16s_relu_place<NBLK, SPP>), dim3((unsigned)blocks), dim3(64 * NW), lds, s, src, n, t, T, wu, bias, cout,
+                           pl.dst, pl.dH, pl.dW, pl.dC, pl.off_y, pl.off_x, pl.c_off, fTT, fT);
     return hipGetLastError() == hipSuccess ? SWK_OK : SWK_ERR_HIP;
 }
 
@@ -221,12 +335,10 @@
 
 typedef __bf16 bf16x4 __attribute__((ext_vector_type(4)));
 
-template <int NBLK, int SPP, int TGW, int WCB, int WPS>
-__global__ __launch_bounds__(64 * NBLK * WCB, WPS) void k_wino3x3_bf16s_shared_relu_place(const float *__restrict__ src, int nseg, int t, int T,
-                                                                                         const uint16_t *__restrict__ wu,
-                                                                                         const float *__restrict__ bias, int cout,
-                                                                                         float *__restrict__ dst, int dH, int dW, int dC, int off_y,
-                                                                                         int off_x, int c_off, FastDiv fTT, FastDiv fT)
+template <int NBLK, int SPP, int TGW, int WCB, int WPS, bool E1>
+__device__ __forceinline__ void wino3x3_bf16s_shared_tasks(const float *__restrict__ src, int nseg, int t, int T, const uint16_t *__restrict__ wu,
+                                                           const float *__restrict__ bias, int cout, float *__restrict__ dst, int dH, int dW,
+                                                           int dC, int off_y, int off_x, int c_off, FastDiv fTT, FastDiv fT, const FireE1 e1)
 {
     constexpr int NW = NBLK * WCB, NT = 64 * NW, KG = NBLK, CIN = 8 * KG, S = CIN / 16, PHS = S / SPP, SLOTS = 32 * TGW * WCB, NP = 32 * NBLK;
     constexpr bool LATE = WPS == 4;
@@ -245,6 +357,8 @@
     const int64_t ntiles = (int64_t)nseg * TT, src_floats = (int64_t)nseg * t * t * CIN;
     const int64_t ntasks = (ntiles + SLOTS - 1) / SLOTS;
     for (int i = tid; i < NP; i += NT) lbias[i] = i < cout ? bias[i] : 0.0f;
+    if constexpr (E1)
+        for (int i = tid; i < NP; i += NT) lbias[NP + i] = i < cout ? e1.bias[i] : 0.0f;
 
     const int item = NH == 2 ? tid : tid >> 1, shalf = NH == 2 ? 0 : tid & 1;
     const int sg = item % KG, sslot = item / KG;
@@ -274,7 +388,8 @@
             for (int h = 0; h < NH; ++h) st[i][h] = *(const float4 *)(q + 16 * h);
         }
     };
-    auto stage_store = [&](int p, uint4 *Vn) {
+    auto stage_store = [&](int p, uint4 *Vn, auto direct) {
+        constexpr bool DIRECT = decltype(direct)::value;
         const float sx = (p >> 2) == 1 ? 1.0f : -1.0f, sn = (p & 3) == 1 ? 1.0f : -1.0f;
         bf16x4 v1[NH], v2[NH], v3[NH];
 #pragma unroll
@@ -283,7 +398,7 @@
                         c[4] = {st[2][h].x, st[2][h].y, st[2][h].z, st[2][h].w}, d[4] = {st[3][h].x, st[3][h].y, st[3][h].z, st[3][h].w};
 #pragma unroll
             for (int e = 0; e < 4; ++e) {
-                const float v = __builtin_fmaf(__builtin_fmaf(d[e], sn, c[e]), sx, __builtin_fmaf(b[e], sn, a[e]));
+                const float v = DIRECT ? a[e] : __builtin_fmaf(__builtin_fmaf(d[e], sn, c[e]), sx, __builtin_fmaf(b[e], sn, a[e]));
                 __bf16 x1, x2, x3;
                 split3(v, x1, x2, x3);
                 v1[h][e] = x1; v2[h][e] = x2; v3[h][e] = x3;
@@ -302,6 +417,14 @@
             ((uint2 *)(q + 2 * KG * VT))[shalf] = __builtin_bit_cast(uint2, v3[0]);
         }
     };
+    auto stage_issue_px = [&](int d) {
+        const int os = ((1 + (d >> 1)) * t + 1 + (d & 1)) * (CIN * 4);
+        const char *q = srcb + (sbase + (unsigned)(os < slim ? os : slim));
+#pragma unroll
+        for (int h = 0; h < NH; ++h) st[0][h] = *(const float4 *)(q + 16 * h);
+    };
+    constexpr std::false_type WINO{};
+    constexpr std::true_type PIXEL{};
 
     const unsigned wvoff = (unsigned)(lane * 16);
     auto w_pieces = [&](auto first, auto count, unsigned l, const char *gp) {
@@ -310,8 +433,8 @@
         for (int i = 0; i + 3 <= N; i += 3) lds_dma_copy<3>(l + (F + i) * 1024u, gp + (F + i) * 1024, wvoff);
         if constexpr (N % 3 != 0) lds_dma_copy<N % 3>(l + (F + N - N % 3) * 1024u, gp + (F + N - N % 3) * 1024, wvoff);
     };
-    auto w_issue = [&](int g, int buf) {
-        const char *gp = (const char *)wu + ((int64_t)g * NBLK + cb) * WPB;
+    auto w_issue = [&](const uint16_t *wbase, int g, int buf) {
+        const char *gp = (const char *)wbase + ((int64_t)g * NBLK + cb) * WPB;
         const unsigned l = __builtin_amdgcn_readfirstlane((unsigned)(uintptr_t)(Wl + (buf * NBLK + cb) * WPB));
         if (WCB == 1 || wj == 0) w_pieces(std::integral_constant<int, 0>(), std::integral_constant<int, PC0>(), l, gp);
         else w_pieces(std::integral_constant<int, PC0>(), std::integral_constant<int, PC - PC0>(), l, gp);
@@ -321,8 +444,8 @@
     if (task < ntasks) {
         stage_setup(task);
         stage_issue(0);
-        stage_store(0, V0);
-        w_issue(0, 0);
+        stage_store(0, V0, WINO);
+        w_issue(wu, 0, 0);
     }
     lds_dma_wait<0>();
     __syncthreads();
@@ -363,7 +486,8 @@
             const uint4 *Vc = (p & 1) ? V1 : V0;
             uint4 *Vn = (p & 1) ? V0 : V1;
             const int pn = (p + 1) & 15;
-            if (p == 15 && more) stage_setup(task + gridDim.x);
+            const bool px = E1 && p == 15;
+            if (!E1 && p == 15 && more) stage_setup(task + gridDim.x);
             const int xi = p >> 2, nu = p & 3;
             const float ax[2] = {xi < 3 ? 1.0f : 0.0f, xi == 0 ? 0.0f : xi == 1 ? 1.0f : -1.0f};
             const float an[2] = {nu < 3 ? 1.0f : 0.0f, nu == 0 ? 0.0f : nu == 1 ? 1.0f : -1.0f};
@@ -375,12 +499,18 @@
 #pragma unroll
             for (int h = 0; h < PHS; ++h) {
                 const int g = p * PHS + h, gn = g + 1 == 16 * PHS ? 0 : g + 1;
-                w_issue(gn, (g + 1) & 1);
-                if (h == 0 && !LATE) stage_issue(pn);
+                if (E1 && g + 1 == 16 * PHS) w_issue(e1.wu, 0, 0);
+                else w_issue(wu, gn, (g + 1) & 1);
+                auto issue = [&]() {
+                    if (px) stage_issue_px(0);
+                    else stage_issue(pn);
+                };
+                if (h == 0 && !LATE) issue();
                 phase(Wl + ((g & 1) * NBLK + cb) * WPB, Vc, h * SPP, M);
                 if (h == PHS - 1) {
-                    if (LATE) stage_issue(pn);
-                    stage_store(pn, Vn);
+                    if (LATE) issue();
+                    if (px) stage_store(0, Vn, PIXEL);
+                    else stage_store(pn, Vn, WINO);
 #pragma unroll
                     for (int i = 0; i < 2; ++i)
 #pragma unroll
@@ -394,8 +524,10 @@
                             }
                         }
                 }
-                if (h == 0 && PHS > 1) lds_dma_wait<LATE ? 0 : 4 * NH>();
-                else lds_dma_wait<0>();
+                if (h == 0 && PHS > 1) {
+                    if (px) lds_dma_wait<LATE ? 0 : NH>();
+                    else lds_dma_wait<LATE ? 0 : 4 * NH>();
+                } else lds_dma_wait<0>();
                 if (h == PHS - 1 || WCB > 1) __syncthreads();
             }
         }
@@ -404,6 +536,7 @@
         const int re = le & 31, he = le >> 5;
         int64_t ro[TGW];
         bool valid[TGW], vy1[TGW], vx1[TGW];
+        unsigned em[TGW];
 #pragma unroll
         for (int tg = 0; tg < TGW; ++tg) {
             const int64_t m = task * SLOTS + (tg0 + tg) * 32 + re;
@@ -415,6 +548,7 @@
             ro[tg] = ((b * dH + off_y + 2 * ty) * dW + off_x + 2 * tx) * (int64_t)dC + c_off + 32 * cb + 4 * he;
             vy1[tg] = 2 * ty + 1 < o;
             vx1[tg] = 2 * tx + 1 < o;
+            em[tg] = E1 && valid[tg] ? fire_e1_mask(2 * ty, 2 * tx, o, e1.live_lo, e1.live_n) : 0u;
         }
 #pragma unroll
         for (int tg = 0; tg < TGW; ++tg) {
@@ -432,31 +566,104 @@
                     }
                 }
         }
+        if constexpr (E1) {
+            for (int d = 0; d < 4; ++d) {
+                const uint4 *Vc = (d & 1) ? V1 : V0;
+                uint4 *Vn = (d & 1) ? V0 : V1;
+                if (d == 3 && more) stage_setup(task + gridDim.x);
+                f16v M[TGW];
+#pragma unroll
+                for (int tg = 0; tg < TGW; ++tg)
+#pragma unroll
+                    for (int e = 0; e < 16; ++e) M[tg][e] = 0.0f;
+#pragma unroll
+                for (int h = 0; h < PHS; ++h) {
+                    const int g = d * PHS + h;
+                    if (d == 3 && h == PHS - 1) w_issue(wu, 0, 0);
+                    else w_issue(e1.wu, h + 1 == PHS ? 0 : h + 1, (g + 1) & 1);
+                    auto issue = [&]() {
+                        if (d < 3) stage_issue_px(d + 1);
+                        else stage_issue(0);
+                    };
+                    if (h == 0 && !LATE) issue();
+                    phase(Wl + ((g & 1) * NBLK + cb) * WPB, Vc, h * SPP, M);
+                    if (h == PHS - 1) {
+                        if (LATE) issue();
+                        if (d < 3) stage_store(0, Vn, PIXEL);
+                        else stage_store(0, Vn, WINO);
+                    }
+                    if (h == 0 && PHS > 1) {
+                        if (d < 3) lds_dma_wait<LATE ? 0 : NH>();
+                        else lds_dma_wait<LATE ? 0 : 4 * NH>();
+                    } else lds_dma_wait<0>();
+                    if (h == PHS - 1 || WCB > 1) __syncthreads();
+                }
+#pragma unroll
+                for (int tg = 0; tg < TGW; ++tg) {
+                    if (!((em[tg] >> d) & 1u)) continue;
+                    float *q = dst + ro[tg] + (e1.c_off - c_off) + ((int64_t)(d >> 1) * dW + (d & 1)) * dC;
+#pragma unroll
+                    for (int gq = 0; gq < 4; ++gq) {
+                        const int c = 32 * cb + 8 * gq + 4 * he;
+                        if (c < cout) store_bias_relu(q + 8 * gq, M[tg], gq, *(const float4 *)(lbias + NP + c));
+                    }
+                }
+            }
+        }
     }
 }
 
 template <int NBLK, int SPP, int TGW, int WCB, int WPS>
+__global__ __launch_bounds__(64 * NBLK * WCB, WPS) void k_wino3x3_bf16s_shared_relu_place(const float *__restrict__ src, int nseg, int t, int T,
+                                                                                         const uint16_t *__restrict__ wu,
+                                                                                         const float *__restrict__ bias, int cout,
+                                                                                         float *__restrict__ dst, int dH, int dW, int dC, int off_y,
+                                                                                         int off_x, int c_off, FastDiv fTT, FastDiv fT)
+{
+    wino3x3_bf16s_shared_tasks<NBLK, SPP, TGW, WCB, WPS, false>(src, nseg, t, T, wu, bias, cout, dst, dH, dW, dC, off_y, off_x, c_off, fTT, fT,
+                                                                FireE1{});
+}
+template <int NBLK, int SPP, int TGW, int WCB, int WPS>
+__global__ __launch_bounds__(64 * NBLK * WCB, WPS) void k_fire_expand_bf16s_shared_relu_place(const float *__restrict__ src, int nseg, int t, int T,
+                                                                                             const uint16_t *__restrict__ wu,
+                                                                                             const float *__restrict__ bias, int cout,
+                                                                                             float *__restrict__ dst, int dH, int dW, int dC,
+                                                                                             int off_y, int off_x, int c_off, FastDiv fTT, FastDiv fT,
+                                                                                             FireE1 e1)
+{
+    wino3x3_bf16s_shared_tasks<NBLK, SPP, TGW, WCB, WPS, true>(src, nseg, t, T, wu, bias, cout, dst, dH, dW, dC, off_y, off_x, c_off, fTT, fT, e1);
+}
+
+template <int NBLK, int SPP, int TGW, int WCB, int WPS, bool E1 = false>
 static int launch_wino3x3_bf16s_shared(hipStream_t s, const float *src, int n, int t, const uint16_t *wu, const float *bias, int cout,
-                                       const Place &pl)
+                                       const Place &pl, const FireE1 &e1 = FireE1{})
 {
     constexpr int KG = NBLK, CIN = 8 * NBLK, SLOTS = 32 * TGW * WCB, VT = SLOTS + WinoVPadW<KG>::value;
-    constexpr size_t lds = (size_t)2 * NBLK * SPP * 3 * 1024 + (size_t)2 * 3 * KG * VT * 16 + 32 * NBLK * sizeof(float);
+    constexpr size_t lds = (size_t)2 * NBLK * SPP * 3 * 1024 + (size_t)2 * 3 * KG * VT * 16 + (E1 ? 2 : 1) * 32 * NBLK * sizeof(float);
     constexpr int per_cu = 4 * WPS / (NBLK * WCB);
     static_assert(per_cu >= 1 && per_cu * lds <= 160 * 1024 - 256, "LDS of a CU's workgroups");
     static unsigned long long attr_mask = 0;
-    if (!ensure_dyn_lds((const void *)k_wino3x3_bf16s_shared_relu_place<NBLK, SPP, TGW, WCB, WPS>, 160 * 1024 - 256, attr_mask)) return SWK_ERR_HIP;
+    const void *kernel;
+    if constexpr (E1) kernel = (const void *)k_fire_expand_bf16s_shared_relu_place<NBLK, SPP, TGW, WCB, WPS>;
+    else kernel = (const void *)k_wino3x3_bf16s_shared_relu_place<NBLK, SPP, TGW, WCB, WPS>;
+    if (!ensure_dyn_lds(kernel, 160 * 1024 - 256, attr_mask)) return SWK_ERR_HIP;
     if ((int64_t)n * t * t * CIN * 4 >= ((int64_t)1 << 32)) return SWK_ERR_CAPACITY;
     const int T = (t - 2 + 1) / 2;
     const int64_t ntiles = (int64_t)n * T * T;
     int64_t blocks = (ntiles + SLOTS - 1) / SLOTS;
     if (blocks > 256 * per_cu) blocks = 256 * per_cu;
-    hipLaunchKernelGGL((k_wino3x3_bf16s_shared_relu_place<NBLK, SPP, TGW, WCB, WPS>), dim3((unsigned)blocks), dim3(64 * NBLK * WCB), lds, s, src, n, t,
-                       T, wu, bias, cout, pl.dst, pl.dH, pl.dW, pl.dC, pl.off_y, pl.off_x, pl.c_off, FastDiv((unsigned)(T * T)),
-                       FastDiv((unsigned)T));
+    const FastDiv fTT((unsigned)(T * T)), fT((unsigned)T);
+    if constexpr (E1)
+        hipLaunchKernelGGL((k_fire_expand_bf16s_shared_relu_place<NBLK, SPP, TGW, WCB, WPS>), dim3((unsigned)blocks), dim3(64 * NBLK * WCB), lds, s,
+                           src, n, t, T, wu, bias, cout, pl.dst, pl.dH, pl.dW, pl.dC, pl.off_y, pl.off_x, pl.c_off, fTT, fT, e1);
+    else
+        hipLaunchKernelGGL((k_wino3x3_bf16s_shared_relu_place<NBLK, SPP, TGW, WCB, WPS>), dim3((unsigned)blocks), dim3(64 * NBLK * WCB), lds, s, src,
+                           n, t, T, wu, bias, cout, pl.dst, pl.dH, pl.dW, pl.dC, pl.off_y, pl.off_x, pl.c_off, fTT, fT);
     return hipGetLastError() == hipSuccess ? SWK_OK : SWK_ERR_HIP;
 }
 
 int g_wino_bf16s_layout = 0;
+int g_fire_expand_fused = 0;
 
 }
 
@@ -513,5 +720,61 @@
     return SWK_ERR_ARG;
 }
 
+int32_t swk_expand1x1_weights_bf16s(const float *weight, int32_t cout, int32_t cin, uint16_t *out)
+{
+    if (!weight || !out || cout < 1 || cin < 16 || (cin & 15)) return SWK_ERR_ARG;
+    const int spp = swk::wino_bf16s_spp(cin, cout), S = cin / 16, CG = (cout + 31) / 32;
+    if (S % spp) return SWK_ERR_ARG;
+    for (int64_t i = 0, e = (int64_t)cin * CG * 32 * 3; i < e; ++i) out[i] = 0;
+    for (int co = 0; co < cout; ++co)
+        for (int ci = 0; ci < cin; ++ci) {
+            const int s = ci >> 4, ph = s / spp, sub = s % spp, lane = ((ci >> 3) & 1) * 32 + (co & 31), j = ci & 7, cb = co >> 5;
+            uint16_t part[3];
+            swk::split3_host(weight[(int64_t)co * cin + ci], part);
+            const int64_t blk = ((int64_t)ph * CG + cb) * spp + sub;
+            for (int k = 0; k < 3; ++k) out[((blk * 3 + k) * 64 + lane) * 8 + j] = part[k];
+        }
+    return SWK_OK;
+}
+
+int32_t swk_fire_expand_fused(int32_t cin, int32_t cout)
+{
+    const bool built = (cin == 32 && cout == 128) || (cin == 48 && cout == 192) || (cin == 64 && cout == 256);
+    if (!built || swk::g_fire_expand_fused == 1) return 0;
+    return 1;
+}
+
+int32_t swk_nhwc_fire_expand_bf16s_bias_relu_place(void *stream, const float *src, int32_t n, int32_t t, int32_t cin, const uint16_t *w3_s,
+                                                   const float *bias3, int32_t cout3, const uint16_t *w1_s, const float *bias1, int32_t cout1,
+                                                   float *dst, int32_t dH, int32_t dW, int32_t dC, int32_t off_y, int32_t off_x, int32_t c_off3,
+                                                   int32_t c_off1, int32_t live_lo, int32_t live_n)
+{
+    const swk::Place pl{dst, dH, dW, dC, off_y, off_x, c_off3}, pl1{dst, dH, dW, dC, off_y, off_x, c_off1};
+    if (!src || !w3_s || !w1_s || !bias3 || !bias1 || n < 1 || t < 3 || cout1 != cout3 || !swk::place_ok(pl, t - 2, t - 2, cout3, true) ||
+        !swk::place_ok(pl1, t - 2, t - 2, cout1, true) || (((uintptr_t)src | (uintptr_t)w3_s | (uintptr_t)w1_s) & 15))
+        return SWK_ERR_ARG;
+    if ((c_off1 < c_off3 ? c_off3 - c_off1 : c_off1 - c_off3) < cout3 || live_lo < 0 || live_n < 0 || live_lo + live_n > t - 2) return SWK_ERR_ARG;
+    using namespace swk;
+    hipStream_t s = (hipStream_t)stream;
+    const FireE1 e1{w1_s, bias1, c_off1, live_lo, live_n};
+    const int knob = g_wino_bf16s_layout;
+    if (cin == 32 && cout3 == 128) {
+        const int lay = knob ? knob : 1;
+        if (lay == 2) return launch_wino3x3_bf16s_shared<4, 2, 2, 2, 2, true>(s, src, n, t, w3_s, bias3, cout3, pl, e1);
+        return launch_wino3x3_bf16s<4, 2, true>(s, src, n, t, w3_s, bias3, cout3, pl, e1);
+    }
+    if (cin == 48 && cout3 == 192) {
+        const int lay = knob ? knob : 2;
+        if (lay == 2) return launch_wino3x3_bf16s_shared<6, 3, 1, 2, 3, true>(s, src, n, t, w3_s, bias3, cout3, pl, e1);
+        return launch_wino3x3_bf16s<6, 3, true>(s, src, n, t, w3_s, bias3, cout3, pl, e1);
+    }
+    if (cin == 64 && cout3 == 256) {
+        const int lay = knob ? knob : 2;
+        if (lay == 2) return launch_wino3x3_bf16s_shared<8, 2, 1, 2, 4, true>(s, src, n, t, w3_s, bias3, cout3, pl, e1);
+        return launch_wino3x3_bf16s<8, 2, true>(s, src, n, t, w3_s, bias3, cout3, pl, e1);
+    }
+    return SWK_ERR_ARG;
+}
+
 }
 #pragma GCC visibility pop
diff --git a/swiftwatcher_amd/segment_classification.py b/swiftwatcher_amd/segment_classification.py
--- a/swiftwatcher_amd/segment_classification.py
+++ b/swiftwatcher_amd/segment_classification.py
@@ -150,10 +150,12 @@
         self.winograd = True
         self.wino_split_bf16 = os.environ.get("SWK_WINO_SPLIT_BF16", "1") == "1"
         self.fuse_pool = os.environ.get("SWK_FUSE_POOL", "1") == "1"
+        self.fuse_expand = os.environ.get("SWK_FUSE_EXPAND", "1") == "1"
         self._w1 = None
         self._wt3 = {}
         self._ww3 = {}
         self._ws3 = {}
+        self._ws1 = {}
 
     def macs_per_segment(self):
         m = self.model
@@ -169,6 +171,8 @@
             sq, e1, e3 = layer.squeeze, layer.expand1x1, layer.expand3x3
             executed += n * n * sq.out_channels * sq.in_channels
             e1_side = n if on_gpu else t
+            if on_gpu and self._fused_expand(layer, crop, t):
+                e1_side = 2 * ((t - 2 + 1) // 2)
             executed += e1_side * e1_side * e1.out_channels * e1.in_channels
             wino = on_gpu and self.winograd and e3.out_channels == 4 * e3.in_channels and e3.in_channels in (16, 32, 48, 64)
             if wino:
@@ -227,6 +231,8 @@
         for j, (kind, layer, tile, off, n, pad, crop) in enumerate(self.plan):
             if kind == "fire":
                 self._w3_operand(j, layer.expand3x3)
+                if self._fused_expand(layer, crop, tile.shape[2] + pad[0] + pad[1]):
+                    self._w1s_operand(j, layer.expand1x1)
         self._head_operand()
 
     def _conv1_operand(self):
@@ -246,6 +252,27 @@
         if self.winograd and cout == 4 * cin and cin in (16, 32, 48, 64):
             return "bf16s" if self.wino_split_bf16 and cin != 16 else "f32"
         return "direct"
+
+    def _fused_expand(self, layer, crop, t):
+        from . import _lib
+        e1, e3 = layer.expand1x1, layer.expand3x3
+        if not (self.fuse_expand and self.own_kernels and self._w3_kind(e3) == "bf16s"):
+            return False
+        if e1.out_channels != e3.out_channels or e1.in_channels != e3.in_channels or tuple(crop) != (1, t - 2):
+            return False
+        return bool(_lib.load().swk_fire_expand_fused(e3.in_channels, e3.out_channels))
+
+    def _w1s_operand(self, j, conv):
+        from . import _lib
+        w = self._ws1.get(j)
+        if w is None:
+            cin, cout = conv.in_channels, conv.out_channels
+            wc = conv.weight.detach().to("cpu", torch.float32).reshape(cout, cin).contiguous()
+            out = torch.empty(3 * cin * 32 * (-(-cout // 32)), dtype=torch.int16)
+            if _lib.load().swk_expand1x1_weights_bf16s(wc.data_ptr(), cout, cin, out.data_ptr()):
+                raise RuntimeError("swk_expand1x1_weights_bf16s failed")
+            w = self._ws1[j] = out.to(conv.weight.device)
+        return w
 
     def _w3_operand(self, j, conv, kind=None):
         from . import _lib
@@ -364,6 +391,17 @@
                                                       dest.shape[3], dest.shape[1], off, off, c_off)
             if rc:
                 raise RuntimeError("swk_nhwc_conv3x3_bias_relu_place failed (%d)" % rc)
+
+        def fire_expand(src, j, layer, dest, off, live_lo, live_n):
+            src = nhwc(src)
+            e1, e3 = layer.expand1x1, layer.expand3x3
+            rc = lib.swk_nhwc_fire_expand_bf16s_bias_relu_place(stream, src.data_ptr(), k, src.shape[2], e3.in_channels,
+                                                                self._w3_operand(j, e3, "bf16s").data_ptr(), e3.bias.data_ptr(),
+                                                                e3.out_channels, self._w1s_operand(j, e1).data_ptr(), e1.bias.data_ptr(),
+                                                                e1.out_channels, dest.data_ptr(), dest.shape[2], dest.shape[3],
+                                                                dest.shape[1], off, off, e1.out_channels, 0, live_lo, live_n)
+            if rc:
+                raise RuntimeError("swk_nhwc_fire_expand_bf16s_bias_relu_place failed (%d)" % rc)
 
         def pool(src, dst):
             rc = lib.swk_nhwc_maxpool3s2(stream, src.data_ptr(), k, src.shape[2], src.shape[3], src.shape[1], dst.data_ptr())
@@ -417,6 +455,8 @@
                 dest, doff = live[j][rows], 0
             else:
                 dest, doff = bufs[j + 1][rows], self.plan[j + 1][3]
+            t = sq.shape[2]
+            fused = self.own_kernels and self._fused_expand(layer, crop, t) and k * t * t * layer.expand3x3.in_channels * 4 < (1 << 32)
             if self.own_kernels:
                 if fuse and to_pool is not None:
                     assert (to_pool.shape[2] - 3) // 2 + 1 == n
@@ -424,12 +464,15 @@
                     to_pool = None
                 else:
                     conv1x1(x, 0, n, layer.squeeze, sq, off, 0)
-                conv1x1(sq, off, n, layer.expand1x1, dest, doff + off - c, 0)
+                if not fused:
+                    conv1x1(sq, off, n, layer.expand1x1, dest, doff + off - c, 0)
             else:
                 place(conv2d(x, layer.squeeze.weight, None), layer.squeeze.bias, sq, 0, n, off, 0)
                 e1 = conv2d(sq, layer.expand1x1.weight, None)
                 place(e1, layer.expand1x1.bias, dest, c, cn, doff, 0)
-            if self.own_kernels:
+            if fused:
+                fire_expand(sq, j, layer, dest, doff, off - c, n)
+            elif self.own_kernels:
                 conv3x3(sq, j, layer.expand3x3, dest, doff, c1)
             else:
                 place(conv2d(sq, layer.expand3x3.weight, None), layer.expand3x3.bias, dest, 0, cn, doff, c1)
```

After: 41880. 1.6% lower.
